# PrioteasaAndrei/music-style-transfer-ldm

Hardware: AMD Instinct MI355X
Metric: UNet denoising steps/sec on 1×128×512 mel-latents, 1/2/4/8 MI355X (higher is better)
Workload: dtype fp32; 1 GPU; config 2: 50-step DDIM reverse sample (49 UNet+update iterations per step), batch 8/GPU, 1x128x512 mel -> [8,32,16,64] latents, eta=0.0, hipGraph replay of 1 concurrent sub-batch chains; global_batch=8, parallelism=dp1 (batch shards)

## Files before the change

### include/ldm_capi.h

```cpp
#ifndef LDM_CAPI_H
#define LDM_CAPI_H

#include <stddef.h>
#include <stdint.h>

#ifdef __cplusplus
extern "C" {
#endif

#define LDM_CAPI_VERSION 1

const char* ldm_last_error(void);
int ldm_capi_version(void);
int ldm_device_count(int* count);

typedef struct ldm_conv_desc {
    int32_t B, Cin, Hin, Win;
    int32_t Cout, Hout, Wout;
    int32_t kh, kw, stride, pad, out_pad;
    int32_t transposed;
    int32_t layout;
} ldm_conv_desc;

enum {
// ... 19 lines not shown
    float bn_eps;
    int32_t act;
    const float* bcast_add;
    const float* skip_add;
    float* act_out;
    int32_t dtype;
} ldm_epilogue;

typedef struct ldm_conv_plan {
    int32_t kind;
    int32_t tm, tn, wk;
    int32_t ks;
    int32_t balance;
    int64_t packed_floats;
    int64_t ws_floats;
} ldm_conv_plan;

int ldm_conv_make_plan(const ldm_conv_desc* d, ldm_conv_plan* plan);
int ldm_conv_tiled_plan(const ldm_conv_desc* d, int32_t dtype, ldm_conv_plan* plan);
int ldm_conv_sconv_plan(const ldm_conv_desc* d, int32_t dtype, ldm_conv_plan* plan);
int ldm_conv_make_plan_forced(const ldm_conv_desc* d, int kind, int tm, int tn, int wk, int ks,
                              ldm_conv_plan* plan);
int ldm_conv_pack_weight(const ldm_conv_desc* d, const ldm_conv_plan* plan, const float* w,
                         float* packed, void* stream);
int32_t ldm_conv_storage16(const ldm_conv_desc* d, const ldm_conv_plan* plan);
int ldm_conv_forward(const ldm_conv_desc* d, const ldm_conv_plan* plan, const float* x, const float* w,
                     const ldm_epilogue* ep, float* y, void* stream);
int ldm_conv_forward_ws(const ldm_conv_desc* d, const ldm_conv_plan* plan, const float* x, const float* w,
                        const ldm_epilogue* ep, float* y, float* workspace, void* stream);

int64_t ldm_reduce_workspace_floats(int32_t B, int32_t C, int32_t HW);
int ldm_batchnorm_train(float* x, int32_t B, int32_t C, int32_t HW, const float* weight, const float* bias,
                        float* running_mean, float* running_var, float momentum, float eps, int32_t act,
                        float* save_mean, float* save_invstd, float* workspace, void* stream);
int ldm_batchnorm_train_out(const float* x, float* y, int32_t B, int32_t C, int32_t HW, const float* weight,
                            const float* bias, float* running_mean, float* running_var, float momentum, float eps,
                            int32_t act, float* save_mean, float* save_invstd, float* workspace, void* stream);
int ldm_batchnorm_stats(const float* x, int32_t B, int32_t C, int32_t HW, double* stats, float* workspace,
                        void* stream);
int ldm_batchnorm_stats_code(const float* x, int32_t code, int32_t B, int32_t C, int32_t HW, double* stats,
                             float* workspace, void* stream);
int ldm_batchnorm_apply(float* x, int32_t B, int32_t C, int32_t HW, const double* stats, double count,
                        const float* weight, const float* bias, float* running_mean, float* running_var,
                        float momentum, float eps, int32_t act, float* save_mean, float* save_invstd, void* stream);
int ldm_batchnorm_apply_out(const float* x, float* y, int32_t B, int32_t C, int32_t HW, const double* stats,
                            double count, const float* weight, const float* bias, float* running_mean,
                            float* running_var, float momentum, float eps, int32_t act, float* save_mean,
                            float* save_invstd, void* stream);

int ldm_batchnorm_eval(const float* x, float* y, int32_t B, int32_t C, int32_t HW, const float* weight,
                       const float* bias, const float* running_mean, const float* running_var, float eps, int32_t act,
                       void* stream);

int ldm_activation(const float* x, float* y, int64_t n, int32_t act, void* stream);

int ldm_sinusoid_embed(const void* t, int32_t t_is_float, int32_t B, int32_t dim, const float* freqs, float* out,
                       void* stream);

int ldm_time_mlp_forward(const void* t, int32_t t_is_float, int32_t B, int32_t dim, const float* freqs,
                         const float* w1, const float* b1, const float* w2, const float* b2, float* out,
                         void* stream);

int ldm_attention_fold_keys(const float* kv, const float* wq, const float* bq, int32_t B, int32_t E, int32_t heads,
                            int32_t S, float scale, float* kf, float* bf, void* stream);
int ldm_attention_folded(const float* z, const float* kv, const float* kf, const float* bf, float* out, int32_t B,
                         int32_t E, int32_t heads, int32_t L, int32_t S, void* stream);
int ldm_attention_folded_keys(const float* z, const float* kv, const float* kf, const float* bf,
                              const float* key_bias, float* out, int32_t B, int32_t E, int32_t heads, int32_t L,
                              int32_t S, void* stream);
int ldm_attention_fold_keys_bias(const float* kv, const float* wq, const float* bq, int32_t B, int32_t E,
                                 int32_t heads, int32_t S, float scale, const float* key_bias, float* kf, float* bf,
                                 void* stream);
int ldm_attention_folded_probs(const float* z, const float* kf, const float* bf, float* p, int32_t B, int32_t E,
                               int32_t heads, int32_t L, int32_t S, void* stream);
int32_t ldm_bneck_fold_supported(int32_t B, int32_t H, int32_t W);
int ldm_bneck_fold_values(const float* w_fold, const float* kv, float* u, int32_t B, void* stream);
int ldm_bneck_pv(const float* u, const float* p, const float* pos_bias, float* y, int32_t B, int32_t dtype,
                 void* stream);
int ldm_ca1_probs(const float* z4, const float* kf, const float* bf, float* p, int32_t B, void* stream);
int32_t ldm_ca1_probs_form(void);
int ldm_set_cin1_packed(int on);
int ldm_set_cin1_s1(int on);
int ldm_set_flash_split(int on);
int ldm_fold_conv_proj(const ldm_conv_desc* d, const float* w_conv, const float* b_conv, const float* w_proj,
                       const float* b_proj, int32_t Cmid, float* w_out, float* pos_bias_out, void* stream);
int ldm_attention_core(const float* q, const float* kv, float* out, int32_t B, int32_t E, int32_t heads,
                       int32_t L, int32_t S, float scale, void* stream);
int ldm_attention_flash_supported(int32_t E, int32_t heads);
int ldm_attention_forward_lse(const float* q, const float* kv, float* out, float* lse, int32_t B, int32_t E,
                              int32_t heads, int32_t L, int32_t S, float scale, void* stream);

int ldm_q_sample(const float* x0, const float* eps, const float* coef_table, int32_t T, const int64_t* t, float* zt,
                 int32_t B, int64_t per_sample, void* stream);
int ldm_predict_start(const float* zt, const float* eps, const float* coef_table, int32_t T, const int64_t* t,
                      float* x0, int32_t B, int64_t per_sample, void* stream);
int ldm_sched_backward(int32_t kind, const float* grad, const float* coef_table, int32_t T, const int64_t* t,
                       float* grad_a, float* grad_b, int32_t B, int64_t per_sample, void* stream);
int ldm_ddim_step(float* x, const float* eps, const float* coef, float eta, float* x0_log, float* eps_log,
                  int64_t n, void* stream);
int ldm_msolver_step(float* x, const float* eps, const float* coef, const float* x0_prev, float* x0_log,
                     float* eps_log, int64_t n, void* stream);

int ldm_loss_forward(int32_t kind, const float* a, const float* b, int64_t n, void* workspace, float* out,
                     void* stream);
int ldm_loss_backward(int32_t kind, const float* a, const float* b, int64_t n, const float* grad_out, float* grad_a,
                      float* grad_b, void* stream);

typedef struct ldm_unet_weights {
    const float* conv_w[9];
    const float* conv_b[9];
    ldm_conv_plan conv_plan[9];
    const float* ca_wq[2];
    const float* ca_bq[2];
    ldm_conv_plan ca_plan_q[2];
    const float* ca_wkv[2];
    const float* ca_bkv[2];
    ldm_conv_plan ca_plan_kv[2];
    const float* ca_wo[2];
    const float* ca_bo[2];
    ldm_conv_plan ca_plan_o[2];
    const float* t_freqs;
    const float* t_w1;
    const float* t_b1;
    const float* t_w2;
    const float* t_b2;
    const float* ca_wq_raw[2];
    const float* fold_w[2];
    const float* fold_pb[2];
    int32_t use_fold;
    const float* step_w[9];
    const float* step_pb[2];
    int32_t use_step;
    int32_t step_dtype;
    const float* step_bneck_w;
} ldm_unet_weights;

typedef struct ldm_unet_shape {
    int32_t B, C, H, W;
    int32_t nf;
} ldm_unet_shape;

int64_t ldm_unet_workspace_floats(const ldm_unet_shape* s, const ldm_unet_weights* w);
int ldm_unet_make_plans(const ldm_unet_shape* s, ldm_unet_weights* w);
int ldm_unet_layer_desc(const ldm_unet_shape* s, int32_t layer, ldm_conv_desc* d);
int ldm_unet_forward(const ldm_unet_shape* s, const ldm_unet_weights* w, const float* z, const void* t,
                     int32_t t_is_float, const float* s5, const float* s6, float* out, float* workspace,
                     void* stream);

#define LDM_SOLVER_DDIM 0
#define LDM_SOLVER_MULTISTEP 1

typedef struct ldm_sample_args {
    int32_t solver, nsteps;
    float eta;
    int32_t S5, S6;
    float* x;
    const float *s5, *s6, *key_bias5, *key_bias6;
    const float *s5_base, *s6_base, *key_bias5_base, *key_bias6_base, *guide_scale;
    const float *z0, *n0, *keep, *keep_coef;
    const int64_t* t_table;
    const float* coef_table;
    float *x0_logs, *eps_logs;
    int64_t log_step_stride;
    float* workspace;
    void* stream;
} ldm_sample_args;

int64_t ldm_sample_workspace_floats(const ldm_unet_shape* s, const ldm_unet_weights* w, const ldm_sample_args* a);
int ldm_sample(const ldm_unet_shape* s, const ldm_unet_weights* w, const ldm_sample_args* a);
int ldm_guide_eps(const float* e_t, const float* e_b, const float* scale, int64_t per_sample, int32_t B, float* out,
                  void* stream);
int ldm_keep_blend(float* x, const float* z0, const float* n0, const float* keep, const float* coef, int32_t B, int32_t C,
                   int64_t HW, void* stream);

int ldm_mel_quantize(const float* db, uint8_t* out, int64_t n, float max_db, void* stream);
int ldm_mel_dequantize(const uint8_t* in, float* db, int64_t n, float max_db, void* stream);
int ldm_u8_to_unit(const uint8_t* in, float* out, int64_t n, void* stream);

int64_t ldm_stft_table_floats(int32_t n_fft);
int ldm_stft_fill_tables(int32_t n_fft, float* host_tables);
int ldm_stft(const float* y, int32_t B, int64_t L, int32_t n_fft, int32_t hop, const float* tables, float* S,
             float* mag, int32_t power, void* stream);
int ldm_istft(const float* S, const float* mag, float* y, int32_t B, int32_t T, int64_t L, int32_t n_fft,
              int32_t hop, const float* tables, void* stream);
int64_t ldm_griffinlim_workspace(int32_t B, int32_t n_fft, int32_t T);
int ldm_griffinlim(const float* mag, const float* init_angles, float* y, int32_t B, int32_t T, int64_t L,
                   int32_t n_fft, int32_t hop, int32_t n_iter, float momentum, const float* tables,
                   float* workspace, void* stream);
int ldm_mel_project(const float* P, const float* M, const int32_t* lohi, float* mel, int32_t B, int32_t F,
                    int32_t n_mels, int32_t T, void* stream);
int ldm_power_to_db(const float* x, float* out, int32_t B, int64_t n, float amin, float top_db, float* workspace,
                    void* stream);
int ldm_db_to_power(const float* x, float* out, int64_t n, void* stream);
int ldm_mel_invert(const float* mel, const float* M, const float* Mt, const float* Minv, const int32_t* lohi,
                   float inv_lambda, int32_t iters, int32_t take_sqrt, float* x, float* workspace, int32_t B,
                   int32_t F, int32_t n_mels, int32_t T, void* stream);

int64_t ldm_resample_out_len(int64_t L, int32_t up, int32_t down);
int ldm_resample_f32(const float* x, int32_t B, int64_t L, const float* taps, int32_t up, int32_t down, int32_t W,
                     float* y, void* stream);
int ldm_resample_pcm16(const int16_t* pcm, int64_t L, int32_t channels, const float* taps, int32_t up, int32_t down,
                       int32_t W, float* y, void* stream);
int64_t ldm_trim_workspace_floats(int32_t B, int64_t L, int32_t hop);
int ldm_trim_bounds(const float* y, int32_t B, int64_t L, int32_t frame_length, int32_t hop, float top_db,
                    float* workspace, int64_t* bounds, void* stream);

int64_t ldm_mel_window_count(int64_t T_total, int32_t frames, int32_t overlap);
int ldm_mel_windows(const float* P, int32_t n_mels, int64_t T_total, int32_t frames, int32_t overlap, float amin,
                    float top_db, float max_db, float* x, float* ref_db, void* stream);
int ldm_mel_stitch(const float* y, const float* ref_db, int32_t N, int32_t n_mels, int32_t frames, int32_t overlap,
                   int64_t T_total, float max_db, float* power, float* db, void* stream);

int64_t ldm_step_packed_floats(int32_t layer);
int ldm_step_pack_weight(int32_t layer, const float* w, float* packed, void* stream);
int ldm_step_pack_weight_dt(int32_t layer, int32_t dtype, const float* w, float* packed, void* stream);
int ldm_step_conv(int32_t layer, int32_t B, int32_t H, int32_t W, const float* x, const float* packed,
                  const float* bias, const float* bcast, const float* skip, float* y, void* stream);
int64_t ldm_step_workspace_floats(int32_t B, int32_t H, int32_t W);
int64_t ldm_step_workspace_counter_floats(int32_t B, int32_t H, int32_t W);
int ldm_step_conv_ws(int32_t layer, int32_t B, int32_t H, int32_t W, const float* x, const float* packed,
                     const float* bias, const float* bcast, const float* skip, float* y, int32_t dtype,
                     float* workspace, void* stream);
int ldm_step_dec1_ddim(int32_t B, int32_t H, int32_t W, const float* d2, const float* packed, const float* bias,
                       const float* coef, float eta, float* xs, float* x0_log, float* eps_log, int32_t dtype,
                       void* stream);
int ldm_step_dec1_msolver(int32_t B, int32_t H, int32_t W, const float* d2, const float* packed, const float* bias,
                          const float* coef, float* xs, const float* x0_prev, float* x0_log, float* eps_log,
                          int32_t dtype, void* stream);
int ldm_step_layer_forms(int32_t* ks_layers);
int ldm_step_conv_dt(int32_t layer, int32_t B, int32_t H, int32_t W, const float* x, const float* packed,
                     const float* bias, const float* bcast, const float* skip, float* y, int32_t dtype, void* stream);

int64_t ldm_conv_wgrad_workspace_floats(const ldm_conv_desc* d);
int ldm_conv_backward_weight_dt(const ldm_conv_desc* d, const float* x, const float* dy, float* dw,
                                int32_t accumulate, float* workspace, int32_t dtype, void* stream);
int ldm_conv_backward_weight_defer(const ldm_conv_desc* d, const float* x, const float* dy, float* dw,
                                   int32_t accumulate, float* workspace, int32_t dtype, int32_t* splits_out,
                                   void* stream);
typedef struct ldm_wgrad_red_job {
    const float* partial;
    float* dw;
    int32_t S, MN, accumulate;
} ldm_wgrad_red_job;
int ldm_wgrad_reduce_many(const ldm_wgrad_red_job* jobs, int32_t n, void* stream);
int32_t ldm_conv_wgrad_storage16(const ldm_conv_desc* d);
int ldm_conv_backward_weight(const ldm_conv_desc* d, const float* x, const float* dy, float* dw, int32_t accumulate,
                             float* workspace, void* stream);
int ldm_act_backward(const float* dy, const float* act_out, const float* pre_act, int32_t act, int32_t B, int32_t C,
                     int32_t HW, float* dv, float* dbias, float* dbcast, float* workspace, void* stream);
int ldm_act_backward_defer(const float* dy, const float* act_out, const float* pre_act, int32_t act_code, int32_t B,
                           int32_t C, int32_t HW, float* dv, float* dbias, float* workspace, int32_t* q_out, void* stream);
int64_t ldm_act_partial_floats(int32_t B, int32_t C, int32_t HW);
// ... 84 lines not shown
```

### music-style-transfer-ldm_amd/csrc/common.h

```cpp
#pragma once
#include <hip/hip_runtime.h>

#include <cstdint>
#include <string>

#include "ldm_capi.h"

namespace ldm {

void set_error(const std::string& msg);
int fail(int code, const std::string& msg);

#define LDM_HIP_TRY(expr)                                                                      \
    do {                                                                                       \
        hipError_t _e = (expr);                                                                \
        if (_e != hipSuccess)                                                                  \
            return ::ldm::fail(1000 + (int)_e, std::string(#expr) + ": " + hipGetErrorString(_e)); \
    } while (0)

#define LDM_CHECK_LAUNCH(name)                                                                 \
    do {                                                                                       \
        hipError_t _e = hipGetLastError();                                                     \
        if (_e != hipSuccess)                                                                  \
            return ::ldm::fail(1000 + (int)_e, std::string("launch ") + name + ": " + hipGetErrorString(_e)); \
// ... 86 lines not shown
    int32_t dy[kMaxPhase][kMaxTap], dx[kMaxPhase][kMaxTap];
    int32_t kk[kMaxPhase][kMaxTap];
    int64_t wofs[kMaxPhase];
    int32_t kchunks[kMaxPhase];
};

int build_phase_table(const ldm_conv_desc& d, PhaseTable& pt);

struct PackJob {
    const float* w;
    void* out;
    int64_t first_block, total;
    int32_t kind, dt, Cin, Cout, KK, transposed, Mpad, nphase;
    int32_t ntap[kMaxPhase];
    int64_t wofs[kMaxPhase];
    int32_t kk[kMaxPhase][kMaxTap];
    FastDiv fd_mpad, fd_cin, fd_ntap[kMaxPhase];
    FastDiv fd_kr;
    int32_t remap;
};
int conv_pack_job(const ldm_conv_desc& d, const ldm_conv_plan& p, PackJob& j);
int tconv_pack_job(const ldm_conv_desc& d, const ldm_conv_plan& p, PackJob& j);

struct EpiArgs;
bool tconv_plan(const ldm_conv_desc& d, int dtype, ldm_conv_plan& plan);
int tconv_pack(const ldm_conv_desc& d, const ldm_conv_plan& p, const float* w, float* packed, hipStream_t st);
int tconv_forward(const ldm_conv_desc& d, const ldm_conv_plan& p, const float* x, const float* w, const EpiArgs& ep,
                  float* y, hipStream_t st);
bool sconv_plan(const ldm_conv_desc& d, int dtype, ldm_conv_plan& plan);
int sconv_forward(const ldm_conv_desc& d, const ldm_conv_plan& p, const float* x, const float* w, const EpiArgs& ep,
                  float* y, hipStream_t st);

struct EpiArgs {
    const float* bias;
    const float* bn_w;
    const float* bn_b;
    const float* bn_m;
    const float* bn_v;
    float bn_eps;
    int32_t act;
    const float* pos_bias;
    const float* bcast;
    const float* skip;
    float* act_out;
    const float* ddim_coef;
    float ddim_eta;
    float* ddim_x;
    float* ddim_x0_log;
    float* ddim_eps_log;
    int32_t lowp;
    int32_t round_out;
    int32_t x16, y16;
    const float* ms_coef;
    const float* ms_x0_prev;
    const float* guide_eb;
    const float* guide_scale;
    float* ddim_x2;
    const float* keep_z0;
    const float* keep_n0;
    const float* keep_w;
    const float* keep_coef;
};

int conv_forward_ex(const ldm_conv_desc& d, const ldm_conv_plan& p, const float* x, const float* w, const EpiArgs& ep,
                    float* y, float* ws, hipStream_t st);

int attention_core_ex(const float* q, const float* kv, float* out, int32_t B, int32_t E, int32_t heads, int32_t L,
                      int32_t S, float scale, bool tok, hipStream_t st);

bool attention_flash_supported(int E, int heads);
int attention_flash(const float* q, const float* kv, float* out, float* lse, int32_t B, int32_t E, int32_t heads,
                    int32_t L, int32_t S, float scale, bool tok, hipStream_t st);

int attention_folded(const float* z, const float* kv, const float* kf, const float* bf, float* out, int32_t B,
                     int32_t E, int32_t heads, int32_t L, int32_t S, hipStream_t st);
int attention_fold_keys(const float* kv, const float* wq, const float* bq, int32_t B, int32_t E, int32_t heads,
                        int32_t S, float scale, float* kf, float* bf, hipStream_t st);
int attention_folded_probs(const float* z, const float* kf, const float* bf, float* p, int32_t B, int32_t E,
                           int32_t heads, int32_t L, int32_t S, hipStream_t st);
int attention_folded_keys(const float* z, const float* kv, const float* kf, const float* bf, const float* key_bias,
                          float* out, int32_t B, int32_t E, int32_t heads, int32_t L, int32_t S, hipStream_t st);
int attention_fold_keys_bias(const float* kv, const float* wq, const float* bq, int32_t B, int32_t E, int32_t heads,
                             int32_t S, float scale, const float* key_bias, float* kf, float* bf, hipStream_t st);
bool bneck_fold_supported(int B, int H, int W);
int bneck_fold_values(const float* wf, const float* kv, float* u, int B, hipStream_t st);
int bneck_pv(const float* u, const float* p, const float* pb, float* y, int B, int dtype, hipStream_t st);

struct StepConv {
    const float* x;
    const float* w;
    float* y;
    const float* bias;
    const float* bcast;
    const float* skip;
    const float* coef;
    float eta;
    float* xs;
    float* x0_log;
    float* eps_log;
    int msolver;
    const float* x0_prev;
    int dtype;
    int plain;
    const float* guide_eb;
    const float* guide_scale;
    float* xs2;
    const float* keep_base;
    const float* keep_row;
    int64_t keep_stride;
    float* ws;
};
int step_conv(int layer, int B, int H, int W, const StepConv& s, hipStream_t st);
int64_t step_ws_floats(int B, int H, int W, int64_t* cnt_floats = nullptr);
int step_ks_mask();
#ifndef LDM_DEBUG_BOUNDS
#define LDM_DEBUG_BOUNDS 0
#endif
int step_layout(const float* x, float* y, int B, int C, int HW, bool to_nhwc, hipStream_t st);

bool wgrad2_plan_ws(const ldm_conv_desc& d, int64_t& ws_floats);
int wgrad2_run(const ldm_conv_desc& d, const float* dense, const float* gath, float* partial, int& splits, int dtype,
               hipStream_t st, int st16 = 0, float* dw_direct = nullptr);
int wgrad2_storage16(const ldm_conv_desc& d);

__device__ __forceinline__ float ddim_update(float xv, float e, const float* coef, float eta, float& x0) {
#pragma clang fp contract(off)
    const float sat = coef[0], s1t = coef[1], san = coef[2], s1n = coef[3];
    const float dxt = s1t * e;
    x0 = (xv - dxt) / sat;
    const float dxn = s1n * e;
    const float nc = eta * (dxn - dxt);
    const float t1 = san * x0;
    return (t1 + dxn) + nc;
}

__device__ __forceinline__ float msolver_update(float xv, float e, const float* coef, bool has_prev, float x0_prev,
                                                float& x0) {
#pragma clang fp contract(off)
    const float at = coef[0], st = coef[1], cx = coef[2], c0 = coef[3];
    const float dxt = st * e;
    x0 = (xv - dxt) / at;
    const float t0 = cx * xv;
    const float t1 = c0 * x0;
    float xn = t0 + t1;
    if (has_prev) {
        const float t2 = coef[4] * x0_prev;
        xn = xn + t2;
    }
    return xn;
}

__device__ __forceinline__ float guide_eps(float e_t, float e_b, float s) {
#pragma clang fp contract(off)
    const float d = e_t - e_b;
    const float g = s * d;
    return e_b + g;
}

__device__ __forceinline__ float keep_blend(float xu, float z0, float n0, float w, float a, float b) {
#pragma clang fp contract(off)
    const float k = a * z0;
    const float n = b * n0;
    const float known = k + n;
    const float u = 1.0f - w;
    const float p = u * xu;
    const float q = w * known;
    return p + q;
}

__device__ __forceinline__ float round16(float v, int mode) {
    if (mode == LDM_DT_F16) return (float)(_Float16)v;
    if (mode == LDM_DT_BF16) return (float)(__bf16)v;
    return v;
}

template <int ST>
__device__ __forceinline__ float from16(unsigned short u) {
    if constexpr (ST == LDM_DT_F16) return (float)__builtin_bit_cast(_Float16, u);
    else return __builtin_bit_cast(float, (unsigned)u << 16);
}
template <int ST>
__device__ __forceinline__ unsigned short to16s(float v) {
    if constexpr (ST == LDM_DT_F16) return __builtin_bit_cast(unsigned short, (_Float16)v);
    else return __builtin_bit_cast(unsigned short, (__bf16)v);
}
template <int ST, int W>
__device__ __forceinline__ void ld_st(const void* p, size_t o, bool h, float (&v)[W]) {
    if (ST != 0 && h) {
        const unsigned short* q = reinterpret_cast<const unsigned short*>(p) + o;
        if constexpr (W == 8) {
            const uint4 t = *reinterpret_cast<const uint4*>(q);
            const unsigned u[4] = {t.x, t.y, t.z, t.w};
#pragma unroll
// ... 125 lines not shown
```

### music-style-transfer-ldm_amd/csrc/conv.hip

```cpp
#include <algorithm>
#include <type_traits>
#include <cstdio>
#include <cstdlib>

#include "common.h"
#include "conv_epi.h"

#pragma clang fp contract(off)

#ifndef LDM_DIAG
#define LDM_DIAG 0
#endif

namespace ldm {

template <bool PH4 = true>
__device__ __forceinline__ int sel_phase(const int32_t (&v)[kMaxPhase], int ph) {
    if constexpr (!PH4) return v[0];
    const int x0 = v[0], x1 = v[1], x2 = v[2], x3 = v[3];
    return (x0 & -(int)(ph == 0)) | (x1 & -(int)(ph == 1)) | (x2 & -(int)(ph == 2)) | (x3 & -(int)(ph == 3));
}

int build_phase_table(const ldm_conv_desc& d, PhaseTable& pt) {
    pt = PhaseTable{};
    for (int p = 0; p < kMaxPhase; ++p)
        for (int t = 0; t < kMaxTap; ++t) pt.dy[p][t] = -0x4000;
    LDM_REQUIRE(d.B > 0 && d.Cin > 0 && d.Hin > 0 && d.Win > 0 && d.Cout > 0, "conv: empty dimension");
    LDM_REQUIRE(d.kh > 0 && d.kw > 0 && d.kh * d.kw <= kMaxTap, "conv: kernel larger than 4x4 unsupported");
    if (!d.transposed) {
        const int ho = (d.Hin + 2 * d.pad - d.kh) / d.stride + 1;
        const int wo = (d.Win + 2 * d.pad - d.kw) / d.stride + 1;
        LDM_REQUIRE(d.stride >= 1 && d.Hout == ho && d.Wout == wo, "conv: output size mismatch");
        pt.nphase = 1;
        pt.Hq = d.Hout;
        pt.Wq = d.Wout;
        pt.sy = d.stride;
        pt.osy = 1;
        pt.ry[0] = pt.rx[0] = 0;
        int n = 0;
        for (int a = 0; a < d.kh; ++a)
            for (int b = 0; b < d.kw; ++b) {
                pt.dy[0][n] = (int32_t)(a - d.pad);
                pt.dx[0][n] = (int32_t)(b - d.pad);
                pt.kk[0][n] = (int32_t)(a * d.kw + b);
                ++n;
            }
        pt.ntap[0] = n;
        return 0;
    }
    const int ho = (d.Hin - 1) * d.stride - 2 * d.pad + d.kh + d.out_pad;
    const int wo = (d.Win - 1) * d.stride - 2 * d.pad + d.kw + d.out_pad;
    LDM_REQUIRE(d.Hout == ho && d.Wout == wo, "conv_transpose: output size mismatch");
    if (d.stride == 1) {
        pt.nphase = 1;
        pt.Hq = d.Hout;
        pt.Wq = d.Wout;
        pt.sy = 1;
        pt.osy = 1;
        int n = 0;
        for (int a = 0; a < d.kh; ++a)
            for (int b = 0; b < d.kw; ++b) {
                pt.dy[0][n] = (int32_t)(d.pad - a);
                pt.dx[0][n] = (int32_t)(d.pad - b);
                pt.kk[0][n] = (int32_t)(a * d.kw + b);
                ++n;
            }
        pt.ntap[0] = n;
        return 0;
    }
    LDM_REQUIRE(d.stride == 2 && d.Hout == 2 * d.Hin && d.Wout == 2 * d.Win,
                "conv_transpose: only stride 2 with Hout == 2*Hin is supported");
    pt.nphase = 4;
    pt.Hq = d.Hin;
    pt.Wq = d.Win;
    pt.sy = 1;
    pt.osy = 2;
    for (int ry = 0; ry < 2; ++ry)
        for (int rx = 0; rx < 2; ++rx) {
            const int p = ry * 2 + rx;
            pt.ry[p] = ry;
            pt.rx[p] = rx;
            int n = 0;
            for (int a = 0; a < d.kh; ++a) {
                const int vy = ry + d.pad - a;
                if (vy & 1) continue;
                for (int b = 0; b < d.kw; ++b) {
                    const int vx = rx + d.pad - b;
                    if (vx & 1) continue;
                    LDM_REQUIRE(n < kMaxTap, "conv_transpose: too many taps");
// ... 13 lines not shown

static int layout_for_plan(const ldm_conv_desc& d, const ldm_conv_plan& p, PhaseTable& pt, int& Mpad, int64_t& floats) {
    int rc = build_phase_table(d, pt);
    if (rc) return rc;
    floats = 0;
    Mpad = d.Cout;
    if (p.kind == 0) {
        for (int i = 0; i < pt.nphase; ++i) pt.wofs[i] = 0, pt.kchunks[i] = 0;
        return 0;
    }
    const int ck = chunk_k(p.kind);
    LDM_REQUIRE(d.Cin % ck == 0, "conv: MFMA plan needs Cin % chunk == 0");
    const int bm = tile_m(p.kind) * p.tm;
    Mpad = (d.Cout + bm - 1) / bm * bm;
    for (int i = 0; i < pt.nphase; ++i) {
        pt.kchunks[i] = pt.ntap[i] * (d.Cin / ck);
        pt.wofs[i] = floats;
        floats += (int64_t)pt.kchunks[i] * Mpad * ck;
    }
    return 0;
}

template <int KIND>
struct Mfma;

template <>
struct Mfma<1> {
    static constexpr int TILE = 32, NLG = 2, NACC = 16;
    typedef floatx16 acc_t;
    static __device__ __forceinline__ acc_t mma(float a, float b, acc_t c) {
        return __builtin_amdgcn_mfma_f32_32x32x2f32(a, b, c, 0, 0, 0);
    }
    static __device__ __forceinline__ int row(int r, int lg) { return (r & 3) + 8 * (r >> 2) + 4 * lg; }
    template <int DT>
    static __device__ __forceinline__ acc_t mma4(floatx4 a, floatx4 b, acc_t c) { return mma32_lowp<DT>(a, b, c); }
};

template <>
struct Mfma<2> {
    static constexpr int TILE = 16, NLG = 4, NACC = 4;
    typedef floatx4 acc_t;
    static __device__ __forceinline__ acc_t mma(float a, float b, acc_t c) {
        return __builtin_amdgcn_mfma_f32_16x16x4f32(a, b, c, 0, 0, 0);
    }
    static __device__ __forceinline__ int row(int r, int lg) { return 4 * lg + r; }
    template <int DT>
    static __device__ __forceinline__ acc_t mma4(floatx4 a, floatx4 b, acc_t c) { return mma16_lowp<DT>(a, b, c); }
};

constexpr int kMaxKSplit = 16;
constexpr int kMaxConvLds = 160 * 1024;

template <int TM, int TN>
struct Frag {
    floatx4 a[TM];
    float b[TN][4];
};

#ifndef LDM_DIAG
#define LDM_DIAG 0
#endif
#if (LDM_DIAG & 4)
__device__ unsigned long long g_ldm_stamps[1 << 16][6];
#define LDM_STAMP(k)                                                                               \
    do {                                                                                           \
        if (threadIdx.x == 0 && blockIdx.x < (1u << 16))                                          \
            g_ldm_stamps[blockIdx.x][k] = ((k) == 0 || (k) == 5) ? __builtin_amdgcn_s_memrealtime()           \
                                                                 : __builtin_amdgcn_s_memtime();          \
    } while (0)
#else
#define LDM_STAMP(k) \
    do {             \
    } while (0)
#endif

__device__ __forceinline__ void part_store(float* p, float v) {
    __hip_atomic_store(p, v, __ATOMIC_RELAXED, __HIP_MEMORY_SCOPE_AGENT);
}
__device__ __forceinline__ float part_load(const float* p) {
    return __hip_atomic_load(const_cast<float*>(p), __ATOMIC_RELAXED, __HIP_MEMORY_SCOPE_AGENT);
}

template <int KIND, int TM, int TN, int WK, int NT, bool NHWC, int DT>
__global__ __launch_bounds__(64 * WK) void conv_mfma_kernel(ConvArgs a) {
    LDM_STAMP(0);
    using MF = Mfma<KIND>;
    constexpr bool PH4 = NT == 4;
    constexpr int kGroup = TM * TN == 1 ? 8 : (TM * TN == 2 ? 4 : 2);
    constexpr int TILE = MF::TILE, NLG = MF::NLG, CK = 4 * NLG;
    constexpr int BM = TILE * TM, BN = TILE * TN;
    constexpr int LDB = BN + 1, SLAB = BM * LDB;
    extern __shared__ __attribute__((aligned(16))) float smem[];
    __shared__ int s_last;
    const int lane = threadIdx.x & 63;
    const int wave = __builtin_amdgcn_readfirstlane(threadIdx.x >> 6);
    const int HqWq = a.pt.Hq * a.pt.Wq;
    const int Nq = a.B * HqWq;
    int ph, mt, nt, ksp;
    {
        const int nwg = gridDim.x, orig = blockIdx.x;
        const int rest = a.fd_nn.div(orig);
        const int nt0 = orig - rest * a.fd_nn.d;
        const int ph0 = PH4 ? a.fd_nm.div(rest) : 0;
        const int mx0 = rest - ph0 * a.fd_nm.d;
        const int q = nwg >> 3, r = nwg & 7, xcd = orig & 7;
        const int wgid = (xcd < r ? xcd * (q + 1) : r * (q + 1) + (xcd - r) * q) + (orig >> 3);
        const int tile = PH4 ? (wgid >> 2) : wgid;
        const int ph1 = PH4 ? (wgid & 3) : 0;
        const int outer = a.fd_inner.div(tile);
        const int inner = tile - outer * a.fd_inner.d;
        const int o = a.tile_order;
        const int m0_ = -(int)(o == 0), m1_ = -(int)(o == 1), m2_ = -(int)(o == 2);
        ph = (ph0 & m0_) | (ph1 & ~m0_);
        const int mtx = (mx0 & m0_) | (outer & m1_) | (inner & m2_);
        nt = (nt0 & m0_) | (inner & m1_) | (outer & m2_);
        mt = a.fd_ks.div(mtx);
        ksp = mtx - mt * a.ks;
        if constexpr (PH4) {
            if (a.balance) {
                const int p = (int)(wgid >= a.bofs[1]) + (int)(wgid >= a.bofs[2]) + (int)(wgid >= a.bofs[3]);
                const int local = wgid - sel_phase<true>(a.bofs, p);
                const int lks = sel_phase<true>(a.bks_log2, p);
                const int r2 = a.fd_nn.div(local);
                nt = local - r2 * a.fd_nn.d;
                mt = r2 >> lks;
                ksp = r2 - (mt << lks);
                ph = p;
            }
        }
    }
    const int ksn = uni((PH4 && a.balance) ? 1 << sel_phase<PH4>(a.bks_log2, ph) : a.ks);
    const int m0 = mt * BM, n0 = nt * BN;
    const int HWin = a.Hin * a.Win;
    const int col = lane % TILE, lg = lane / TILE;

    constexpr int kOOB = 0x7ffffff0;
    int iy0[TN], ix0[TN], base4[TN];
#pragma unroll
    for (int ni = 0; ni < TN; ++ni) {
        const int n = n0 + TILE * ni + col;
        const bool nv = n < Nq;
        const int nn = nv ? n : 0;
        const int b = a.fd_hw.div(nn);
        const int r = nn - b * HqWq;
        const int qy = a.fd_w.div(r);
        const int qx = r - qy * a.pt.Wq;
        const int iyv = qy * a.pt.sy;
        iy0[ni] = nv ? iyv : -0x4000000;
        ix0[ni] = qx * a.pt.sy;
        base4[ni] = NHWC ? (((b * a.Hin + iyv) * a.Win + ix0[ni]) * a.Cin + 4 * lg) * 4
                         : ((b * a.Cin + 4 * lg) * HWin + iyv * a.Win + ix0[ni]) * 4;
    }

    typename MF::acc_t acc[TM][TN];
#pragma unroll
    for (int mi = 0; mi < TM; ++mi)
#pragma unroll
        for (int ni = 0; ni < TN; ++ni)
#pragma unroll
            for (int r = 0; r < MF::NACC; ++r) acc[mi][ni][r] = 0.f;

    const int cpt = a.Cin / CK;
    const int nchunk = sel_phase<PH4>(a.pk.kchunks, ph);
    const int ph_ry = sel_phase<PH4>(a.pk.ry, ph), ph_rx = sel_phase<PH4>(a.pk.rx, ph);
    const int wstride_b = a.Mpad * CK * 4;
    const int G = uni(ksn * WK), g = uni(ksp * WK + wave);
    const int nmine = nchunk > g ? uni((nchunk - g + G - 1) / G) : 0;
    const int ngrp = (nmine + kGroup - 1) / kGroup;
    const __amdgpu_buffer_rsrc_t xr =
        __builtin_amdgcn_make_buffer_rsrc(uni_ptr(a.x), (short)0, uni(a.B * a.Cin * HWin * 4), 0x00020000);
    const __amdgpu_buffer_rsrc_t wr = __builtin_amdgcn_make_buffer_rsrc(
        uni_ptr(a.w + sel_phase<PH4>(a.pk.wofs, ph)), (short)0, uni(nchunk * wstride_b), 0x00020000);
    const int a_voff = ((m0 + col) * CK + lg * 4) * 4;
    const int cstep_b = NHWC ? CK * 4 : CK * HWin * 4;
    const int tap_mul = NHWC ? a.Cin * 4 : 4;

    constexpr int EPT = (BM * BN + 64 * WK - 1) / (64 * WK);
    constexpr bool kPre = EPT <= 8;
    EpiPre pre[kPre ? EPT : 1];
    int po[kPre ? EPT : 1], pm[kPre ? EPT : 1], ps[kPre ? EPT : 1];
    const bool onhwc = a.out_nhwc != 0;
    auto elem = [&](int e, int& mloc, int& nloc) {
        const int nl_c = e / BM, ml_c = e - nl_c * BM;
// ... 196 lines not shown
        for (int ni = 0; ni < TN; ++ni)
#pragma unroll
            for (int r = 0; r < MF::NACC; ++r)
                sw[(TILE * mi + MF::row(r, lg)) * LDB + TILE * ni + col] = acc[mi][ni][r];
    __syncthreads();
    LDM_STAMP(4);
    if (ksn == 1) {
        if constexpr (kPre) {
#pragma unroll
            for (int k = 0; k < EPT; ++k) {
                if (po[k] < 0) continue;
                const int si = ps[k];
                float v = smem[si];
#pragma unroll
                for (int w = 1; w < WK; ++w) v = v + smem[w * SLAB + si];
                epi_finish(a, pm[k], (size_t)po[k], v, pre[k]);
            }
        } else {
            for (int e = threadIdx.x; e < BM * BN; e += 64 * WK) {
                int mloc, nloc;
                elem(e, mloc, nloc);
                const int m = m0 + mloc, n = n0 + nloc;
                if (m >= a.Cout || n >= Nq) continue;
                const int si = mloc * LDB + nloc;
                float v = smem[si];
#pragma unroll
                for (int w = 1; w < WK; ++w) v = v + smem[w * SLAB + si];
                const int b = n / HqWq;
                const int r = n - b * HqWq;
                const int qyy = r / a.pt.Wq;
                const int qxx = r - qyy * a.pt.Wq;
                epilogue_store(a, m, b, qyy * a.pt.osy + ph_ry, qxx * a.pt.osy + ph_rx, v);
            }
        }
        LDM_STAMP(5);
        return;
    }

    const int tile = (ph * a.nM + mt) * a.nN + nt;
    float* tpart = a.part + (size_t)tile * a.ks * (BM * BN);
    for (int e = threadIdx.x; e < BM * BN; e += 64 * WK) {
        int mloc, nloc;
        elem(e, mloc, nloc);
        const int si = mloc * LDB + nloc;
        float v = smem[si];
#pragma unroll
        for (int w = 1; w < WK; ++w) v = v + smem[w * SLAB + si];
        part_store(tpart + (size_t)ksp * (BM * BN) + e, v);
    }
    asm volatile("s_waitcnt vmcnt(0)" ::: "memory");
    __syncthreads();
    if (threadIdx.x == 0) {
        const int old = __hip_atomic_fetch_add(a.cnt + tile, 1, __ATOMIC_RELAXED, __HIP_MEMORY_SCOPE_AGENT);
        const int last = old == ksn - 1;
        if (last) __hip_atomic_store(a.cnt + tile, 0, __ATOMIC_RELAXED, __HIP_MEMORY_SCOPE_AGENT);
        s_last = last;
    }
    __syncthreads();
    if (!s_last) return;
    for (int e = threadIdx.x; e < BM * BN; e += 64 * WK) {
        int mloc, nloc;
        elem(e, mloc, nloc);
        const int m = m0 + mloc, n = n0 + nloc;
        if (m >= a.Cout || n >= Nq) continue;
        const int si = mloc * LDB + nloc;
        float own = smem[si];
#pragma unroll
        for (int w = 1; w < WK; ++w) own = own + smem[w * SLAB + si];
        float pv[kMaxKSplit];
#pragma unroll
        for (int s2 = 0; s2 < kMaxKSplit; ++s2)
            if (s2 < ksn && s2 != ksp) pv[s2] = part_load(tpart + (size_t)s2 * (BM * BN) + e);
        float v = ksp == 0 ? own : pv[0];
#pragma unroll
        for (int s2 = 1; s2 < kMaxKSplit; ++s2)
            if (s2 < ksn) v = v + (s2 == ksp ? own : pv[s2]);
        const int b = n / HqWq;
        const int r = n - b * HqWq;
        const int qyy = r / a.pt.Wq;
        const int qxx = r - qyy * a.pt.Wq;
        epilogue_store(a, m, b, qyy * a.pt.osy + ph_ry, qxx * a.pt.osy + ph_rx, v);
    }
    LDM_STAMP(5);
}
#if (LDM_DIAG & 4)
extern "C" int ldm_debug_stamps(unsigned long long* host, int nblocks) {
    return (int)hipMemcpyFromSymbol(host, HIP_SYMBOL(g_ldm_stamps), sizeof(unsigned long long) * 6 * nblocks, 0,
                                    hipMemcpyDeviceToHost);
}
#endif

__global__ __launch_bounds__(256) void conv_direct_kernel(ConvArgs a) {
    __shared__ int tab[kMaxPhase * kMaxTap * 3 + kMaxPhase];
    for (int i = threadIdx.x; i < kMaxPhase * kMaxTap * 3 + kMaxPhase; i += blockDim.x) {
        const int which = i / (kMaxPhase * kMaxTap), e = i - which * (kMaxPhase * kMaxTap);
        const int ph = e / kMaxTap, t = e - ph * kMaxTap;
        tab[i] = which == 0 ? a.pt.dy[ph][t] : which == 1 ? a.pt.dx[ph][t] : which == 2 ? a.pt.kk[ph][t]
                                                                                      : a.pt.ntap[e < kMaxPhase ? e : 0];
    }
    __syncthreads();
    const int total = a.B * a.Cout * a.Hout * a.Wout;
    const int idx = (int)(blockIdx.x * blockDim.x + threadIdx.x);
    if (idx >= total) return;
    int rest = a.fd_dwo.div(idx);
    const int ox = idx - rest * a.Wout;
    int r2 = a.fd_dho.div(rest);
    const int oy = rest - r2 * a.Hout;
    const int b = a.fd_dco.div(r2);
    const int co = r2 - b * a.Cout;
    int ph, qy, qx;
    if (a.pt.osy == 1) {
        ph = 0;
        qy = oy;
        qx = ox;
    } else {
        ph = (oy & 1) * 2 + (ox & 1);
        qy = oy >> 1;
        qx = ox >> 1;
    }
    const int HWin = a.Hin * a.Win;
    const float* xb = a.x + (size_t)b * a.Cin * HWin;
    const int wci = a.transposed ? a.Cout * a.KK : a.KK;
    const float* wb = a.w + (a.transposed ? (size_t)co * a.KK : (size_t)co * a.Cin * a.KK);
    const int nt = tab[kMaxPhase * kMaxTap * 3 + ph];
    int off[kMaxTap], wkk[kMaxTap];
    bool ok[kMaxTap];
#pragma unroll
    for (int t = 0; t < kMaxTap; ++t) {
        const int e = ph * kMaxTap + t;
        const int iy = qy * a.pt.sy + tab[e];
        const int ix = qx * a.pt.sy + tab[kMaxPhase * kMaxTap + e];
        ok[t] = t < nt && iy >= 0 && iy < a.Hin && ix >= 0 && ix < a.Win;
        off[t] = ok[t] ? iy * a.Win + ix : 0;
        wkk[t] = t < nt ? tab[2 * kMaxPhase * kMaxTap + e] : 0;
    }
    float acc = 0.f;
    for (int ci = 0; ci < a.Cin; ++ci) {
        const float* xp = xb + (size_t)ci * HWin;
        const float* wq = wb + (size_t)ci * wci;
        float xv[kMaxTap], wv[kMaxTap];
#pragma unroll
        for (int t = 0; t < kMaxTap; ++t) {
            xv[t] = round16(t < nt ? xp[off[t]] : 0.f, a.ep.lowp);
            wv[t] = round16(t < nt ? wq[wkk[t]] : 0.f, a.ep.lowp);
        }
#pragma unroll
        for (int t = 0; t < kMaxTap; ++t)
            if (ok[t]) acc = fmaf(xv[t], wv[t], acc);
    }
    epilogue_store(a, co, b, oy, ox, acc);
}

constexpr int kC1Groups = 8;
__global__ __launch_bounds__(256) void conv_cout1_k3_kernel(ConvArgs a) {
    constexpr int G = kC1Groups, QB = 256 / G;
    __shared__ float wsm[512 * 9];
    __shared__ float4 red[G][QB];
    const int Cin = a.Cin;
    for (int i = threadIdx.x; i < Cin * 9; i += 256) wsm[i] = round16(a.w[i], a.ep.lowp);
    __syncthreads();
    const int g = threadIdx.x / QB, ql = threadIdx.x - g * QB;
    const int wq = a.Wout >> 2;
    const int quad = blockIdx.x * QB + ql;
    const int nquad = a.B * a.Hout * wq;
    const bool qv = quad < nquad;
    const int qq = qv ? quad : 0;
// ... 849 lines not shown
            a.fd_dwo = FastDiv::make(d.Win / 4);
            static const bool split = [] {
                const char* e = std::getenv("LDM_CT4_SPLIT");
                return !e || std::atoi(e) != 0;
            }();
            if (d.Hin % 2 == 0 && d.Cin % 8 == 0 && split) {
                a.fd_dho = FastDiv::make(d.Hin / 2);
                const int64_t tiles = (int64_t)d.B * (d.Hin / 2) * (d.Win / 4);
                lp_dispatch(a.ep, [&](auto lp, auto ro) {
                    constexpr int LP = decltype(lp)::value, RO = decltype(ro)::value;
                    if (LP != 0 && ep.x16)
                        hipLaunchKernelGGL((convT4_cout1_r2s_kernel<LP, RO, LP>), dim3((unsigned)((tiles + 63) / 64)), dim3(256), 0, st, a);
                    else
                        hipLaunchKernelGGL((convT4_cout1_r2s_kernel<LP, RO, 0>), dim3((unsigned)((tiles + 63) / 64)), dim3(256), 0, st, a);
                });
                LDM_CHECK_LAUNCH("convT4_cout1_r2s_kernel");
                return 0;
            }
            if (d.Hin % 2 == 0) {
                a.fd_dho = FastDiv::make(d.Hin / 2);
                const int64_t lanes = (int64_t)d.B * (d.Hin / 2) * (d.Win / 4);
                lp_dispatch(a.ep, [&](auto lp, auto ro) {
                    constexpr int LP = decltype(lp)::value, RO = decltype(ro)::value;
                    if (LP != 0 && ep.x16)
                        hipLaunchKernelGGL((convT4_cout1_r2_kernel<LP, RO, LP>), dim3((unsigned)((lanes + 255) / 256)), dim3(256), 0, st, a);
                    else
                        hipLaunchKernelGGL((convT4_cout1_r2_kernel<LP, RO, 0>), dim3((unsigned)((lanes + 255) / 256)), dim3(256), 0, st, a);
                });
                LDM_CHECK_LAUNCH("convT4_cout1_r2_kernel");
                return 0;
            }
            a.fd_dho = FastDiv::make(d.Hin);
            const int64_t lanes = (int64_t)d.B * d.Hin * (d.Win / 4);
            lp_dispatch(a.ep, [&](auto lp, auto ro) {
                    constexpr int LP = decltype(lp)::value, RO = decltype(ro)::value;
                    if (LP != 0 && ep.x16)
                        hipLaunchKernelGGL((convT4_cout1_kernel<LP, RO, LP>), dim3((unsigned)((lanes + 255) / 256)), dim3(256), 0, st, a);
                    else
                        hipLaunchKernelGGL((convT4_cout1_kernel<LP, RO, 0>), dim3((unsigned)((lanes + 255) / 256)), dim3(256), 0, st, a);
                });
            LDM_CHECK_LAUNCH("convT4_cout1_kernel");
            return 0;
        }
        LDM_REQUIRE(!ep.x16 && !ep.y16, "conv: 16-bit storage on a path without it (ldm_conv_storage16)");
        if (d.Cin == 1 && !d.transposed && d.Cout <= 64 && a.KK <= 16) {
            const int64_t pix = (int64_t)d.B * d.Hout * d.Wout;
            hipLaunchKernelGGL(conv_cin1_kernel, dim3((unsigned)((pix + 255) / 256)), dim3(256), 0, st, a);
            LDM_CHECK_LAUNCH("conv_cin1_kernel");
            return 0;
        }
        if (!d.transposed && d.Cout == 1 && d.kh == 3 && d.kw == 3 && d.stride == 1 && d.pad == 1 && d.Cin % kC1Groups == 0 &&
            d.Cin <= 512 && d.Wout % 4 == 0 && d.Win == d.Wout && d.Hin == d.Hout && ((uintptr_t)x & 15) == 0 && cout1_on()) {
            a.fd_dwo = FastDiv::make(d.Wout / 4);
            a.fd_dho = FastDiv::make(d.Hout);
            const int64_t quads = (int64_t)d.B * d.Hout * (d.Wout / 4);
            constexpr int QB = 256 / kC1Groups;
            hipLaunchKernelGGL(conv_cout1_k3_kernel, dim3((unsigned)((quads + QB - 1) / QB)), dim3(256), 0, st, a);
            LDM_CHECK_LAUNCH("conv_cout1_k3_kernel");
            return 0;
        }
        hipLaunchKernelGGL(conv_direct_kernel, dim3((unsigned)((total + 255) / 256)), dim3(256), 0, st, a);
        LDM_CHECK_LAUNCH("conv_direct_kernel");
        return 0;
    }
    LDM_REQUIRE(plan_ok(d, p.kind, p.tm, p.tn, p.wk, p.ks), "conv forward: invalid plan");
    LDM_REQUIRE(!ep.x16 && !ep.y16, "conv: 16-bit storage on a path without it (ldm_conv_storage16)");
    if (a.ks > 1) {
        PhaseTable pt2;
        LDM_REQUIRE(build_phase_table(d, pt2) == 0 && p.ws_floats == split_ws_floats(d, p, pt2),
                    "conv forward: plan workspace size does not match the descriptor");
        a.cnt = reinterpret_cast<int32_t*>(ws);
        a.part = ws + kSplitCounters;
    }
    LDM_REQUIRE((int64_t)d.B * d.Cin * d.Hin * d.Win * 4 < 0x7ff00000LL &&
                    p.packed_floats * 4 < 0x7ff00000LL && (int64_t)d.B * d.Cout * d.Hout * d.Wout * 4 < 0x7ff00000LL,
                "conv forward: tensor too large for 32-bit buffer offsets (split the batch)");
    const bool in_nhwc = d.layout & 1;
    if (a.ep.lowp == LDM_DT_BF16 && !in_nhwc)
        return p.kind == 1 ? launch_mfma<1, false, 2>(a, p, Nq, st) : launch_mfma<2, false, 2>(a, p, Nq, st);
    if (p.kind == 1) return in_nhwc ? launch_mfma<1, true, 0>(a, p, Nq, st) : launch_mfma<1, false, 0>(a, p, Nq, st);
    return in_nhwc ? launch_mfma<2, true, 0>(a, p, Nq, st) : launch_mfma<2, false, 0>(a, p, Nq, st);
}

}

extern "C" int ldm_conv_forward_ws(const ldm_conv_desc* d, const ldm_conv_plan* plan, const float* x, const float* w,
                                   const ldm_epilogue* ep, float* y, float* workspace, void* stream) {
    LDM_REQUIRE(d && plan && x && w && y, "conv forward: null argument");
    EpiArgs e{};
    if (ep) {
        e.bias = ep->bias;
        e.bn_w = ep->bn_weight;
        e.bn_b = ep->bn_bias;
        e.bn_m = ep->bn_mean;
        e.bn_v = ep->bn_var;
        e.bn_eps = ep->bn_eps;
        e.act = ep->act;
        e.bcast = ep->bcast_add;
        e.skip = ep->skip_add;
        e.act_out = ep->act_out;
        e.lowp = ep->dtype & 0xff;
        LDM_REQUIRE(e.lowp >= LDM_DT_F32 && e.lowp <= LDM_DT_BF16 &&
                        (ep->dtype & ~(0xff | LDM_DT_ROUND_OUT | LDM_DT_X16 | LDM_DT_Y16)) == 0,
                    "conv forward: unknown operand precision");
        e.round_out = (ep->dtype & LDM_DT_ROUND_OUT) ? e.lowp : 0;
        e.x16 = (ep->dtype & LDM_DT_X16) ? 1 : 0;
        e.y16 = (ep->dtype & LDM_DT_Y16) ? 1 : 0;
        LDM_REQUIRE(e.lowp != LDM_DT_F32 || (!e.x16 && !e.y16), "conv forward: 16-bit storage needs a 16-bit dtype");
    }
    return conv_forward_ex(*d, *plan, x, w, e, y, workspace, (hipStream_t)stream);
}

extern "C" int32_t ldm_conv_storage16(const ldm_conv_desc* d, const ldm_conv_plan* plan) {
    if (!d || !plan) return 0;
    if (plan->kind == 3) return LDM_DT_X16 | LDM_DT_Y16;
    if (plan->kind != 0 || d->layout != 0) return 0;
    if (d->Cin == 1 && !d->transposed && d->Cout <= 64 && d->kh == d->kw && (d->kh == 3 || d->kh == 4) &&
        d->stride == 2 && d->Wout % 4 == 0)
        return LDM_DT_Y16;
    if (d->transposed && d->Cout == 1 && d->kh == 4 && d->kw == 4 && d->stride == 2 && d->pad == 1 && d->out_pad == 0 &&
        d->Win % 4 == 0)
        return LDM_DT_X16;
    return 0;
}

extern "C" int ldm_conv_forward(const ldm_conv_desc* d, const ldm_conv_plan* plan, const float* x, const float* w,
                                const ldm_epilogue* ep, float* y, void* stream) {
    return ldm_conv_forward_ws(d, plan, x, w, ep, y, nullptr, stream);
}

extern "C" int ldm_set_cin1_packed(int on) {
    const int prev = ldm::g_cin1_packed;
    ldm::g_cin1_packed = on ? 1 : 0;
    return prev;
}

extern "C" int ldm_set_cin1_s1(int on) {
    const int prev = ldm::g_cin1_s1;
    ldm::g_cin1_s1 = on ? 1 : 0;
    return prev;
}
```

### music-style-transfer-ldm_amd/csrc/misc.hip

```cpp
#include <algorithm>

#include "common.h"

#pragma clang fp contract(off)

namespace ldm {

__global__ __launch_bounds__(256) void time_mlp_kernel(const void* t, int t_is_float, int dim, const float* __restrict__ freqs,
                                                       const float* __restrict__ w1, const float* __restrict__ b1,
                                                       const float* __restrict__ w2, const float* __restrict__ b2,
                                                       float* __restrict__ out) {
    extern __shared__ __attribute__((aligned(16))) float sm[];
    float* emb = sm;
    float* hid = sm + dim;
    const int b = blockIdx.x, i = threadIdx.x;
    const float tv = t_is_float ? ((const float*)t)[b] : (float)((const int64_t*)t)[b];
    const int half = dim / 2;
    if (i < dim) {
        const float arg = tv * freqs[i < half ? i : i - half];
        emb[i] = i < half ? sinf(arg) : cosf(arg);
    }
    __syncthreads();
    if (i < dim) {
        const float* wr = w1 + (size_t)i * dim;
        float acc = 0.f;
        for (int k = 0; k < dim; ++k) acc = fmaf(wr[k], emb[k], acc);
        const float x = acc + b1[i];
        hid[i] = x * 0.5f * (1.0f + erff(x * 0.70710678118654752440f));
    }
    __syncthreads();
    if (i < dim) {
        const float* wr = w2 + (size_t)i * dim;
        float acc = 0.f;
        for (int k = 0; k < dim; ++k) acc = fmaf(wr[k], hid[k], acc);
        out[(size_t)b * dim + i] = acc + b2[i];
    }
}

constexpr int kAttnLT = 16;

__global__ __launch_bounds__(256) void attention_core_kernel(const float* __restrict__ q, const float* __restrict__ kv,
                                                             float* __restrict__ out, int E, int heads, int L, int S,
                                                             float scale) {
    extern __shared__ __attribute__((aligned(16))) float sm[];
    const int d = E / heads;
    const int ltiles = (L + kAttnLT - 1) / kAttnLT;
    const int lt = blockIdx.x % ltiles;
    const int h = (blockIdx.x / ltiles) % heads;
    const int b = blockIdx.x / (ltiles * heads);
    const int l0 = lt * kAttnLT;
    const int nl = min(kAttnLT, L - l0);
    float* Qs = sm;
    float* Ks = Qs + d * kAttnLT;
    float* Vs = Ks + d * S;
    float* Ps = Vs + d * S;
    const float* qb = q + ((size_t)b * E + (size_t)h * d) * L;
    const float* kb = kv + ((size_t)b * 2 * E + (size_t)h * d) * S;
    const float* vb = kv + ((size_t)b * 2 * E + E + (size_t)h * d) * S;
    for (int e = threadIdx.x; e < d * kAttnLT; e += blockDim.x) {
        const int c = e / kAttnLT, l = e - c * kAttnLT;
        Qs[e] = l < nl ? qb[(size_t)c * L + l0 + l] * scale : 0.f;
    }
    for (int e = threadIdx.x; e < d * S; e += blockDim.x) {
        Ks[e] = kb[e];
        Vs[e] = vb[e];
    }
    __syncthreads();
    for (int e = threadIdx.x; e < kAttnLT * S; e += blockDim.x) {
        const int l = e / S, s = e - l * S;
        float acc = 0.f;
        for (int c = 0; c < d; ++c) acc = fmaf(Qs[c * kAttnLT + l], Ks[c * S + s], acc);
        Ps[e] = acc;
    }
    __syncthreads();
    const int lane = threadIdx.x & 63, wave = threadIdx.x >> 6, nw = blockDim.x >> 6;
    for (int l = wave; l < nl; l += nw) {
        float* row = Ps + l * S;
        float mx = -INFINITY;
        for (int s = lane; s < S; s += 64) mx = fmaxf(mx, row[s]);
        for (int o = 32; o > 0; o >>= 1) mx = fmaxf(mx, __shfl_xor(mx, o));
        float sum = 0.f;
        for (int s = lane; s < S; s += 64) {
            const float ex = expf(row[s] - mx);
            row[s] = ex;
            sum += ex;
        }
        for (int o = 32; o > 0; o >>= 1) sum += __shfl_xor(sum, o);
        for (int s = lane; s < S; s += 64) row[s] = row[s] / sum;
    }
    __syncthreads();
    float* ob = out + ((size_t)b * E + (size_t)h * d) * L;
    for (int e = threadIdx.x; e < d * kAttnLT; e += blockDim.x) {
        const int c = e / kAttnLT, l = e - c * kAttnLT;
        if (l >= nl) continue;
        float acc = 0.f;
        const float* pr = Ps + l * S;
        const float* vr = Vs + c * S;
        for (int s = 0; s < S; ++s) acc = fmaf(pr[s], vr[s], acc);
        ob[(size_t)c * L + l0 + l] = acc;
    }
}

template <int KIND>
struct AMfma;
template <>
struct AMfma<1> {
    static constexpr int TILE = 32, NLG = 2, NACC = 16;
    typedef floatx16 acc_t;
    static __device__ __forceinline__ acc_t mma(float a, float b, acc_t c) {
        return __builtin_amdgcn_mfma_f32_32x32x2f32(a, b, c, 0, 0, 0);
    }
    static __device__ __forceinline__ int row(int r, int lg) { return (r & 3) + 8 * (r >> 2) + 4 * lg; }
};
template <>
struct AMfma<2> {
    static constexpr int TILE = 16, NLG = 4, NACC = 4;
    typedef floatx4 acc_t;
    static __device__ __forceinline__ acc_t mma(float a, float b, acc_t c) {
        return __builtin_amdgcn_mfma_f32_16x16x4f32(a, b, c, 0, 0, 0);
// ... 178 lines not shown
    }
    __syncthreads();
    if constexpr (PONLY) {
        float* pb = out + ((size_t)(b * heads + h) * L + l0) * S;
        for (int e = threadIdx.x; e < LT * SP; e += 64 * NW) {
            const int r = e / SP, s = e % SP;
            if (l0 + r < L && s < S) pb[(size_t)r * S + s] = Ps[r * LDP + s];
        }
        return;
    }
    constexpr int NTC = D / TILE;
    float* ob = TOK ? out + (size_t)b * L * E + (size_t)h * D : out + ((size_t)b * E + (size_t)h * D) * L;
    for (int tile = wave; tile < NTC * NTL; tile += NW) {
        const int ct = tile / NTL, lt = tile % NTL;
        typename MF::acc_t acc;
#pragma unroll
        for (int r = 0; r < MF::NACC; ++r) acc[r] = 0.f;
        const float* va = Vs + (ct * TILE + col) * LDP + lg;
        const float* pb = Ps + (lt * TILE + col) * LDP + lg;
#pragma unroll
        for (int k0 = 0; k0 < SP; k0 += KBP * NLG) {
            float av[KBP], bv[KBP];
#pragma unroll
            for (int j = 0; j < KBP; ++j) {
                av[j] = va[k0 + NLG * j];
                bv[j] = pb[k0 + NLG * j];
            }
#pragma unroll
            for (int j = 0; j < KBP; ++j) acc = MF::mma(av[j], bv[j], acc);
        }
        const int l = l0 + lt * TILE + col;
        if (l < L) {
            if constexpr (TOK && KIND == 2) {
                *reinterpret_cast<float4*>(ob + (size_t)l * E + ct * TILE + 4 * lg) = make_float4(acc[0], acc[1], acc[2], acc[3]);
            } else {
#pragma unroll
                for (int r = 0; r < MF::NACC; ++r) ob[(ct * TILE + MF::row(r, lg)) * qcs + l * qls] = acc[r];
            }
        }
    }
}

__global__ __launch_bounds__(256) void attention_fold_keys_kernel(const float* __restrict__ kv, const float* __restrict__ wq,
                                                                  const float* __restrict__ bq, int B, int E, int heads,
                                                                  int S, float scale, float* __restrict__ kf,
                                                                  float* __restrict__ bf, int64_t first) {
    const int d = E / heads;
    const int64_t nk = (int64_t)B * heads * E * S;
    const int64_t idx = first + (int64_t)blockIdx.x * blockDim.x + threadIdx.x;
    if (idx < nk) {
        const int e = (int)(idx % E);
        int64_t r = idx / E;
        const int s = (int)(r % S);
        r /= S;
        const int h = (int)(r % heads), b = (int)(r / heads);
        const float* kr = kv + ((int64_t)b * 2 * E + (int64_t)h * d) * S + s;
        const float* wr = wq + (int64_t)h * d * E + e;
        double acc = 0.0;
        int c = 0;
        for (; c + 16 <= d; c += 16) {
            float wv[16], kvv[16];
#pragma unroll
            for (int u = 0; u < 16; ++u) {
                wv[u] = wr[(int64_t)(c + u) * E];
                kvv[u] = kr[(int64_t)(c + u) * S];
            }
#pragma unroll
            for (int u = 0; u < 16; ++u) acc += (double)wv[u] * (double)kvv[u];
        }
        for (; c < d; ++c) acc += (double)wr[(int64_t)c * E] * (double)kr[(int64_t)c * S];
        kf[idx] = (float)(acc * (double)scale);
    } else if (idx < nk + (int64_t)B * heads * S) {
        const int64_t j = idx - nk;
        const int s = (int)(j % S);
        const int bh = (int)(j / S);
        const int h = bh % heads, b = bh / heads;
        const float* kr = kv + ((int64_t)b * 2 * E + (int64_t)h * d) * S + s;
        double acc = 0.0;
        for (int c = 0; c < d; ++c) acc += (double)bq[h * d + c] * (double)kr[(int64_t)c * S];
        bf[j] = (float)(acc * (double)scale);
    }
}

__global__ __launch_bounds__(256) void attention_fold_keys4_kernel(const float* __restrict__ kv, const float* __restrict__ wq,
                                                                   const float* __restrict__ bq, int B, int E, int heads,
                                                                   int S, float scale, float* __restrict__ kf,
                                                                   float* __restrict__ bf) {
    const int d = E / heads;
    const int SG = S / 4;
    const int64_t n = (int64_t)B * heads * SG * (E + 1);
    const int64_t idx = (int64_t)blockIdx.x * blockDim.x + threadIdx.x;
    if (idx >= n) return;
    const int e = (int)(idx % (E + 1));
    int64_t r = idx / (E + 1);
    const int sg = (int)(r % SG);
    r /= SG;
    const int h = (int)(r % heads), b = (int)(r / heads);
    const float* kr = kv + ((int64_t)b * 2 * E + (int64_t)h * d) * S + sg * 4;
    const bool isb = e == E;
    const float* wr = isb ? bq + h * d : wq + (int64_t)h * d * E + e;
    const int64_t ws = isb ? 1 : E;
    double acc[4] = {0., 0., 0., 0.};
    int c = 0;
    for (; c + 16 <= d; c += 16) {
        float wv[16];
        float4 kq[16];
#pragma unroll
        for (int u = 0; u < 16; ++u) {
            wv[u] = wr[(int64_t)(c + u) * ws];
            kq[u] = *reinterpret_cast<const float4*>(kr + (int64_t)(c + u) * S);
        }
#pragma unroll
        for (int u = 0; u < 16; ++u) {
            const double w = (double)wv[u];
            acc[0] += w * (double)kq[u].x;
            acc[1] += w * (double)kq[u].y;
            acc[2] += w * (double)kq[u].z;
            acc[3] += w * (double)kq[u].w;
        }
    }
    for (; c < d; ++c) {
        const double w = (double)wr[(int64_t)c * ws];
        const float4 k = *reinterpret_cast<const float4*>(kr + (int64_t)c * S);
        acc[0] += w * (double)k.x;
        acc[1] += w * (double)k.y;
        acc[2] += w * (double)k.z;
        acc[3] += w * (double)k.w;
    }
    if (isb) {
#pragma unroll
        for (int j = 0; j < 4; ++j) bf[((int64_t)b * heads + h) * S + sg * 4 + j] = (float)(acc[j] * (double)scale);
        return;
    }
    float* out = kf + (((int64_t)b * heads + h) * S + sg * 4) * E + e;
#pragma unroll
    for (int j = 0; j < 4; ++j) out[(int64_t)j * E] = (float)(acc[j] * (double)scale);
}

__global__ __launch_bounds__(256) void fold_conv_proj_kernel(const float* __restrict__ wc, const float* __restrict__ bc,
                                                             const float* __restrict__ wp, const float* __restrict__ bp,
                                                             int Cout, int Cmid, int Cin, int kh, int kw, int stride,
                                                             int pad, int Hin, int Win, int Hout, int Wout,
                                                             float* __restrict__ w_out, float* __restrict__ pb_out) {
    const int KK = kh * kw;
    const int64_t nw = (int64_t)Cout * Cin * KK;
    const int64_t idx = (int64_t)blockIdx.x * blockDim.x + threadIdx.x;
    if (idx < nw) {
        const int t = (int)(idx % KK);
        const int64_t r = idx / KK;
        const int ci = (int)(r % Cin), co = (int)(r / Cin);
        const float* wr = wc + (int64_t)co * Cmid * KK + t;
        double acc = 0.0;
        for (int j = 0; j < Cmid; ++j) acc += (double)wr[(int64_t)j * KK] * (double)wp[(int64_t)j * Cin + ci];
        w_out[idx] = (float)acc;
    } else if (idx < nw + (int64_t)Cout * Hout * Wout) {
        const int64_t p = idx - nw;
        const int ox = (int)(p % Wout);
        const int oy = (int)((p / Wout) % Hout);
        const int co = (int)(p / ((int64_t)Hout * Wout));
        double acc = bc ? (double)bc[co] : 0.0;
        for (int ky = 0; ky < kh; ++ky) {
            const int iy = oy * stride - pad + ky;
            if (iy < 0 || iy >= Hin) continue;
            for (int kx = 0; kx < kw; ++kx) {
                const int ix = ox * stride - pad + kx;
                if (ix < 0 || ix >= Win) continue;
                const float* wr = wc + (int64_t)co * Cmid * KK + ky * kw + kx;
                for (int j = 0; j < Cmid; ++j) acc += (double)wr[(int64_t)j * KK] * (double)bp[j];
            }
        }
        pb_out[p] = (float)acc;
    }
}

__device__ __forceinline__ bool load_coef(const float* table, int T, const int64_t* t, int b, float& sa, float& s1) {
    const int64_t tb = t[b];
    if (tb < 0 || tb >= T) {
        sa = s1 = __builtin_nanf("");
        return false;
    }
    sa = table[2 * tb];
    s1 = table[2 * tb + 1];
    return true;
}

__global__ __launch_bounds__(256) void q_sample_kernel(const float* __restrict__ x0, const float* __restrict__ eps,
                                                       const float* __restrict__ table, int T,
                                                       const int64_t* __restrict__ t, float* __restrict__ zt,
                                                       int64_t per_sample, int64_t n) {
    const int64_t i = (int64_t)blockIdx.x * blockDim.x + threadIdx.x;
    if (i >= n) return;
    float sa, s1;
    load_coef(table, T, t, (int)(i / per_sample), sa, s1);
    const float u = sa * x0[i];
    const float v = s1 * eps[i];
    zt[i] = u + v;
}

__global__ __launch_bounds__(256) void predict_start_kernel(const float* __restrict__ zt, const float* __restrict__ eps,
                                                            const float* __restrict__ table, int T,
                                                            const int64_t* __restrict__ t, float* __restrict__ x0,
                                                            int64_t per_sample, int64_t n) {
    const int64_t i = (int64_t)blockIdx.x * blockDim.x + threadIdx.x;
    if (i >= n) return;
    float sa, s1;
    load_coef(table, T, t, (int)(i / per_sample), sa, s1);
    const float v = s1 * eps[i];
    x0[i] = (zt[i] - v) / sa;
}

__global__ __launch_bounds__(256) void sched_backward_kernel(int kind, const float* __restrict__ g,
                                                             const float* __restrict__ table, int T,
                                                             const int64_t* __restrict__ t, float* __restrict__ ga,
                                                             float* __restrict__ gb, int64_t per_sample, int64_t n) {
    const int64_t i = (int64_t)blockIdx.x * blockDim.x + threadIdx.x;
    if (i >= n) return;
    float sa, s1;
    load_coef(table, T, t, (int)(i / per_sample), sa, s1);
    const float gv = g[i];
// ... 126 lines not shown
    if (kind == 0) {
        const float d = 2.0f * (a[i] - (b ? b[i] : 0.f)) * scale;
        if (ga) ga[i] = d;
        if (gb) gb[i] = -d;
    } else {
        const float av = a[i];
        const float a2 = av * av;
        if (ga) ga[i] = (av - av / (a2 + 1e-8f)) * scale;
    }
}

static unsigned blocks_for(int64_t n, int t) { return (unsigned)((n + t - 1) / t); }

}

using namespace ldm;

extern "C" int ldm_time_mlp_forward(const void* t, int32_t t_is_float, int32_t B, int32_t dim, const float* freqs,
                                    const float* w1, const float* b1, const float* w2, const float* b2, float* out,
                                    void* stream) {
    LDM_REQUIRE(t && freqs && w1 && b1 && w2 && b2 && out, "time_mlp: null argument");
    LDM_REQUIRE(B > 0 && dim > 1 && dim % 2 == 0 && dim <= 256, "time_mlp: unsupported dim");
    const int threads = (dim + 63) / 64 * 64;
    hipLaunchKernelGGL(time_mlp_kernel, dim3(B), dim3(threads), 2 * dim * sizeof(float), (hipStream_t)stream, t,
                       t_is_float, dim, freqs, w1, b1, w2, b2, out);
    LDM_CHECK_LAUNCH("time_mlp_kernel");
    return 0;
}

namespace ldm {
int attention_folded(const float* z, const float* kv, const float* kf, const float* bf, float* out, int32_t B,
                     int32_t E, int32_t heads, int32_t L, int32_t S, hipStream_t st) {
    LDM_REQUIRE(z && kv && kf && bf && out, "attention (folded): null argument");
    LDM_REQUIRE(B > 0 && heads == 4 && L > 0 && S > 0, "attention (folded): bad shape");
    const int d = E / heads;
#define LDM_ATTF(LP, SP, D, LT, EQV, NWV)                                                                \
    if (d == D && E == EQV && L <= LP && S <= SP) {                                                      \
        const size_t lds = ((size_t)NWV * LT * (SP + 1) + (size_t)D * (SP + 1)) * sizeof(float);       \
        if (lds > 64 * 1024) {                                                                           \
            static bool opted = false;                                                                   \
            if (!opted) {                                                                                \
                LDM_HIP_TRY(hipFuncSetAttribute(                                                         \
                    (const void*)attention_mfma_kernel<2, LP, SP, D, LT, true, EQV, NWV>,                  \
                    hipFuncAttributeMaxDynamicSharedMemorySize, 160 * 1024));                            \
                opted = true;                                                                            \
            }                                                                                            \
        }                                                                                                \
        hipLaunchKernelGGL((attention_mfma_kernel<2, LP, SP, D, LT, true, EQV, NWV>), dim3(B * heads * (LP / LT)), \
                           dim3(64 * NWV), lds, st, z, kv, out, E, heads, L, S, 1.0f, kf, bf);           \
        LDM_CHECK_LAUNCH("attention_mfma_kernel (folded)");                                              \
        return 0;                                                                                        \
    }
    LDM_ATTF(16, 16, 128, 16, 512, 8)
    LDM_ATTF(64, 64, 64, 16, 256, 16)
    LDM_ATTF(32, 32, 64, 16, 256, 8)
    LDM_ATTF(32, 32, 128, 16, 512, 8)
    LDM_ATTF(16, 16, 64, 16, 256, 4)
#undef LDM_ATTF
    return fail(3, "attention (folded): no instance for this shape");
}

int attention_folded_probs(const float* z, const float* kf, const float* bf, float* p, int32_t B, int32_t E,
                           int32_t heads, int32_t L, int32_t S, hipStream_t st) {
    LDM_REQUIRE(z && kf && bf && p, "attention probs (folded): null argument");
    LDM_REQUIRE(B > 0 && heads == 4 && E == 512 && L > 0 && L <= 16 && S > 0 && S <= 16,
                "attention probs (folded): instances for CA1's 2 x 8 plane only (E 512, L, S <= 16)");
    static const int nw = [] {
        const char* e = std::getenv("LDM_CA1P_WAVES");
        return e && std::atoi(e) == 16 ? 16 : 8;
    }();
    if (nw == 16) {
        auto kfn = attention_mfma_kernel<2, 16, 16, 128, 16, true, 512, 16, true>;
        const size_t lds = ((size_t)16 * 16 * 17 + (size_t)128 * 17) * sizeof(float);
        hipLaunchKernelGGL(kfn, dim3(B * heads), dim3(64 * 16), lds, st, z, kf, p, E, heads, L, S, 1.0f, kf, bf);
    } else {
        auto kfn = attention_mfma_kernel<2, 16, 16, 128, 16, true, 512, 8, true>;
        const size_t lds = ((size_t)8 * 16 * 17 + (size_t)128 * 17) * sizeof(float);
        hipLaunchKernelGGL(kfn, dim3(B * heads), dim3(64 * 8), lds, st, z, kf, p, E, heads, L, S, 1.0f, kf, bf);
    }
    LDM_CHECK_LAUNCH("attention_mfma_kernel (folded, probabilities)");
    return 0;
}

int attention_fold_keys(const float* kv, const float* wq, const float* bq, int32_t B, int32_t E, int32_t heads,
                        int32_t S, float scale, float* kf, float* bf, hipStream_t st) {
    LDM_REQUIRE(kv && wq && bq && kf && bf && B > 0 && heads > 0 && E % heads == 0 && S > 0, "fold keys: bad argument");
    const int64_t nk = (int64_t)B * heads * E * S, nb = (int64_t)B * heads * S;
    static const bool k4_on = [] {
        const char* e = std::getenv("LDM_FOLD_KEYS4");
        return e ? std::atoi(e) != 0 : true;
    }();
    const bool k4 = k4_on && S % 4 == 0 && ((uintptr_t)kv & 15) == 0;
    if (k4) {
        const int64_t n4 = (int64_t)B * heads * (S / 4) * (E + 1);
        hipLaunchKernelGGL(attention_fold_keys4_kernel, dim3((unsigned)((n4 + 255) / 256)), dim3(256), 0, st, kv, wq, bq,
                           B, E, heads, S, scale, kf, bf);
        LDM_CHECK_LAUNCH("attention_fold_keys4_kernel");
        return 0;
    }
    const int64_t first = 0, n = nk + nb - first;
    hipLaunchKernelGGL(attention_fold_keys_kernel, dim3((unsigned)((n + 255) / 256)), dim3(256), 0, st, kv, wq, bq, B,
                       E, heads, S, scale, kf, bf, first);
    LDM_CHECK_LAUNCH("attention_fold_keys_kernel");
    return 0;
}

int attention_core_ex(const float* q, const float* kv, float* out, int32_t B, int32_t E, int32_t heads, int32_t L,
                      int32_t S, float scale, bool tok, hipStream_t st) {
    LDM_REQUIRE(q && kv && out, "attention: null argument");
    LDM_REQUIRE(B > 0 && heads > 0 && E % heads == 0 && L > 0 && S > 0, "attention: bad shape");
    const int d = E / heads;
    {
        const dim3 blk(256);
#define LDM_ATT(KIND, LP, SP, D, LT)                                                                      \
    if (d == D && L <= LP && S <= SP) {                                                                   \
        const size_t lds = ((size_t)LT * (SP + 1) + (size_t)D * (SP + 1)) * sizeof(float);              \
        if (tok)                                                                                          \
            hipLaunchKernelGGL((attention_mfma_kernel<KIND, LP, SP, D, LT, true>), dim3(B * heads * (LP / LT)), blk, \
                               lds, st, q, kv, out, E, heads, L, S, scale);                               \
        else                                                                                              \
            hipLaunchKernelGGL((attention_mfma_kernel<KIND, LP, SP, D, LT, false>), dim3(B * heads * (LP / LT)), \
                               blk, lds, st, q, kv, out, E, heads, L, S, scale);                          \
        LDM_CHECK_LAUNCH("attention_mfma_kernel");                                                        \
        return 0;                                                                                         \
    }
        LDM_ATT(2, 16, 16, 64, 16)
        LDM_ATT(2, 16, 16, 128, 16)
        LDM_ATT(2, 32, 32, 64, 16)
        LDM_ATT(2, 32, 32, 128, 16)
        LDM_ATT(2, 64, 64, 64, 16)
        LDM_ATT(2, 64, 64, 128, 16)
#undef LDM_ATT
    }
    if (attention_flash_supported(E, heads)) return attention_flash(q, kv, out, nullptr, B, E, heads, L, S, scale, tok, st);
    LDM_REQUIRE(!tok, "attention: token-major layout needs an MFMA instance for this head size");
    const size_t lds = ((size_t)d * kAttnLT + 2 * (size_t)d * S + (size_t)kAttnLT * S) * sizeof(float);
    LDM_REQUIRE(lds <= 64 * 1024, "attention: head tile exceeds LDS budget");
    const int ltiles = (L + kAttnLT - 1) / kAttnLT;
    hipLaunchKernelGGL(attention_core_kernel, dim3(B * heads * ltiles), dim3(256), lds, st, q, kv, out, E, heads, L, S,
                       scale);
    LDM_CHECK_LAUNCH("attention_core_kernel");
    return 0;
}
}

extern "C" int ldm_attention_core(const float* q, const float* kv, float* out, int32_t B, int32_t E, int32_t heads,
                                  int32_t L, int32_t S, float scale, void* stream) {
    return ldm::attention_core_ex(q, kv, out, B, E, heads, L, S, scale, false, (hipStream_t)stream);
}

extern "C" int ldm_q_sample(const float* x0, const float* eps, const float* coef_table, int32_t T, const int64_t* t,
                            float* zt, int32_t B, int64_t per_sample, void* stream) {
    LDM_REQUIRE(x0 && eps && coef_table && t && zt && B > 0 && per_sample > 0 && T > 0, "q_sample: bad argument");
    const int64_t n = (int64_t)B * per_sample;
    hipLaunchKernelGGL(q_sample_kernel, dim3(blocks_for(n, 256)), dim3(256), 0, (hipStream_t)stream, x0, eps,
                       coef_table, T, t, zt, per_sample, n);
    LDM_CHECK_LAUNCH("q_sample_kernel");
    return 0;
}

extern "C" int ldm_predict_start(const float* zt, const float* eps, const float* coef_table, int32_t T,
                                 const int64_t* t, float* x0, int32_t B, int64_t per_sample, void* stream) {
    LDM_REQUIRE(x0 && eps && coef_table && t && zt && B > 0 && per_sample > 0 && T > 0, "predict_start: bad argument");
    const int64_t n = (int64_t)B * per_sample;
    hipLaunchKernelGGL(predict_start_kernel, dim3(blocks_for(n, 256)), dim3(256), 0, (hipStream_t)stream, zt, eps,
                       coef_table, T, t, x0, per_sample, n);
    LDM_CHECK_LAUNCH("predict_start_kernel");
    return 0;
}

extern "C" int ldm_sched_backward(int32_t kind, const float* grad, const float* coef_table, int32_t T, const int64_t* t,
                                  float* grad_a, float* grad_b, int32_t B, int64_t per_sample, void* stream) {
    LDM_REQUIRE(grad && coef_table && t && B > 0 && per_sample > 0 && T > 0 && (kind == 0 || kind == 1),
                "sched_backward: bad argument");
    const int64_t n = (int64_t)B * per_sample;
    hipLaunchKernelGGL(sched_backward_kernel, dim3(blocks_for(n, 256)), dim3(256), 0, (hipStream_t)stream, kind, grad,
// ... 121 lines not shown
```

### music-style-transfer-ldm_amd/csrc/uconv.hip

```cpp
#include <algorithm>
#include <cstdlib>

#include "uconv_kernel.h"

namespace ldm {
namespace uc {

template <int DT>
__global__ __launch_bounds__(256) void uconv_pack_kernel(const float* __restrict__ w, void* __restrict__ outp,
                                                         int CIN, int COUT, int transposed) {
    const int64_t total = (int64_t)9 * CIN * COUT;
    const int64_t idx = (int64_t)blockIdx.x * blockDim.x + threadIdx.x;
    if (idx >= total) return;
    const int e = (int)(idx % 16);
    const int m = (int)((idx / 16) % COUT);
    const int c = (int)(idx / (16 * (int64_t)COUT));
    const int cc = c / 9, t = c % 9;
    const int ci = cc * 16 + e;
    const float v = transposed ? w[((int64_t)ci * COUT + m) * 9 + t] : w[((int64_t)m * CIN + ci) * 9 + t];
    if constexpr (DT == 0)
        reinterpret_cast<float*>(outp)[idx] = v;
    else if constexpr (DT == LDM_DT_F16)
        reinterpret_cast<_Float16*>(outp)[idx] = (_Float16)v;
    else
        reinterpret_cast<__bf16*>(outp)[idx] = (__bf16)v;
}

__global__ __launch_bounds__(256) void nchw_to_nhwc_kernel(const float* __restrict__ x, float* __restrict__ y, int C,
                                                           int HW, int64_t n) {
    const int64_t idx = (int64_t)blockIdx.x * blockDim.x + threadIdx.x;
    if (idx >= n) return;
    const int c = (int)(idx % C);
    const int64_t r = idx / C;
    const int p = (int)(r % HW);
    const int64_t b = r / HW;
    y[idx] = x[(b * C + c) * HW + p];
}
__global__ __launch_bounds__(256) void nhwc_to_nchw_kernel(const float* __restrict__ x, float* __restrict__ y, int C,
                                                           int HW, int64_t n) {
    const int64_t idx = (int64_t)blockIdx.x * blockDim.x + threadIdx.x;
    if (idx >= n) return;
    const int p = (int)(idx % HW);
    const int64_t r = idx / HW;
    const int c = (int)(r % C);
    const int64_t b = r / C;
    y[idx] = x[(b * HW + p) * C + c];
}

struct LayerGeo {
    int mode, cin, cout;
};
constexpr LayerGeo kGeo[9] = {
    {0, 32, 64},
    {1, 64, 128},
    {1, 128, 256},
    {1, 256, 512},
    {0, 512, 512},
    {2, 512, 256},
    {2, 256, 128},
    {2, 128, 64},
    {0, 64, 32},
};
constexpr int kDiv[9] = {1, 1, 2, 4, 8, 8, 4, 2, 1};


struct KsGeo {
    int tm, tn, wk, ks, wn = 1;
};
constexpr KsGeo kKs[9] = {
    {0, 0, 0, 0},
    {0, 0, 0, 0},
    {2, 2, 4, 2},
    {2, 2, 4, 4},
    {2, 2, 8, 4},
    {2, 2, 4, 8},
    {2, 2, 4, 4},
    {0, 0, 0, 0},
    {0, 0, 0, 0},
};

constexpr KsGeo kKs2[9] = {
    {0, 0, 0, 0}, {0, 0, 0, 0}, {0, 0, 0, 0},
    {1, 2, 8, 2},
    {1, 2, 4, 4, 2},
    {1, 2, 8, 4},
    {0, 0, 0, 0}, {0, 0, 0, 0}, {0, 0, 0, 0},
};

constexpr KsGeo kKs3[9] = {
    {2, 1, 2, 1, 4},
    {2, 1, 4, 1, 2},
    {2, 1, 8, 1},
    {1, 1, 16, 1},
    {0, 0, 0, 0},
    {1, 1, 16, 2},
    {1, 1, 16, 1},
    {1, 2, 8, 1},
    {1, 2, 4, 1, 2},
};
constexpr int kKs3Default = 0x1ED;

static int env_int(const char* name, int dflt, int base = 10) {
    const char* e = std::getenv(name);
    return e ? (int)std::strtol(e, nullptr, base) : dflt;
}
static int ks3_mask() {
    static const int m = env_int("LDM_UCONV_KS3", kKs3Default, 0);
    return m;
}
constexpr int kKsDefault = (1 << 3) | (1 << 4) | (1 << 5);
static int ks_mask() {
    static const int m = env_int("LDM_UCONV_KS", kKsDefault, 0);
    return m;
}
constexpr int kKsDefaultLowp = kKsDefault;
static int ks_mask_lowp() {
    static const int m = env_int("LDM_UCONV_KS_LOWP", kKsDefaultLowp, 0);
    return m;
}
// ... 24 lines not shown
}
static bool plane_taps() {
    static const bool on = env_int("LDM_UCONV_PLANE", 1) != 0;
    return on;
}
static bool dec4_par() {
    static const bool on = env_int("LDM_UCONV_DEC4_PAR", 1) != 0;
    return on;
}

static bool ks_on(int layer, int dtype = LDM_DT_F32) {
    return kKs[layer].ks > 1 && (((dtype == LDM_DT_F32 ? ks_mask() : ks_mask_lowp()) >> layer) & 1);
}
static int ks_form(int layer, int dtype = LDM_DT_F32, int H = 16, int W = 64) {
    if (layer >= 0 && layer <= 8 && kKs3[layer].wk > 0 && ((ks3_mask() >> layer) & 1) && H == 16 && W == 64 &&
        (layer == 3 || layer == 5 ? plane_taps() : window_taps()))
        return 3;
    if (layer < 0 || layer > 8 || !ks_on(layer, dtype)) return 0;
    return (kKs2[layer].ks > 1 && ((ks2_mask() >> layer) & 1)) ? 2 : 1;
}
static const KsGeo& ks_row(int layer, int form) { return form == 3 ? kKs3[layer] : (form == 2 ? kKs2[layer] : kKs[layer]); }
static void ks_tiles(int layer, int B, int H, int W, int64_t& tiles, int64_t& slab_floats, int form = 1) {
    const LayerGeo& g = kGeo[layer];
    const KsGeo& k = ks_row(layer, form);
    const int Hin = H / kDiv[layer], Win = W / kDiv[layer];
    const int64_t nq = (int64_t)B * (g.mode == 1 ? (Hin / 2) * (Win / 2) : Hin * Win);
    tiles = (int64_t)(g.cout / (16 * k.tm)) * ((nq + 16 * k.tn * k.wn - 1) / (16 * k.tn * k.wn));
    slab_floats = tiles * k.ks * (g.mode == 2 ? 4 : 1) * k.tm * k.tn * k.wn * 256;
}
}

int64_t step_packed_floats(int layer) {
    if (layer < 0 || layer > 8) return -1;
    return (int64_t)9 * uc::kGeo[layer].cin * uc::kGeo[layer].cout;
}

int step_ks_mask() {
    int m = uc::ks_mask();
    for (int l = 0; l < 9; ++l)
        if (uc::kKs3[l].wk > 0 && ((uc::ks3_mask() >> l) & 1))
            m = uc::kKs3[l].ks > 1 && !(l == 5 && uc::dec4_par()) ? (m | (1 << l)) : (m & ~(1 << l));
    return m;
}

int64_t step_ws_floats(int B, int H, int W, int64_t* cnt_floats) {
    using namespace uc;
    int64_t mt = 0, ms = 0;
    for (int l = 0; l < 9; ++l) {
        for (int form = 1; form <= 3; ++form) {
            if ((form == 1 ? kKs[l].ks : (form == 2 ? kKs2[l].ks : kKs3[l].ks)) <= 1) continue;
            int64_t t, sf;
            ks_tiles(l, B, H, W, t, sf, form);
            mt = std::max(mt, t);
            ms = std::max(ms, sf);
        }
    }
    const int64_t c = (mt + 63) / 64 * 64;
    if (cnt_floats) *cnt_floats = c;
    return c + ms;
}


namespace uc {
static int make_args(int layer, int B, int H, int W, const StepConv& s, UArgs& a) {
    LDM_REQUIRE(layer >= 0 && layer <= 8, "step conv: layer index");
    LDM_REQUIRE(B > 0 && H % 8 == 0 && W % 8 == 0, "step conv: latent H, W must be multiples of 8");
    const LayerGeo& g = kGeo[layer];
    const int Hin = H / kDiv[layer], Win = W / kDiv[layer];
    a = UArgs{};
    a.x = s.x;
    a.w = s.w;
    a.y = s.y;
    a.bias = s.bias;
    a.bcast = s.bcast;
    a.skip = s.skip;
    a.coef = s.coef;
    a.xs = s.xs;
    a.x0_log = s.x0_log;
    a.eps_log = s.eps_log;
    a.eta = s.eta;
    a.x0_prev = s.x0_prev;
    if (s.guide_eb) a.skip = s.guide_eb, a.bcast = s.guide_scale, a.y = s.xs2;
    if (s.keep_base) a.skip = s.keep_base, a.bcast = s.keep_row;
    a.B = B;
    a.Hin = Hin;
    a.Win = Win;
    if (g.mode == 0) {
        a.Hout = Hin, a.Wout = Win, a.Hq = Hin, a.Wq = Win;
    } else if (g.mode == 1) {
        a.Hout = Hin / 2, a.Wout = Win / 2, a.Hq = a.Hout, a.Wq = a.Wout;
    } else {
        a.Hout = 2 * Hin, a.Wout = 2 * Win, a.Hq = Hin, a.Wq = Win;
    }
    a.Nq = B * a.Hq * a.Wq;
    a.fd_hw = FastDiv::make(a.Hq * a.Wq);
    a.fd_w = FastDiv::make(a.Wq);
    LDM_REQUIRE((int64_t)B * Hin * Win * g.cin * 4 < 0x7ff00000LL && (int64_t)B * a.Hout * a.Wout * g.cout * 4 < 0x7ff00000LL,
                "step conv: tensor too large for 32-bit buffer offsets");
    LDM_REQUIRE(s.x && s.w && s.bias, "step conv: null operand");
    LDM_REQUIRE(!s.msolver || (layer == 8 && s.x0_log), "step conv: the multistep update is dec1's and needs its x0 log");
    LDM_REQUIRE((!s.plain && !s.guide_eb) || layer == 8, "step conv: the guided loop's two launches are dec1's");
    LDM_REQUIRE(!s.plain || (s.y && !s.guide_eb), "step conv: dec1's base half is a plain conv into y");
    LDM_REQUIRE(!s.guide_eb || ((s.guide_scale || s.keep_base) && s.xs2 && s.xs2 != s.xs),
                "step conv: guidance needs its scales and second state");
    LDM_REQUIRE(!s.keep_base || (layer == 8 && !s.plain && s.keep_row && (!s.guide_eb || s.guide_eb == s.keep_base)),
                "step conv: the regional keep is dec1's and needs its region and row (e_b leading the region when guided)");
    LDM_REQUIRE(!s.keep_base || (int64_t)a.B * a.Hout * a.Wout * g.cout == s.keep_stride,
                "step conv: the keep region was laid out for another batch or plane than this launch's");
    return 0;
}

static KsWs ks_ws(int layer, int B, int H, int W, int ksv, float* ws) {
    KsWs k;
    if (ksv && ks_row(layer, ksv).ks > 1) {
        k.ws = ws;
        k.ws_floats = step_ws_floats(B, H, W, &k.cnt_floats);
        ks_tiles(layer, B, H, W, k.tiles, k.slab_floats, ksv);
    }
    return k;
}

template <int FLAG, int MODE, int CIN, int COUT, int TM, int TN, int WN, int WK, int NCH, int S, int EPI, int KS = 1>
static int launch_opt(bool on, const UArgs& a, int dtype, hipStream_t st, const KsWs& k = {}) {
    if (on) return launch<MODE, CIN, COUT, TM, TN, WN, WK, NCH, S, EPI | FLAG, KS>(a, dtype, st, k);
    return launch<MODE, CIN, COUT, TM, TN, WN, WK, NCH, S, EPI, KS>(a, dtype, st, k);
}

static int dec1_geo(int ksv, int W, int Wq) {
    if (ksv == 3) return 0;
    if (dec1_thin(W)) return window_taps() ? 1 : 2;
    return window_taps() && Wq % 32 == 0 ? 3 : 4;
}
}

int step_conv(int layer, int B, int H, int W, const StepConv& s, hipStream_t st) {
    using namespace uc;
    const int ksv = s.ws ? ks_form(layer, s.dtype, H, W) : 0;
    UArgs a;
    if (int rc = make_args(layer, B, H, W, s, a)) return rc;
    const KsWs k = ks_ws(layer, B, H, W, ksv, s.ws);
    const int dt = s.dtype;
    const bool win = window_taps();
    const bool pl28 = a.Hin == 2 && a.Win == 8 && plane_taps(), pl416 = a.Hin == 4 && a.Win == 16 && plane_taps();
    int geo = 0;
    auto dec1_ms = [&](auto g) { return dec1_launch<EPI_MSOLVER, decltype(g)::value>(a, dt, st); };
    auto dec1_ddim = [&](auto g) { return dec1_launch<EPI_DDIM, decltype(g)::value>(a, dt, st); };
    if (layer == 8) {
        LDM_REQUIRE(ksv != 3 || (win && a.Wq % 64 == 0), "dec1 (variant 3): 64-column rows");
        geo = dec1_geo(ksv, W, a.Wq);
        if (s.keep_base) return step_dec1_keep(geo, a, s, st);
        if (s.plain || s.guide_eb) return step_dec1_guided(geo, a, s, st);
        LDM_REQUIRE(s.xs && s.coef, "dec1: sampler state, coefficients");
    }
    if (ksv == 3) {
        switch (layer) {
            case 0: LDM_REQUIRE(s.y && win && a.Wq % 64 == 0, "enc1 (variant 3): y, 64-column rows");
                return launch<0, 32, 64, 2, 1, 4, 2, 9, 9, EPI_RELU | EPI_WINDOW, 1>(a, dt, st);
            case 1: LDM_REQUIRE(s.y && s.bcast && win && a.Wq % 32 == 0, "enc2 (variant 3): y, t_emb, 32-column rows");
                return launch<1, 64, 128, 2, 1, 2, 4, 9, 9, EPI_RELU | EPI_BCAST | EPI_WINDOW, 1>(a, dt, st);
            case 2: LDM_REQUIRE(s.y && win && a.Wq % 16 == 0, "enc3 (variant 3): y, 16-column rows");
                return launch<1, 128, 256, 2, 1, 1, 8, 9, 9, EPI_RELU | EPI_WINDOW, 1>(a, dt, st);
            case 6: LDM_REQUIRE(s.y && s.skip && win && a.Wq % 16 == 0, "dec3 (variant 3): y, skip, 16-column rows");
                return launch<2, 256, 128, 1, 1, 1, 16, 9, 9, EPI_RELU | EPI_SKIP | EPI_WINDOW, 1>(a, dt, st);
            case 7: LDM_REQUIRE(s.y && s.skip && win && a.Wq % 32 == 0, "dec2 (variant 3): y, skip, 32-column rows");
                return launch<2, 128, 64, 1, 2, 1, 8, 9, 9, EPI_RELU | EPI_SKIP | EPI_WINDOW, 1>(a, dt, st);
            case 8: return s.msolver ? dec1_ms(std::integral_constant<int, 0>{}) : dec1_ddim(std::integral_constant<int, 0>{});
            case 3: LDM_REQUIRE(s.y && pl416, "enc4 (variant 3): y, 4 x 16 input plane");
                return launch<1, 256, 512, 1, 1, 1, 16, 9, 9, EPI_RELU | EPI_POSB | EPI_PLANE, 1>(a, dt, st);
            case 5: LDM_REQUIRE(s.y && s.skip && pl28, "dec4 (variant 3): y, skip, 2 x 8 plane");
                if (dec4_par())
                    return launch<2, 512, 256, 1, 1, 1, 16, 10, 10, EPI_RELU | EPI_SKIP | EPI_PLANE, kTapClass>(a, dt, st);
                return launch<2, 512, 256, 1, 1, 1, 16, 9, 9, EPI_RELU | EPI_SKIP | EPI_PLANE, 2>(a, dt, st, k);
            default: return fail(2, "step conv: no K-split variant 3 for this layer");
        }
    }
    if (ksv == 2) {
        switch (layer) {
            case 3: LDM_REQUIRE(s.y, "enc4: y");
                return launch_opt<EPI_PLANE, 1, 256, 512, 1, 2, 1, 8, 9, 9, EPI_RELU | EPI_POSB, 2>(pl416, a, dt, st, k);
            case 4: LDM_REQUIRE(s.y, "bottleneck: y");
                return launch_opt<EPI_PLANE, 0, 512, 512, 1, 2, 2, 4, 18, 18, EPI_RELU | EPI_POSB, 4>(pl28, a, dt, st, k);
            case 5: LDM_REQUIRE(s.y && s.skip, "dec4: y, skip");
                return launch_opt<EPI_PLANE, 2, 512, 256, 1, 2, 1, 8, 9, 9, EPI_RELU | EPI_SKIP, 4>(pl28, a, dt, st, k);
            default: return fail(2, "step conv: no K-split variant 2 for this layer");
        }
    }
    if (ksv) {
        switch (layer) {
            case 2: LDM_REQUIRE(s.y, "enc3: y"); return launch<1, 128, 256, 2, 2, 1, 4, 9, 9, EPI_RELU, 2>(a, dt, st, k);
            case 3: LDM_REQUIRE(s.y, "enc4: y");
                return launch_opt<EPI_PLANE, 1, 256, 512, 2, 2, 1, 4, 9, 9, EPI_RELU | EPI_POSB, 4>(pl416, a, dt, st, k);
            case 4: LDM_REQUIRE(s.y, "bottleneck: y");
                return launch_opt<EPI_PLANE, 0, 512, 512, 2, 2, 1, 8, 9, 9, EPI_RELU | EPI_POSB, 4>(pl28, a, dt, st, k);
            case 5: LDM_REQUIRE(s.y && s.skip, "dec4: y, skip");
                return launch_opt<EPI_PLANE, 2, 512, 256, 2, 2, 1, 4, 9, 9, EPI_RELU | EPI_SKIP, 8>(pl28, a, dt, st, k);
            case 6: LDM_REQUIRE(s.y && s.skip, "dec3: y, skip");
                return launch<2, 256, 128, 2, 2, 1, 4, 9, 9, EPI_RELU | EPI_SKIP, 4>(a, dt, st, k);
            default: return fail(2, "step conv: no K-split variant for this layer");
        }
    }
    switch (layer) {
        case 0: LDM_REQUIRE(s.y, "enc1: y");
            return launch_opt<EPI_WINDOW, 0, 32, 64, 2, 1, 4, 1, 18, 18, EPI_RELU>(win && a.Wq % 64 == 0, a, dt, st);
        case 1: LDM_REQUIRE(s.y && s.bcast, "enc2: y, t_emb");
            if (enc2_wide(W)) return launch_opt<EPI_WINDOW, 1, 64, 128, 1, 1, 4, 1, 36, 36, EPI_RELU | EPI_BCAST>(win, a, dt, st);
            return launch_opt<EPI_WINDOW, 1, 64, 128, 2, 2, 1, 4, 9, 9, EPI_RELU | EPI_BCAST>(win && a.Wq % 32 == 0, a, dt, st);
        case 2: LDM_REQUIRE(s.y, "enc3: y");
            if (enc3_thin(W)) return launch_opt<EPI_WINDOW, 1, 128, 256, 1, 1, 2, 2, 36, 36, EPI_RELU>(win, a, dt, st);
            return launch_opt<EPI_WINDOW, 1, 128, 256, 2, 1, 1, 4, 18, 18, EPI_RELU>(win && a.Wq % 16 == 0, a, dt, st);
        case 3: LDM_REQUIRE(s.y, "enc4: y"); return launch<1, 256, 512, 1, 1, 1, 4, 36, 36, EPI_RELU | EPI_POSB>(a, dt, st);
        case 4: LDM_REQUIRE(s.y, "bottleneck: y"); return launch<0, 512, 512, 1, 1, 1, 8, 36, 12, EPI_RELU | EPI_POSB>(a, dt, st);
        case 5: LDM_REQUIRE(s.y && s.skip, "dec4: y, skip");
            return launch<2, 512, 256, 1, 1, 1, 8, 36, 12, EPI_RELU | EPI_SKIP>(a, dt, st);
        case 6: LDM_REQUIRE(s.y && s.skip, "dec3: y, skip");
            return launch_opt<EPI_WINDOW, 2, 256, 128, 1, 1, 1, 4, 36, 36, EPI_RELU | EPI_SKIP>(win && a.Wq % 16 == 0, a, dt, st);
        case 7: LDM_REQUIRE(s.y && s.skip, "dec2: y, skip");
            return launch_opt<EPI_WINDOW, 2, 128, 64, 1, 2, 1, 4, 18, 18, EPI_RELU | EPI_SKIP>(win && a.Wq % 32 == 0, a, dt, st);
        default: return s.msolver ? dec1_visit(geo, dec1_ms) : dec1_visit(geo, dec1_ddim);
    }
}

int step_layout(const float* x, float* y, int B, int C, int HW, bool to_nhwc, hipStream_t st) {
    const int64_t n = (int64_t)B * C * HW;
    const unsigned blocks = (unsigned)((n + 255) / 256);
    if (to_nhwc)
        hipLaunchKernelGGL(uc::nchw_to_nhwc_kernel, dim3(blocks), dim3(256), 0, st, x, y, C, HW, n);
    else
        hipLaunchKernelGGL(uc::nhwc_to_nchw_kernel, dim3(blocks), dim3(256), 0, st, x, y, C, HW, n);
    LDM_CHECK_LAUNCH("layout transpose");
    return 0;
}

}

using namespace ldm;
// ... 107 lines not shown
```

### music-style-transfer-ldm_amd/csrc/uconv_kernel.h

```cpp
#pragma once
#include <algorithm>
#include <type_traits>
#include <utility>

#include "common.h"

#pragma clang fp contract(off)

namespace ldm {
namespace uc {

enum : int { EPI_RELU = 1, EPI_BCAST = 2, EPI_SKIP = 4, EPI_POSB = 8, EPI_DDIM = 16, EPI_PLANE = 32, EPI_WINDOW = 64, EPI_MSOLVER = 128, EPI_GUIDE = 256, EPI_KEEP = 512 };

struct UArgs {
    const float* x;
    const float* w;
    float* y;
    const float* bias;
    const float* bcast;
    const float* skip;
    const float* coef;
    float* xs;
    float* x0_log;
    float* eps_log;
    float eta;
    int32_t B, Hin, Win, Hout, Wout;
    int32_t Hq, Wq, Nq;
    int32_t nMt, nNt, order;
    int32_t xpm, xpn;
    FastDiv fd_hw, fd_w, fd_mt, fd_nt, fd_tiles;
    float* slab;
    int32_t* cnt;
    const float* x0_prev;
};

__host__ __device__ constexpr int tky(int t) { return t / 3; }
__host__ __device__ constexpr int tkx(int t) { return t % 3; }
__host__ __device__ constexpr int tphase(int t) { return (tky(t) != 1 ? 2 : 0) + (tkx(t) != 1 ? 1 : 0); }
__host__ __device__ constexpr int toff(int t) { return (tky(t) == 0 ? 2 : 0) + (tkx(t) == 0 ? 1 : 0); }
constexpr int kTapClass = -1;
__host__ __device__ constexpr int tc_ntap(int TC) { return TC == 1 ? 4 : (TC == 2 ? 5 : 9); }
__host__ __device__ constexpr int tc_tap(int TC, int i) {
    return TC == 1 ? 6 * (i >> 1) + 2 * (i & 1) : (TC == 2 ? (i == 0 ? 1 : (i == 4 ? 7 : i + 2)) : i);
}
__host__ __device__ constexpr int tc_nph(int MODE, int TC) { return MODE != 2 ? 1 : (TC == 1 ? 1 : (TC == 2 ? 3 : 4)); }
template <int MODE, int TC = 0>
__host__ __device__ constexpr int b_src(int st, int S, int i) {
    if (MODE != 2) return i;
    constexpr int CPC = tc_ntap(TC);
    const int c = st * S + i;
    for (int j = 0; j < i; ++j) {
        const int cj = st * S + j;
        if (cj / CPC == c / CPC && toff(tc_tap(TC, cj % CPC)) == toff(tc_tap(TC, c % CPC))) return j;
    }
    return i;
}
__host__ __device__ constexpr int tc_own(int TC) {
    for (int i = 0; i < tc_ntap(TC); ++i)
        if (toff(tc_tap(TC, i)) == 0) return i;
    return -1;
}

#ifndef UCONV_DIAG
#define UCONV_DIAG 0
#endif
#ifndef UCONV_XAUX
#define UCONV_XAUX 0
#endif
#if (UCONV_DIAG & 4)
__device__ unsigned long long g_uconv_stamps[4096][5];
#define UCONV_STAMP(k)                                                                                 \
    do {                                                                                               \
        if (threadIdx.x == 0 && blockIdx.x < 4096u)                                                    \
            g_uconv_stamps[blockIdx.x][k] = ((k) == 0 || (k) == 4) ? __builtin_amdgcn_s_memrealtime() \
                                                                   : __builtin_amdgcn_s_memtime();    \
    } while (0)
#else
#define UCONV_STAMP(k) \
    do {               \
    } while (0)
#endif

template <int B, int E, class F>
__device__ __forceinline__ void static_for(F&& f) {
    if constexpr (B < E) {
        f(std::integral_constant<int, B>{});
        static_for<B + 1, E>(f);
    }
}

template <int MODE, int CIN, int COUT, int TM, int TN, int WN, int WK, int NCH, int S, int EPI, int DT, int KS, int TC = 0>
__device__ __forceinline__ void uconv_body(const UArgs& a, int bid_in) {
    constexpr int NPH = tc_nph(MODE, TC);
    constexpr int NST = NCH / S;
    constexpr int CPC = tc_ntap(TC);
// ... 450 lines not shown
            constexpr int p = k / (TM * TN), mi = (k / TN) % TM, ni = k % TN;
            vv[k] = acc[0][p][mi][ni];
        }
    });
    if constexpr (KS > 1) {
        const int tile = mt + nt * a.nMt;
        const __amdgpu_buffer_rsrc_t sr = __builtin_amdgcn_make_buffer_rsrc(uni_ptr(a.slab), (short)0, 0x7fffffff, 0x00020000);
        auto slab_off = [&](int kk, int f) { return ((((tile * KS + kk) * WN + wn) * NFR + f) * 64 + lane) * 16; };
        static_for<0, NMY>([&](auto kc) {
            constexpr int k = decltype(kc)::value;
            const int f = frag(k);
            if (f < NFR)
                __builtin_amdgcn_raw_buffer_store_b128(__builtin_bit_cast(__attribute__((ext_vector_type(4))) unsigned, vv[k]),
                                                       sr, slab_off(ks, f), 0, 16);
        });
        asm volatile("s_waitcnt vmcnt(0)" ::: "memory");
        __syncthreads();
        int* flag = reinterpret_cast<int*>(smem);
        if (threadIdx.x == 0) {
            const int old = __hip_atomic_fetch_add(a.cnt + tile, 1, __ATOMIC_RELAXED, __HIP_MEMORY_SCOPE_AGENT);
            const int last = old == KS - 1;
            if (last) __hip_atomic_store(a.cnt + tile, 0, __ATOMIC_RELAXED, __HIP_MEMORY_SCOPE_AGENT);
            *flag = last;
        }
        __syncthreads();
        if (!*flag) return;
        static_for<0, NMY>([&](auto kc) {
            constexpr int k = decltype(kc)::value;
            const int f = frag(k);
            const int fc = f < NFR ? f : NFR - 1;
            floatx4 part[KS];
#pragma unroll
            for (int kk = 0; kk < KS; ++kk)
                part[kk] = __builtin_bit_cast(floatx4, __builtin_amdgcn_raw_buffer_load_b128(sr, slab_off(kk, fc), 0, 16));
            floatx4 sum = ks == 0 ? vv[k] : part[0];
#pragma unroll
            for (int kk = 1; kk < KS; ++kk) sum = sum + (kk == ks ? vv[k] : part[kk]);
            vv[k] = sum;
        });
    }
    static_for<0, NMY>([&](auto kc) {
        constexpr int k = decltype(kc)::value;
        const int f = frag(k);
        const floatx4 v = vv[k];
        const Out ot = out_of(f);
        if (!ot.ok) return;
        const floatx4 bias = pre_b[k];
        floatx4 o;
#pragma unroll
        for (int r = 0; r < 4; ++r) {
            float sv = round16(v[r] + bias[r], DT);
            if (EPI & EPI_RELU) sv = sv < 0.f ? 0.f : sv;
            o[r] = sv;
        }
        if constexpr ((EPI & EPI_BCAST) != 0) {
#pragma unroll
            for (int r = 0; r < 4; ++r) o[r] = round16(o[r] + pre_c[k][r], DT);
        }
        if constexpr ((EPI & EPI_SKIP) != 0) {
#pragma unroll
            for (int r = 0; r < 4; ++r) o[r] = round16(o[r] + pre_s[k][r], DT);
        }
        if constexpr ((EPI & EPI_GUIDE) != 0) {
#pragma unroll
            for (int r = 0; r < 4; ++r) o[r] = guide_eps(o[r], pre_g[k][r], pre_gs[k]);
        }
        if constexpr ((EPI & EPI_MSOLVER) != 0) {
            const floatx4 xv = pre_s[k];
            floatx4 xn;
            const bool hp = a.x0_prev != nullptr;
            const size_t hw = (size_t)a.Hout * a.Wout;
            const size_t lbase = ((size_t)ot.b * COUT + ot.m) * hw + (size_t)ot.oy * a.Wout + ot.ox;
#pragma unroll
            for (int r = 0; r < 4; ++r) {
                float x0;
                xn[r] = msolver_update(xv[r], o[r], a.coef, hp, hp ? pre_h[k][r] : 0.f, x0);
                a.x0_log[lbase + r * hw] = x0;
                if (a.eps_log) a.eps_log[lbase + r * hw] = o[r];
            }
            if constexpr ((EPI & EPI_KEEP) != 0) {
#pragma unroll
                for (int r = 0; r < 4; ++r) xn[r] = keep_blend(xn[r], pre_kz[k][r], pre_kn[k][r], pre_kw[k], pre_ka, pre_kb);
            }
            *reinterpret_cast<floatx4*>(a.xs + (size_t)ot.pix * COUT + ot.m) = xn;
            if constexpr ((EPI & EPI_GUIDE) != 0) *reinterpret_cast<floatx4*>(a.y + (size_t)ot.pix * COUT + ot.m) = xn;
        } else if constexpr ((EPI & EPI_DDIM) != 0) {
            const floatx4 xv = pre_s[k];
            floatx4 xn;
            const size_t hw = (size_t)a.Hout * a.Wout;
            const size_t lbase = ((size_t)ot.b * COUT + ot.m) * hw + (size_t)ot.oy * a.Wout + ot.ox;
#pragma unroll
            for (int r = 0; r < 4; ++r) {
                float x0;
                xn[r] = ddim_update(xv[r], o[r], a.coef, a.eta, x0);
                if (a.x0_log) a.x0_log[lbase + r * hw] = x0;
                if (a.eps_log) a.eps_log[lbase + r * hw] = o[r];
            }
            if constexpr ((EPI & EPI_KEEP) != 0) {
#pragma unroll
                for (int r = 0; r < 4; ++r) xn[r] = keep_blend(xn[r], pre_kz[k][r], pre_kn[k][r], pre_kw[k], pre_ka, pre_kb);
            }
            *reinterpret_cast<floatx4*>(a.xs + (size_t)ot.pix * COUT + ot.m) = xn;
            if constexpr ((EPI & EPI_GUIDE) != 0) *reinterpret_cast<floatx4*>(a.y + (size_t)ot.pix * COUT + ot.m) = xn;
        } else {
            *reinterpret_cast<floatx4*>(a.y + (size_t)ot.pix * COUT + ot.m) = o;
        }
    });
    UCONV_STAMP(4);
}

template <int MODE, int CIN, int COUT, int TM, int TN, int WN, int WK, int NCH, int S, int EPI, int DT, int KS = 1>
__global__ __launch_bounds__(64 * WN * WK) __attribute__((amdgpu_waves_per_eu((WN * WK + 3) / 4, (WN * WK + 3) / 4)))
void uconv_kernel(UArgs a) {
    if constexpr (KS == kTapClass) {
        const int tiles = a.nMt * a.nNt;
        if ((int)blockIdx.x < tiles)
            uconv_body<MODE, CIN, COUT, TM, TN, WN, WK, NCH / 5 * 4, S / 5 * 4, EPI, DT, 1, 1>(a, blockIdx.x);
        else
            uconv_body<MODE, CIN, COUT, TM, TN, WN, WK, NCH, S, EPI, DT, 1, 2>(a, (int)blockIdx.x - tiles);
    } else {
        uconv_body<MODE, CIN, COUT, TM, TN, WN, WK, NCH, S, EPI, DT, KS>(a, blockIdx.x);
    }
}

bool xcd_grid();

struct KsWs {
    float* ws = nullptr;
    int64_t tiles = 0, slab_floats = 0, cnt_floats = 0, ws_floats = 0;
};

template <int CIN, int COUT, int TM, int TN, int WN, int KS>
static int set_grid(UArgs& a, const KsWs& k) {
    constexpr int bm = 16 * TM, bn = 16 * TN * WN;
    a.nMt = COUT / bm;
    a.nNt = (a.Nq + bn - 1) / bn;
    const int64_t wbytes = (int64_t)9 * CIN * COUT * 4, xbytes = (int64_t)a.B * a.Hin * a.Win * CIN * 4;
    a.order = wbytes > xbytes ? 0 : 1;
    if (xcd_grid() && ((int64_t)a.nMt * a.nNt) % 8 == 0) {
        int64_t best = -1;
        for (int pm = 1; pm <= 8; pm *= 2) {
            const int pn = 8 / pm;
            if (a.nMt % pm || a.nNt % pn) continue;
            const int64_t est = pn * wbytes + pm * xbytes;
            if (best < 0 || est < best) best = est, a.xpm = pm, a.xpn = pn;
        }
        if (best >= 0) a.order = 2;
    }
    a.fd_mt = FastDiv::make(a.nMt);
    a.fd_nt = FastDiv::make(a.nNt);
    a.fd_tiles = FastDiv::make(a.nMt * a.nNt);
    if constexpr (KS > 1) {
        LDM_REQUIRE(k.ws && k.tiles == (int64_t)a.nMt * a.nNt && k.ws_floats >= k.cnt_floats + k.slab_floats &&
                        (k.cnt_floats + k.slab_floats) * 4 < 0x7fffffffLL,
                    "step conv: split-K workspace geometry");
        a.cnt = reinterpret_cast<int32_t*>(k.ws);
        a.slab = k.ws + k.cnt_floats;
    }
    return 0;
}

template <int MODE, int CIN, int COUT, int TM, int TN, int WN, int WK, int NCH, int S, int EPI, int DT, int KS>
static int launch_dt(const UArgs& a, hipStream_t st) {
    constexpr int NPH = KS == kTapClass ? tc_nph(MODE, 2) : tc_nph(MODE, 0);
    constexpr int NCC = KS == kTapClass ? S / 5 : S / 9;
    const int blocks = a.nMt * a.nNt * (KS == kTapClass ? 2 : KS);
    size_t lds = std::max<size_t>(WK > 1 ? (size_t)WK * WN * NPH * TM * TN * 64 * 16 : 0, KS > 1 ? 16 : 0);
    if constexpr ((EPI & EPI_PLANE) != 0)
        lds = (WK > 1 ? (size_t)WK * WN * NPH * TM * TN * 64 * 16 : 0) + (size_t)WN * WK * NCC * TN * (MODE == 1 ? 4096 : 1024);
    if constexpr ((EPI & EPI_WINDOW) != 0) {
        constexpr int WR = MODE == 2 ? 2 : 3;
        constexpr int WC = MODE == 0 ? 16 * TN + 2 : (MODE == 1 ? 32 * TN + 1 : 16 * TN + 1);
        lds = (WK > 1 ? (size_t)WK * WN * NPH * TM * TN * 64 * 16 : 0) + (size_t)WN * WK * NCC * WR * WC * 64;
    }
    auto kfn = uconv_kernel<MODE, CIN, COUT, TM, TN, WN, WK, NCH, S, EPI, DT, KS>;
    if (lds > 64 * 1024) {
        static bool opted = false;
        if (!opted) {
            LDM_HIP_TRY(hipFuncSetAttribute((const void*)kfn, hipFuncAttributeMaxDynamicSharedMemorySize, 160 * 1024));
            opted = true;
        }
    }
    hipLaunchKernelGGL(kfn, dim3((unsigned)blocks), dim3(64 * WN * WK), lds, st, a);
    LDM_CHECK_LAUNCH("uconv_kernel");
    return 0;
}

template <int MODE, int CIN, int COUT, int TM, int TN, int WN, int WK, int NCH, int S, int EPI, int KS = 1>
static int launch(UArgs a, int dtype, hipStream_t st, const KsWs& k = {}) {
    if (int rc = set_grid<CIN, COUT, TM, TN, WN, KS>(a, k)) return rc;
    switch (dtype) {
        case LDM_DT_F32: return launch_dt<MODE, CIN, COUT, TM, TN, WN, WK, NCH, S, EPI, 0, KS>(a, st);
        case LDM_DT_F16: return launch_dt<MODE, CIN, COUT, TM, TN, WN, WK, NCH, S, EPI, 1, KS>(a, st);
        case LDM_DT_BF16: return launch_dt<MODE, CIN, COUT, TM, TN, WN, WK, NCH, S, EPI, 2, KS>(a, st);
        default: return fail(2, "step conv: unknown operand precision");
    }
}

struct Dec1Geo {
    int tm, tn, wn, wk, nch, s, flag;
};
constexpr Dec1Geo kDec1Geo[5] = {
    {1, 2, 2, 4, 9, 9, EPI_WINDOW},
    {1, 2, 2, 2, 18, 18, EPI_WINDOW},
    {1, 2, 2, 2, 18, 18, 0},
    {2, 2, 1, 4, 9, 9, EPI_WINDOW},
    {2, 2, 1, 4, 9, 9, 0},
};
template <int EPI, int GEO>
static int dec1_launch(const UArgs& a, int dtype, hipStream_t st) {
    constexpr Dec1Geo g = kDec1Geo[GEO];
    return launch<0, 64, 32, g.tm, g.tn, g.wn, g.wk, g.nch, g.s, EPI | g.flag>(a, dtype, st);
}
template <class F>
static int dec1_visit(int geo, F&& f) {
    switch (geo) {
        case 0: return f(std::integral_constant<int, 0>{});
        case 1: return f(std::integral_constant<int, 1>{});
        case 2: return f(std::integral_constant<int, 2>{});
        case 3: return f(std::integral_constant<int, 3>{});
        case 4: return f(std::integral_constant<int, 4>{});
        default: return fail(2, "step conv: unknown dec1 geometry");
    }
}

int step_dec1_guided(int geo, const UArgs& a, const StepConv& s, hipStream_t st);
int step_dec1_keep(int geo, const UArgs& a, const StepConv& s, hipStream_t st);

}
}
```

### music-style-transfer-ldm_amd/csrc/unet.hip

```cpp
#include <cmath>
#include <cstdlib>

#include "common.h"

namespace ldm {

static int layer_desc(const ldm_unet_shape& s, int layer, ldm_conv_desc& d) {
    LDM_REQUIRE(s.B > 0 && s.C > 0 && s.nf > 0, "unet: bad shape");
    LDM_REQUIRE(s.H % 8 == 0 && s.W % 8 == 0 && s.H >= 8 && s.W >= 8,
                "unet: latent H and W must be multiples of 8 (skip connections, model.py:221-227)");
    LDM_REQUIRE(s.nf * 4 == 256, "unet: CrossAttention dims are fixed at 512/256 (model.py:184-185) -> num_filters 64");
    d = ldm_conv_desc{};
    d.B = s.B;
    const int nf = s.nf;
    const int H = s.H, W = s.W;
    auto conv = [&](int cin, int hin, int win, int cout, int stride) {
        d.Cin = cin;
        d.Hin = hin;
        d.Win = win;
        d.Cout = cout;
        d.kh = d.kw = 3;
        d.stride = stride;
        d.pad = 1;
        d.out_pad = 0;
// ... 206 lines not shown
    LDM_TRY(conv_forward_ex(d, plan, d2 + fuse->gB * HW * s.nf, w.conv_w[8], eb, fuse->eb, convws, st));
    EpiArgs ep = eb;
    fuse_epi(ep, *fuse);
    ep.guide_eb = fuse->eb;
    ep.guide_scale = fuse->gscale;
    ep.ddim_x2 = fuse->x + fuse->gB * HW * s.C;
    return conv_forward_ex(d, plan, d2, w.conv_w[8], ep, nullptr, convws, st);
}

static int style_kv(const ldm_unet_shape& s, const ldm_unet_weights& w, const float* s5, const float* s6,
                    const UNetWs& ws, hipStream_t st) {
    LDM_TRY(conv_call(s, ws.convws, 10, w.ca_plan_kv[0], s5, w.ca_wkv[0], w.ca_bkv[0], 0, nullptr, nullptr, ws.kv2, st));
    LDM_TRY(conv_call(s, ws.convws, 13, w.ca_plan_kv[1], s6, w.ca_wkv[1], w.ca_bkv[1], 0, nullptr, nullptr, ws.kv1, st));
    return 0;
}

static int style_kv_tokens(const ldm_unet_shape& s, const ldm_unet_weights& w, int j, const float* sm, int S, float* kv,
                           hipStream_t st) {
    ldm_conv_desc d;
    LDM_TRY(layer_desc(s, 10 + 3 * j, d));
    d.Win = d.Wout = S;
    const ldm_conv_plan& bound = w.ca_plan_kv[j];
    LDM_REQUIRE(bound.kind >= 0 && bound.kind <= 2, "style mix: the K/V projection's plan must be a direct or fp32 MFMA plan");
    ldm_conv_plan plan;
    LDM_TRY(ldm_conv_make_plan_forced(&d, bound.kind, bound.tm, bound.tn, bound.wk, 1, &plan));
    LDM_REQUIRE(plan.packed_floats == bound.packed_floats && plan.ws_floats == 0, "style mix: K/V projection plan mismatch");
    EpiArgs ep{};
    ep.bias = w.ca_bkv[j];
    ep.act = 0;
    return conv_forward_ex(d, plan, sm, w.ca_wkv[j], ep, kv, nullptr, st);
}

static int unet_forward(const ldm_unet_shape& s, const ldm_unet_weights& w, const float* z, const void* t,
                        int t_is_float, const float* s5, const float* s6, float* out, const UNetWs& ws,
                        hipStream_t st, const float* temb_pre = nullptr, const DdimFuse* fuse = nullptr,
                        bool kv_ready = false) {
    const int HW = s.H * s.W;
    const int L2 = HW / 16, L1 = HW / 64;
    const float* temb = temb_pre;
    if (!temb) {
        LDM_TRY(ldm_time_mlp_forward(t, t_is_float, s.B, 128, w.t_freqs, w.t_w1, w.t_b1, w.t_w2, w.t_b2, ws.temb, st));
        temb = ws.temb;
    }
    LDM_TRY(conv_call(s, ws.convws, 0, w.conv_plan[0], z, w.conv_w[0], w.conv_b[0], LDM_ACT_RELU, nullptr, nullptr, ws.z1, st));
    LDM_TRY(conv_call(s, ws.convws, 1, w.conv_plan[1], ws.z1, w.conv_w[1], w.conv_b[1], LDM_ACT_RELU, temb, nullptr, ws.z2, st));
    LDM_TRY(conv_call(s, ws.convws, 2, w.conv_plan[2], ws.z2, w.conv_w[2], w.conv_b[2], LDM_ACT_RELU, nullptr, nullptr, ws.z3, st));
    if (!kv_ready) LDM_TRY(style_kv(s, w, s5, s6, ws, st));
    LDM_TRY(conv_call(s, ws.convws, 9, w.ca_plan_q[0], ws.z3, w.ca_wq[0], w.ca_bq[0], 0, nullptr, nullptr, ws.q2, st));
    LDM_TRY(attention_core_ex(ws.q2, ws.kv2, ws.a2, s.B, 256, 4, L2, L2, (float)std::sqrt(1.0 / 64.0), true, st));
    LDM_TRY(conv_call(s, ws.convws, 11, w.ca_plan_o[0], ws.a2, w.ca_wo[0], w.ca_bo[0], 0, nullptr, nullptr, ws.c2, st));
    LDM_TRY(conv_call(s, ws.convws, 3, w.conv_plan[3], ws.c2, w.conv_w[3], w.conv_b[3], LDM_ACT_RELU, nullptr, nullptr, ws.z4, st));
    LDM_TRY(conv_call(s, ws.convws, 12, w.ca_plan_q[1], ws.z4, w.ca_wq[1], w.ca_bq[1], 0, nullptr, nullptr, ws.q1, st));
    LDM_TRY(attention_core_ex(ws.q1, ws.kv1, ws.a1, s.B, 512, 4, L1, L1, (float)std::sqrt(1.0 / 128.0), true, st));
    LDM_TRY(conv_call(s, ws.convws, 14, w.ca_plan_o[1], ws.a1, w.ca_wo[1], w.ca_bo[1], 0, nullptr, nullptr, ws.c1, st));
    LDM_TRY(conv_call(s, ws.convws, 4, w.conv_plan[4], ws.c1, w.conv_w[4], w.conv_b[4], LDM_ACT_RELU, nullptr, nullptr, ws.zb, st));
    LDM_TRY(conv_call(s, ws.convws, 5, w.conv_plan[5], ws.zb, w.conv_w[5], w.conv_b[5], LDM_ACT_RELU, nullptr, ws.z3, ws.d4, st));
    LDM_TRY(conv_call(s, ws.convws, 6, w.conv_plan[6], ws.d4, w.conv_w[6], w.conv_b[6], LDM_ACT_RELU, nullptr, ws.z2, ws.d3, st));
    LDM_TRY(conv_call(s, ws.convws, 7, w.conv_plan[7], ws.d3, w.conv_w[7], w.conv_b[7], LDM_ACT_RELU, nullptr, ws.z1, ws.d2, st));
    LDM_TRY(dec1_call(s, w, ws.d2, ws.convws, out, st, fuse));
    return 0;
}

static int unet_forward_folded(const ldm_unet_shape& s, const ldm_unet_weights& w, const float* z, const UNetWs& ws,
                               hipStream_t st, const float* temb, const DdimFuse* fuse, int S5, int S6) {
    const int HW = s.H * s.W;
    const int L2 = HW / 16, L1 = HW / 64;
    LDM_TRY(conv_call(s, ws.convws, 0, w.conv_plan[0], z, w.conv_w[0], w.conv_b[0], LDM_ACT_RELU, nullptr, nullptr, ws.z1, st));
    LDM_TRY(conv_call(s, ws.convws, 1, w.conv_plan[1], ws.z1, w.conv_w[1], w.conv_b[1], LDM_ACT_RELU, temb, nullptr, ws.z2, st));
    LDM_TRY(conv_call(s, ws.convws, 2, w.conv_plan[2], ws.z2, w.conv_w[2], w.conv_b[2], LDM_ACT_RELU, nullptr, nullptr, ws.z3, st));
    LDM_TRY(attention_folded_keys(ws.z3, ws.kv2, ws.kf2, ws.bf2, nullptr, ws.a2, s.B, 256, 4, L2, S5, st));
    LDM_TRY(conv_call(s, ws.convws, 3, w.conv_plan[3], ws.a2, w.fold_w[0], nullptr, LDM_ACT_RELU, nullptr, nullptr, ws.z4, st,
                      nullptr, w.fold_pb[0]));
    LDM_TRY(attention_folded_keys(ws.z4, ws.kv1, ws.kf1, ws.bf1, nullptr, ws.a1, s.B, 512, 4, L1, S6, st));
    LDM_TRY(conv_call(s, ws.convws, 4, w.conv_plan[4], ws.a1, w.fold_w[1], nullptr, LDM_ACT_RELU, nullptr, nullptr, ws.zb, st,
                      nullptr, w.fold_pb[1]));
    LDM_TRY(conv_call(s, ws.convws, 5, w.conv_plan[5], ws.zb, w.conv_w[5], w.conv_b[5], LDM_ACT_RELU, nullptr, ws.z3, ws.d4, st));
    LDM_TRY(conv_call(s, ws.convws, 6, w.conv_plan[6], ws.d4, w.conv_w[6], w.conv_b[6], LDM_ACT_RELU, nullptr, ws.z2, ws.d3, st));
    LDM_TRY(conv_call(s, ws.convws, 7, w.conv_plan[7], ws.d3, w.conv_w[7], w.conv_b[7], LDM_ACT_RELU, nullptr, ws.z1, ws.d2, st));
    LDM_TRY(dec1_call(s, w, ws.d2, ws.convws, nullptr, st, fuse));
    return 0;
}

static int unet_step_kernels(const ldm_unet_shape& s, const ldm_unet_weights& w, const UNetWs& ws, hipStream_t st,
                             const float* temb, const DdimFuse& fuse, int S5, int S6, bool bfold) {
    const int HW = s.H * s.W;
    const int L2 = HW / 16, L1 = HW / 64;
    const float* xin[9] = {ws.xs, ws.z1, ws.z2, ws.a2, ws.a1, ws.zb, ws.d4, ws.d3, ws.d2};
    float* yout[9] = {ws.z1, ws.z2, ws.z3, ws.z4, ws.zb, ws.d4, ws.d3, ws.d2, nullptr};
    const float* bias[9] = {w.conv_b[0], w.conv_b[1], w.conv_b[2], w.step_pb[0], w.step_pb[1], w.conv_b[5], w.conv_b[6],
                            w.conv_b[7], w.conv_b[8]};
    const float* skip[9] = {nullptr, nullptr, nullptr, nullptr, nullptr, ws.z3, ws.z2, ws.z1, nullptr};
    StepConv c[9];
    for (int l = 0; l < 9; ++l) {
        c[l] = StepConv{};
        c[l].x = xin[l];
        c[l].w = w.step_w[l];
        c[l].y = yout[l];
        c[l].bias = bias[l];
        c[l].skip = skip[l];
        c[l].dtype = w.step_dtype;
        c[l].ws = ws.uks;
    }
    c[1].bcast = temb;
    c[8].coef = fuse.coef;
    c[8].eta = fuse.eta;
    c[8].xs = ws.xs;
    c[8].x0_log = fuse.x0_log;
    c[8].eps_log = fuse.eps_log;
    c[8].msolver = fuse.msolver;
    c[8].x0_prev = fuse.x0_prev;
    if (fuse.kw && !fuse.gB) c[8].keep_base = fuse.kbase, c[8].keep_row = fuse.krow, c[8].keep_stride = fuse.kstride;
    auto dec1_guided = [&]() -> int {
        const int Bh = fuse.gB;
        StepConv cb = c[8];
        cb.x = ws.d2 + (size_t)Bh * HW * s.nf;
        cb.y = fuse.eb;
        cb.plain = 1;
        cb.coef = nullptr, cb.xs = nullptr, cb.x0_log = nullptr, cb.eps_log = nullptr, cb.msolver = 0, cb.x0_prev = nullptr;
        LDM_TRY(step_conv(8, Bh, s.H, s.W, cb, st));
        StepConv ct = c[8];
        ct.guide_eb = fuse.eb;
        ct.guide_scale = fuse.gscale;
        ct.xs2 = ws.xs + (size_t)Bh * HW * s.C;
        if (fuse.kw)
            ct.keep_base = fuse.kbase, ct.keep_row = fuse.krow, ct.keep_stride = fuse.kstride, ct.guide_scale = nullptr;
        return step_conv(8, Bh, s.H, s.W, ct, st);
    };
    auto run = [&](int l0, int l1) -> int {
        for (int l = l0; l <= l1; ++l) {
            if (l == 8 && fuse.gB) LDM_TRY(dec1_guided());
            else LDM_TRY(step_conv(l, s.B, s.H, s.W, c[l], st));
        }
        return 0;
    };
    LDM_TRY(run(0, 2));
    LDM_TRY(attention_folded_keys(ws.z3, ws.kv2, ws.kf2, ws.bf2, nullptr, ws.a2, s.B, 256, 4, L2, S5, st));
    LDM_TRY(run(3, 3));
    if (bfold) {
        if (ca1_probs_own()) LDM_TRY(ca1_probs(ws.z4, ws.kf1, ws.bf1, ws.p1, s.B, st));
        else LDM_TRY(attention_folded_probs(ws.z4, ws.kf1, ws.bf1, ws.p1, s.B, 512, 4, L1, L1, st));
        LDM_TRY(bneck_pv(ws.ubn, ws.p1, w.step_pb[1], ws.zb, s.B, w.step_dtype, st));
        return run(5, 8);
    }
    LDM_TRY(attention_folded_keys(ws.z4, ws.kv1, ws.kf1, ws.bf1, nullptr, ws.a1, s.B, 512, 4, L1, S6, st));
    return run(4, 8);
}

}

using namespace ldm;

extern "C" int ldm_step_layer_forms(int32_t* ks_layers) {
    LDM_REQUIRE(ks_layers, "step_layer_forms: null argument");
    *ks_layers = step_ks_mask();
    return 0;
}

extern "C" int ldm_unet_layer_desc(const ldm_unet_shape* s, int32_t layer, ldm_conv_desc* d) {
    LDM_REQUIRE(s && d, "unet_layer_desc: null argument");
    return layer_desc(*s, layer, *d);
}

extern "C" int64_t ldm_unet_workspace_floats(const ldm_unet_shape* s, const ldm_unet_weights* w) {
    if (!s) return -1;
    return carve(*s, w, nullptr).total;
}

extern "C" int ldm_unet_make_plans(const ldm_unet_shape* s, ldm_unet_weights* w) {
    LDM_REQUIRE(s && w, "unet_make_plans: null argument");
    for (int l = 0; l < 15; ++l) {
        ldm_conv_desc d;
        LDM_TRY(layer_desc(*s, l, d));
        ldm_conv_plan* p = l < 9 ? &w->conv_plan[l]
                                 : ((l - 9) % 3 == 0 ? &w->ca_plan_q[(l - 9) / 3]
                                                     : ((l - 9) % 3 == 1 ? &w->ca_plan_kv[(l - 9) / 3]
                                                                         : &w->ca_plan_o[(l - 9) / 3]));
        LDM_TRY(ldm_conv_make_plan(&d, p));
    }
    return 0;
}

extern "C" int ldm_unet_forward(const ldm_unet_shape* s, const ldm_unet_weights* w, const float* z, const void* t,
                                int32_t t_is_float, const float* s5, const float* s6, float* out, float* workspace,
                                void* stream) {
    LDM_REQUIRE(s && w && z && t && s5 && s6 && out && workspace, "unet_forward: null argument");
    UNetWs ws = carve(*s, w, workspace);
    return unet_forward(*s, *w, z, t, t_is_float, s5, s6, out, ws, (hipStream_t)stream);
}

struct Guide {
    const float *s5_base, *s6_base, *key_bias5_base, *key_bias6_base, *scale;
};
struct Keep {
    const float *z0, *n0, *w, *coef;
};
static int64_t keep_region_floats(const ldm_unet_shape& s, int32_t nsteps, bool guided) {
    const int64_t HW = (int64_t)s.H * s.W, dense = s.B * s.C * HW;
    return (guided ? 3 : 2) * dense + s.B * HW + (int64_t)nsteps * (2 + (guided ? s.B : 0));
}
__global__ __launch_bounds__(256) void keep_rows_kernel(const float* __restrict__ coef, const float* __restrict__ scale,
                                                        float* __restrict__ rows, int B, int64_t n) {
    const int64_t i = (int64_t)blockIdx.x * blockDim.x + threadIdx.x;
    if (i >= n) return;
    const int rl = 2 + (scale ? B : 0);
    const int64_t r = i / rl;
    const int j = (int)(i - r * rl);
    rows[i] = j < 2 ? coef[2 * r + j] : scale[j - 2];
}

__global__ __launch_bounds__(256) void concat_halves_kernel(const float* __restrict__ a, const float* __restrict__ b,
                                                            float* __restrict__ out, int64_t rowlen, int64_t n) {
    const int64_t i = (int64_t)blockIdx.x * blockDim.x + threadIdx.x;
    if (i >= n) return;
    const int64_t r = i / (2 * rowlen), j = i - r * 2 * rowlen;
    const float* src = j < rowlen ? a : b;
    out[i] = src ? src[r * rowlen + (j < rowlen ? j : j - rowlen)] : 0.f;
}
static int concat_halves(const float* a, const float* b, float* out, int64_t rows, int64_t rowlen, hipStream_t st) {
    const int64_t n = rows * 2 * rowlen;
    hipLaunchKernelGGL(concat_halves_kernel, dim3((unsigned)((n + 255) / 256)), dim3(256), 0, st, a, b, out, rowlen, n);
    LDM_CHECK_LAUNCH("concat_halves_kernel");
    return 0;
}

static int sample_loop(const ldm_unet_shape* sc, const ldm_unet_weights* w, float* x, const float* s5, const float* s6,
                       const int64_t* t_table, const float* coef_table, int32_t nsteps, float eta, float* x0_logs,
                       float* eps_logs, int64_t log_step_stride, float* workspace, void* stream, bool msolver,
                       int32_t S5 = 0, int32_t S6 = 0, const float* key_bias5 = nullptr,
                       const float* key_bias6 = nullptr, const Guide* g = nullptr, const Keep* kp = nullptr) {
    ldm_unet_shape sh = *sc;
    if (g) sh.B = 2 * sc->B;
    const ldm_unet_shape* s = &sh;
    const int L2 = s->H * s->W / 16, L1 = s->H * s->W / 64;
    if (S5 <= 0) S5 = L2;
    if (S6 <= 0) S6 = L1;
    const bool gbias = g && (key_bias5 || key_bias6 || g->key_bias5_base || g->key_bias6_base);
    const bool mix = S5 != L2 || S6 != L1 || key_bias5 || key_bias6 || gbias;
    LDM_REQUIRE(!mix || w->use_fold, "style mix: the reverse loop attends over several references only with the "
                                     "folded cross-attentions (use_fold)");
    UNetWs ws = carve(*s, w, workspace, S5, S6, g != nullptr);
    float* temb_all = workspace + ws.total;
    const int64_t dense = (int64_t)sc->B * s->C * s->H * s->W;
    LDM_REQUIRE(log_step_stride == 0 || log_step_stride >= dense, "ddim_sample: log stride smaller than a step");
    const int64_t n = log_step_stride ? log_step_stride : dense;
    hipStream_t st = (hipStream_t)stream;
    const size_t cw = msolver ? 8 : 4;
    if (g) {
        float* temb_b = temb_all + (size_t)nsteps * s->B * 128;
        LDM_TRY(ldm_time_mlp_forward(t_table, 0, nsteps * sc->B, 128, w->t_freqs, w->t_w1, w->t_b1, w->t_w2, w->t_b2,
                                     temb_b, st));
        LDM_TRY(concat_halves(temb_b, temb_b, temb_all, nsteps, (int64_t)sc->B * 128, st));
        LDM_TRY(concat_halves(s5, g->s5_base, ws.s5cat, 1, (int64_t)sc->B * 256 * S5, st));
        LDM_TRY(concat_halves(s6, g->s6_base, ws.s6cat, 1, (int64_t)sc->B * 512 * S6, st));
        s5 = ws.s5cat, s6 = ws.s6cat;
        if (key_bias5 || g->key_bias5_base) {
            LDM_TRY(concat_halves(key_bias5, g->key_bias5_base, ws.kb5cat, 1, (int64_t)sc->B * S5, st));
            key_bias5 = ws.kb5cat;
        }
        if (key_bias6 || g->key_bias6_base) {
            LDM_TRY(concat_halves(key_bias6, g->key_bias6_base, ws.kb6cat, 1, (int64_t)sc->B * S6, st));
            key_bias6 = ws.kb6cat;
        }
    } else {
        LDM_TRY(ldm_time_mlp_forward(t_table, 0, nsteps * s->B, 128, w->t_freqs, w->t_w1, w->t_b1, w->t_w2, w->t_b2,
                                     temb_all, st));
    }
    if (S5 == L2 && S6 == L1) {
        LDM_TRY(style_kv(*s, *w, s5, s6, ws, st));
    } else {
        LDM_TRY(style_kv_tokens(*s, *w, 0, s5, S5, ws.kv2, st));
        LDM_TRY(style_kv_tokens(*s, *w, 1, s6, S6, ws.kv1, st));
    }
    const int HW = s->H * s->W;
    auto make_fuse = [&](int i, float* xstate) {
        DdimFuse fuse{coef_table + cw * (size_t)i, eta, xstate, x0_logs ? x0_logs + (size_t)i * n : nullptr,
                      eps_logs ? eps_logs + (size_t)i * n : nullptr, msolver,
                      msolver && i > 0 ? x0_logs + (size_t)(i - 1) * n : nullptr};
        if (g) fuse.gB = sc->B, fuse.eb = ws.eb, fuse.gscale = g->scale;
        if (kp) fuse.kz0 = kp->z0, fuse.kn0 = kp->n0, fuse.kw = kp->w, fuse.kcoef = kp->coef + 2 * (size_t)i;
        return fuse;
    };
    if (w->use_fold) {
        LDM_REQUIRE(w->ca_wq_raw[0] && w->ca_wq_raw[1] && w->fold_w[0] && w->fold_w[1] && w->fold_pb[0] && w->fold_pb[1],
                    "ddim_sample: use_fold needs the folded weights");
        LDM_TRY(attention_fold_keys_bias(ws.kv2, w->ca_wq_raw[0], w->ca_bq[0], s->B, 256, 4, S5,
                                         (float)std::sqrt(1.0 / 64.0), key_bias5, ws.kf2, ws.bf2, st));
        LDM_TRY(attention_fold_keys_bias(ws.kv1, w->ca_wq_raw[1], w->ca_bq[1], s->B, 512, 4, S6,
                                         (float)std::sqrt(1.0 / 128.0), key_bias6, ws.kf1, ws.bf1, st));
        if (w->use_step) {
            LDM_REQUIRE(s->C == 32 && s->nf == 64, "ddim_sample: the step kernels are built for latent 32 / 64 filters");
            for (int l = 0; l < 9; ++l) LDM_REQUIRE(w->step_w[l], "ddim_sample: use_step needs the step weights");
            LDM_REQUIRE(w->step_pb[0] && w->step_pb[1], "ddim_sample: use_step needs the folded biases");
            LDM_REQUIRE(w->step_dtype >= LDM_DT_F32 && w->step_dtype <= LDM_DT_BF16, "ddim_sample: step_dtype");
            const bool bfold = use_bneck_fold(*s, w) && S6 == L1 && !key_bias6;
            if (bfold) LDM_TRY(bneck_fold_values(w->step_bneck_w, ws.kv1, ws.ubn, s->B, st));
            LDM_TRY(step_layout(x, ws.xs, sc->B, s->C, HW, true, st));
            if (g) LDM_TRY(step_layout(x, ws.xs + dense, sc->B, s->C, HW, true, st));
            float* kreg = temb_all + (size_t)nsteps * (g ? 3 : 1) * sc->B * 128;
            const int krl = 2 + (g ? sc->B : 0);
            float* krows = kreg + (g ? 3 : 2) * dense + (int64_t)sc->B * HW;
            if (kp) {
                float* kz = kreg + (g ? dense : 0);
                LDM_TRY(step_layout(kp->z0, kz, sc->B, s->C, HW, true, st));
                LDM_TRY(step_layout(kp->n0, kz + dense, sc->B, s->C, HW, true, st));
                LDM_HIP_TRY(hipMemcpyAsync(kz + 2 * dense, kp->w, (size_t)sc->B * HW * 4, hipMemcpyDeviceToDevice, st));
                const int64_t nr = (int64_t)nsteps * krl;
                hipLaunchKernelGGL(keep_rows_kernel, dim3((unsigned)((nr + 255) / 256)), dim3(256), 0, st, kp->coef,
                                   g ? g->scale : nullptr, krows, sc->B, nr);
                LDM_CHECK_LAUNCH("keep_rows_kernel");
            }
            for (int i = 0; i < nsteps; ++i) {
                DdimFuse fuse = make_fuse(i, ws.xs);
                if (kp) {
                    fuse.kbase = kreg, fuse.krow = krows + (size_t)i * krl, fuse.kstride = dense;
                    if (g) fuse.eb = kreg;
                }
                LDM_TRY(unet_step_kernels(*s, *w, ws, st, temb_all + (size_t)i * s->B * 128, fuse, S5, S6, bfold));
            }
            return step_layout(ws.xs, x, sc->B, s->C, HW, false, st);
        }
    }
    float* xstate = x;
    if (g) {
        LDM_TRY(concat_halves(x, x, ws.xs, 1, dense, st));
        xstate = ws.xs;
    }
    for (int i = 0; i < nsteps; ++i) {
        const DdimFuse fuse = make_fuse(i, xstate);
        if (w->use_fold)
            LDM_TRY(unet_forward_folded(*s, *w, xstate, ws, st, temb_all + (size_t)i * s->B * 128, &fuse, S5, S6));
        else
            LDM_TRY(unet_forward(*s, *w, xstate, t_table + (size_t)i * sc->B, 0, s5, s6, nullptr, ws, st,
                                 temb_all + (size_t)i * s->B * 128, &fuse, true));
    }
    if (g) LDM_HIP_TRY(hipMemcpyAsync(x, ws.xs, (size_t)dense * 4, hipMemcpyDeviceToDevice, st));
    return 0;
}

static bool guidance_on(const ldm_sample_args& a) { return a.s5_base || a.s6_base || a.guide_scale; }
static bool keep_on(const ldm_sample_args& a) { return a.z0 || a.n0 || a.keep || a.keep_coef; }

extern "C" int64_t ldm_sample_workspace_floats(const ldm_unet_shape* s, const ldm_unet_weights* w, const ldm_sample_args* a) {
    if (!s || !a || a->nsteps < 0 || a->S5 < 0 || a->S6 < 0 || s->B <= 0) return -1;
    const bool guided = guidance_on(*a);
    ldm_unet_shape sh = *s;
    if (guided) sh.B = 2 * s->B;
    const int64_t n = carve(sh, w, nullptr, a->S5, a->S6, guided).total + (int64_t)a->nsteps * (guided ? 3 : 1) * s->B * 128;
    return keep_on(*a) ? n + keep_region_floats(*s, a->nsteps, guided) : n;
}

static int workspace_extent_ok(int64_t need, const float* workspace, void* stream) {
    hipStreamCaptureStatus cs = hipStreamCaptureStatusNone;
    if (hipStreamIsCapturing((hipStream_t)stream, &cs) != hipSuccess) {
        (void)hipGetLastError();
        return 0;
    }
    if (cs != hipStreamCaptureStatusNone) return 0;
    hipDeviceptr_t base = nullptr;
    size_t size = 0;
    if (hipMemGetAddressRange(&base, &size, (hipDeviceptr_t)workspace) != hipSuccess || !base) {
        (void)hipGetLastError();
        return 0;
    }
    LDM_REQUIRE(need > 0, "sample: bad shape for the workspace size");
    const int64_t avail = (int64_t)(((const char*)base + size) - (const char*)workspace);
    LDM_REQUIRE(avail >= need * 4, "sample: the workspace's allocation ends before the size ldm_sample_workspace_floats "
                                   "gives for these arguments (was it sized for another configuration?)");
    return 0;
}

extern "C" int ldm_sample(const ldm_unet_shape* s, const ldm_unet_weights* w, const ldm_sample_args* a) {
    LDM_REQUIRE(s && w && a, "sample: null argument");
    LDM_REQUIRE(a->solver == LDM_SOLVER_DDIM || a->solver == LDM_SOLVER_MULTISTEP, "sample: unknown solver");
    const bool msolver = a->solver == LDM_SOLVER_MULTISTEP;
    LDM_REQUIRE(a->x && a->s5 && a->s6 && a->t_table && a->coef_table && a->workspace && (!msolver || a->x0_logs),
                "sample: null argument");
    LDM_REQUIRE(a->nsteps >= 0, "sample: negative step count");
    LDM_REQUIRE(a->S5 >= 0 && a->S6 >= 0, "sample: negative key count");
    const bool guided = guidance_on(*a), keep = keep_on(*a);
    if (guided) {
        LDM_REQUIRE(a->s5_base && a->s6_base, "guided sample: null base style maps");
        LDM_REQUIRE(a->guide_scale, "guided sample: null guidance scale");
        LDM_REQUIRE(s->B > 0 && s->B <= (1 << 20), "guided sample: bad batch");
    } else {
        LDM_REQUIRE(!a->key_bias5_base && !a->key_bias6_base, "sample: base key biases without a base style");
    }
    LDM_REQUIRE(!keep || (a->z0 && a->n0 && a->keep && a->keep_coef),
                "sample: z0, n0, keep and keep_coef go together (one is NULL)");
    if (a->nsteps == 0) return 0;
    LDM_TRY(workspace_extent_ok(ldm_sample_workspace_floats(s, w, a), a->workspace, a->stream));
    const Guide g{a->s5_base, a->s6_base, a->key_bias5_base, a->key_bias6_base, a->guide_scale};
    const Keep k{a->z0, a->n0, a->keep, a->keep_coef};
    return sample_loop(s, w, a->x, a->s5, a->s6, a->t_table, a->coef_table, a->nsteps, msolver ? 0.f : a->eta, a->x0_logs,
                       a->eps_logs, a->log_step_stride, a->workspace, a->stream, msolver, a->S5, a->S6, a->key_bias5,
                       a->key_bias6, guided ? &g : nullptr, keep ? &k : nullptr);
}
```

### music-style-transfer-ldm_amd/ldm_amd/_lib.py

```python
import ctypes
import os

import torch

PKG_ROOT = os.path.dirname(os.path.dirname(os.path.abspath(__file__)))
LIB_PATH = os.environ.get("LDM_AMD_LIB", os.path.join(PKG_ROOT, "lib", "libldm_amd.so"))

c_int32 = ctypes.c_int32
c_int64 = ctypes.c_int64
c_float = ctypes.c_float
c_vp = ctypes.c_void_p
c_fp = ctypes.c_void_p


class ConvDesc(ctypes.Structure):
    _fields_ = [(n, c_int32) for n in
                ("B", "Cin", "Hin", "Win", "Cout", "Hout", "Wout", "kh", "kw", "stride", "pad", "out_pad", "transposed",
                 "layout")]

    def key(self):
        return tuple(getattr(self, f[0]) for f in self._fields_)


class Epilogue(ctypes.Structure):
# ... 75 lines not shown
    "ldm_step_layer_forms": (c_int32, [c_vp]),
    "ldm_step_dec1_ddim": (c_int32, [c_int32, c_int32, c_int32, c_fp, c_fp, c_fp, c_fp, c_float, c_fp, c_fp, c_fp,
                                     c_int32, c_vp]),
    "ldm_step_dec1_msolver": (c_int32, [c_int32, c_int32, c_int32, c_fp, c_fp, c_fp, c_fp, c_fp, c_fp, c_fp, c_fp,
                                        c_int32, c_vp]),
    "ldm_step_conv_ws": (c_int32, [c_int32, c_int32, c_int32, c_int32, c_fp, c_fp, c_fp, c_fp, c_fp, c_fp, c_int32,
                                   c_fp, c_vp]),
    "ldm_mel_quantize": (c_int32, [c_fp, c_fp, c_int64, ctypes.c_float, c_vp]),
    "ldm_mel_dequantize": (c_int32, [c_fp, c_fp, c_int64, ctypes.c_float, c_vp]),
    "ldm_u8_to_unit": (c_int32, [c_fp, c_fp, c_int64, c_vp]),
    "ldm_stft_table_floats": (c_int64, [c_int32]),
    "ldm_stft_fill_tables": (c_int32, [c_int32, c_vp]),
    "ldm_stft": (c_int32, [c_fp, c_int32, c_int64, c_int32, c_int32, c_fp, c_fp, c_fp, c_int32, c_vp]),
    "ldm_istft": (c_int32, [c_fp, c_fp, c_fp, c_int32, c_int32, c_int64, c_int32, c_int32, c_fp, c_vp]),
    "ldm_griffinlim_workspace": (c_int64, [c_int32, c_int32, c_int32]),
    "ldm_griffinlim": (c_int32, [c_fp, c_fp, c_fp, c_int32, c_int32, c_int64, c_int32, c_int32, c_int32, c_float,
                                 c_fp, c_fp, c_vp]),
    "ldm_mel_project": (c_int32, [c_fp, c_fp, c_vp, c_fp, c_int32, c_int32, c_int32, c_int32, c_vp]),
    "ldm_power_to_db": (c_int32, [c_fp, c_fp, c_int32, c_int64, c_float, c_float, c_fp, c_vp]),
    "ldm_db_to_power": (c_int32, [c_fp, c_fp, c_int64, c_vp]),
    "ldm_mel_invert": (c_int32, [c_fp, c_fp, c_fp, c_fp, c_vp, c_float, c_int32, c_int32, c_fp, c_fp, c_int32,
                                 c_int32, c_int32, c_int32, c_vp]),
    "ldm_resample_out_len": (c_int64, [c_int64, c_int32, c_int32]),
    "ldm_resample_f32": (c_int32, [c_fp, c_int32, c_int64, c_fp, c_int32, c_int32, c_int32, c_fp, c_vp]),
    "ldm_resample_pcm16": (c_int32, [c_vp, c_int64, c_int32, c_fp, c_int32, c_int32, c_int32, c_fp, c_vp]),
    "ldm_trim_workspace_floats": (c_int64, [c_int32, c_int64, c_int32]),
    "ldm_trim_bounds": (c_int32, [c_fp, c_int32, c_int64, c_int32, c_int32, c_float, c_fp, c_vp, c_vp]),
    "ldm_mel_window_count": (c_int64, [c_int64, c_int32, c_int32]),
    "ldm_mel_windows": (c_int32, [c_fp, c_int32, c_int64, c_int32, c_int32, c_float, c_float, c_float, c_fp, c_fp,
                                  c_vp]),
    "ldm_mel_stitch": (c_int32, [c_fp, c_fp, c_int32, c_int32, c_int32, c_int32, c_int64, c_float, c_fp, c_fp, c_vp]),
    "ldm_batchnorm_train": (c_int32, [c_fp, c_int32, c_int32, c_int32, c_fp, c_fp, c_fp, c_fp, c_float, c_float,
                                      c_int32, c_fp, c_fp, c_fp, c_vp]),
    "ldm_batchnorm_train_out": (c_int32, [c_fp, c_fp, c_int32, c_int32, c_int32, c_fp, c_fp, c_fp, c_fp, c_float,
                                          c_float, c_int32, c_fp, c_fp, c_fp, c_vp]),
    "ldm_batchnorm_apply_out": (c_int32, [c_fp, c_fp, c_int32, c_int32, c_int32, c_vp, ctypes.c_double, c_fp, c_fp,
                                          c_fp, c_fp, c_float, c_float, c_int32, c_fp, c_fp, c_vp]),
    "ldm_maxpool2x2": (c_int32, [c_fp, c_fp, c_int32, c_int32, c_int32, c_int32, c_vp]),
    "ldm_std_mse_workspace_floats": (c_int64, [c_int32, c_int64]),
    "ldm_std_mse_moments": (c_int32, [c_fp, c_fp, c_int32, c_int64, c_vp, c_fp, c_vp]),
    "ldm_std_mse_accumulate": (c_int32, [c_vp, c_int32, c_int64, ctypes.c_double, ctypes.c_double, c_vp, c_fp, c_vp]),
    "ldm_batchnorm_stats": (c_int32, [c_fp, c_int32, c_int32, c_int32, c_vp, c_fp, c_vp]),
    "ldm_batchnorm_apply": (c_int32, [c_fp, c_int32, c_int32, c_int32, c_vp, ctypes.c_double, c_fp, c_fp, c_fp, c_fp,
                                      c_float, c_float, c_int32, c_fp, c_fp, c_vp]),
    "ldm_batchnorm_eval": (c_int32, [c_fp, c_fp, c_int32, c_int32, c_int32, c_fp, c_fp, c_fp, c_fp, c_float, c_int32,
                                     c_vp]),
    "ldm_activation": (c_int32, [c_fp, c_fp, c_int64, c_int32, c_vp]),
    "ldm_sinusoid_embed": (c_int32, [c_vp, c_int32, c_int32, c_int32, c_fp, c_fp, c_vp]),
    "ldm_time_mlp_forward": (c_int32, [c_vp, c_int32, c_int32, c_int32, c_fp, c_fp, c_fp, c_fp, c_fp, c_fp, c_vp]),
    "ldm_attention_core": (c_int32, [c_fp, c_fp, c_fp, c_int32, c_int32, c_int32, c_int32, c_int32, c_float, c_vp]),
    "ldm_attention_flash_supported": (c_int32, [c_int32, c_int32]),
    "ldm_attention_forward_lse": (c_int32, [c_fp, c_fp, c_fp, c_fp, c_int32, c_int32, c_int32, c_int32, c_int32,
                                            c_float, c_vp]),
    "ldm_attention_backward_flash": (c_int32, [c_fp, c_fp, c_fp, c_fp, c_fp, c_fp, c_fp, c_fp, c_int32, c_int32,
                                               c_int32, c_int32, c_int32, c_float, c_vp]),
    "ldm_pack_job_bytes": (c_int64, []),
    "ldm_pack_many_prepare": (c_int32, [ctypes.POINTER(ConvDesc), ctypes.POINTER(ConvPlan), ctypes.POINTER(c_vp),
                                        ctypes.POINTER(c_vp), c_int32, c_vp, ctypes.POINTER(c_int64)]),
    "ldm_pack_many": (c_int32, [c_vp, c_int32, c_int64, c_vp]),
    "ldm_im2col": (c_int32, [c_fp, c_int32, c_int32, c_int32, c_int32, c_int32, c_int32, c_int32, c_int32, c_int32,
                             c_fp, c_fp, c_int32, c_int32, c_fp, c_vp]),
    "ldm_col2im": (c_int32, [c_fp, c_int32, c_int32, c_int32, c_int32, c_int32, c_int32, c_int32, c_int32, c_int32,
                             c_fp, c_int32, c_int32, c_fp, c_vp]),
    "ldm_maxpool3s2": (c_int32, [c_fp, c_fp, c_int32, c_int32, c_int32, c_int32, c_vp]),
    "ldm_maxpool3s2_backward": (c_int32, [c_fp, c_fp, c_fp, c_int32, c_int32, c_int32, c_int32, c_vp]),
    "ldm_lpips_layer": (c_int32, [c_fp, c_fp, c_fp, c_int32, c_int32, c_int32, c_fp, c_fp, c_vp]),
    "ldm_lpips_layer_backward": (c_int32, [c_fp, c_fp, c_fp, c_fp, c_int32, c_int32, c_int32, c_int32, c_int32, c_fp,
                                           c_vp]),
    "ldm_attention_fold_keys": (c_int32, [c_fp, c_fp, c_fp, c_int32, c_int32, c_int32, c_int32, c_float, c_fp, c_fp,
                                          c_vp]),
    "ldm_attention_folded": (c_int32, [c_fp, c_fp, c_fp, c_fp, c_fp, c_int32, c_int32, c_int32, c_int32, c_int32,
                                       c_vp]),
    "ldm_fold_conv_proj": (c_int32, [ctypes.POINTER(ConvDesc), c_fp, c_fp, c_fp, c_fp, c_int32, c_fp, c_fp, c_vp]),
    "ldm_attention_folded_probs": (c_int32, [c_fp, c_fp, c_fp, c_fp, c_int32, c_int32, c_int32, c_int32, c_int32,
                                             c_vp]),
    "ldm_bneck_fold_supported": (c_int32, [c_int32, c_int32, c_int32]),
    "ldm_bneck_fold_values": (c_int32, [c_fp, c_fp, c_fp, c_int32, c_vp]),
    "ldm_bneck_pv": (c_int32, [c_fp, c_fp, c_fp, c_fp, c_int32, c_int32, c_vp]),
    "ldm_ca1_probs": (c_int32, [c_fp, c_fp, c_fp, c_fp, c_int32, c_vp]),
    "ldm_ca1_probs_form": (c_int32, []),
    "ldm_set_cin1_packed": (c_int32, [c_int32]),
    "ldm_set_cin1_s1": (c_int32, [c_int32]),
    "ldm_set_flash_split": (c_int32, [c_int32]),
    "ldm_q_sample": (c_int32, [c_fp, c_fp, c_fp, c_int32, c_vp, c_fp, c_int32, c_int64, c_vp]),
    "ldm_predict_start": (c_int32, [c_fp, c_fp, c_fp, c_int32, c_vp, c_fp, c_int32, c_int64, c_vp]),
    "ldm_sched_backward": (c_int32, [c_int32, c_fp, c_fp, c_int32, c_vp, c_fp, c_fp, c_int32, c_int64, c_vp]),
    "ldm_ddim_step":(c_int32, [c_fp, c_fp, c_fp, c_float, c_fp, c_fp, c_int64, c_vp]),
    "ldm_msolver_step": (c_int32, [c_fp, c_fp, c_fp, c_fp, c_fp, c_fp, c_int64, c_vp]),
    "ldm_loss_forward": (c_int32, [c_int32, c_fp, c_fp, c_int64, c_vp, c_fp, c_vp]),
    "ldm_loss_backward": (c_int32, [c_int32, c_fp, c_fp, c_int64, c_fp, c_fp, c_fp, c_vp]),
    "ldm_unet_workspace_floats": (c_int64, [ctypes.POINTER(UNetShape), ctypes.POINTER(UNetWeights)]),
    "ldm_unet_make_plans": (c_int32, [ctypes.POINTER(UNetShape), ctypes.POINTER(UNetWeights)]),
    "ldm_unet_layer_desc": (c_int32, [ctypes.POINTER(UNetShape), c_int32, ctypes.POINTER(ConvDesc)]),
    "ldm_unet_forward": (c_int32, [ctypes.POINTER(UNetShape), ctypes.POINTER(UNetWeights), c_fp, c_vp, c_int32,
                                   c_fp, c_fp, c_fp, c_fp, c_vp]),
    "ldm_sample_workspace_floats": (c_int64, [ctypes.POINTER(UNetShape), ctypes.POINTER(UNetWeights),
                                              ctypes.POINTER(SampleArgs)]),
    "ldm_sample": (c_int32, [ctypes.POINTER(UNetShape), ctypes.POINTER(UNetWeights), ctypes.POINTER(SampleArgs)]),
    "ldm_attention_folded_keys": (c_int32, [c_fp, c_fp, c_fp, c_fp, c_fp, c_fp, c_int32, c_int32, c_int32, c_int32,
                                            c_int32, c_vp]),
    "ldm_attention_fold_keys_bias": (c_int32, [c_fp, c_fp, c_fp, c_int32, c_int32, c_int32, c_int32, c_float, c_fp,
                                               c_fp, c_fp, c_vp]),
    "ldm_guide_eps": (c_int32, [c_fp, c_fp, c_fp, c_int64, c_int32, c_fp, c_vp]),
    "ldm_keep_blend": (c_int32, [c_fp, c_fp, c_fp, c_fp, c_fp, c_int32, c_int32, c_int64, c_vp]),
    "ldm_conv_tiled_plan": (c_int32, [ctypes.POINTER(ConvDesc), c_int32, ctypes.POINTER(ConvPlan)]),
    "ldm_conv_sconv_plan": (c_int32, [ctypes.POINTER(ConvDesc), c_int32, ctypes.POINTER(ConvPlan)]),
    "ldm_conv_storage16": (c_int32, [ctypes.POINTER(ConvDesc), ctypes.POINTER(ConvPlan)]),
    "ldm_conv_wgrad_storage16": (c_int32, [ctypes.POINTER(ConvDesc)]),
    "ldm_batchnorm_stats_code": (c_int32, [c_fp, c_int32, c_int32, c_int32, c_int32, c_vp, c_fp, c_vp]),
    "ldm_conv_wgrad_workspace_floats": (c_int64, [ctypes.POINTER(ConvDesc)]),
    "ldm_conv_backward_weight_dt": (c_int32, [ctypes.POINTER(ConvDesc), c_fp, c_fp, c_fp, c_int32, c_fp, c_int32, c_vp]),
    "ldm_conv_backward_weight": (c_int32, [ctypes.POINTER(ConvDesc), c_fp, c_fp, c_fp, c_int32, c_fp, c_vp]),
    "ldm_act_backward_defer": (c_int32, [c_fp, c_fp, c_fp, c_int32, c_int32, c_int32, c_int32, c_fp, c_fp, c_fp, c_vp,
                                         c_vp]),
    "ldm_act_partial_floats": (c_int64, [c_int32, c_int32, c_int32]),
    "ldm_batchnorm_backward_dxsum_defer": (c_int32, [c_fp, c_fp, c_fp, c_fp, c_fp, c_fp, c_fp, c_int32, c_int32, c_int32,
                                                     c_int32, c_fp, c_fp, c_fp, c_fp, c_vp, c_vp, c_fp, c_vp]),
    "ldm_bn_dxsum_partial_floats": (c_int64, [c_int32, c_int32, c_int32]),
    "ldm_conv_backward_weight_defer": (c_int32, [c_vp, c_fp, c_fp, c_fp, c_int32, c_fp, c_int32, c_vp, c_vp]),
    "ldm_wgrad_reduce_many": (c_int32, [c_vp, c_int32, c_vp]),
    "ldm_act_finalize_many": (c_int32, [c_vp, c_int32, c_vp]),
    "ldm_act_backward": (c_int32, [c_fp, c_fp, c_fp, c_int32, c_int32, c_int32, c_int32, c_fp, c_fp, c_fp, c_fp,
                                   c_vp]),
    "ldm_batchnorm_backward": (c_int32, [c_fp, c_fp, c_fp, c_fp, c_fp, c_fp, c_fp, c_int32, c_int32, c_int32,
                                         c_int32, c_fp, c_fp, c_fp, c_fp, c_vp]),
    "ldm_batchnorm_backward_dxsum": (c_int32, [c_fp, c_fp, c_fp, c_fp, c_fp, c_fp, c_fp, c_int32, c_int32, c_int32,
                                               c_int32, c_fp, c_fp, c_fp, c_fp, c_fp, c_vp]),
    "ldm_batchnorm_backward_reduce": (c_int32, [c_fp, c_fp, c_fp, c_fp, c_fp, c_fp, c_fp, c_int32, c_int32, c_int32,
                                                c_int32, c_vp, c_fp, c_fp, c_fp, c_vp]),
    "ldm_batchnorm_backward_apply": (c_int32, [c_fp, c_fp, c_fp, c_fp, c_fp, c_fp, c_fp, c_int32, c_int32, c_int32,
                                               c_int32, c_vp, ctypes.c_double, c_fp, c_vp]),
    "ldm_attention_backward": (c_int32, [c_fp, c_fp, c_fp, c_fp, c_fp, c_int32, c_int32, c_int32, c_int32, c_int32,
                                         c_float, c_vp]),
    "ldm_attention_backward_supported": (c_int32, [c_int32, c_int32, c_int32, c_int32]),
    "ldm_unscale_check": (c_int32, [c_vp, c_vp, c_vp, c_int32, c_int32, c_fp, c_vp, c_vp]),
    "ldm_adam_step": (c_int32, [c_vp, c_vp, c_vp, c_int32, c_int32, ctypes.c_double, ctypes.c_double,
                                ctypes.c_double, ctypes.c_double, ctypes.c_double, c_int32, c_int32, c_vp, c_vp]),
    "ldm_adam_step_dev": (c_int32, [c_vp, c_vp, c_vp, c_int32, c_int32, ctypes.c_double, ctypes.c_double,
                                    ctypes.c_double, ctypes.c_double, ctypes.c_double, c_int32, c_fp, c_vp, c_fp,
                                    c_vp]),
    "ldm_update_scale": (c_int32, [c_fp, c_vp, c_vp, c_float, c_float, c_int32, c_vp]),
}

TENSOR_SLOT_WORDS = 5

_LIB = None


class LDMError(RuntimeError):
    pass


def load(path=None):
    global _LIB
    if _LIB is not None and path is None:
        return _LIB
    p = path or LIB_PATH
    if not os.path.exists(p):
        raise LDMError(f"libldm_amd.so not found at {p}: build it with `make -C music-style-transfer-ldm_amd/csrc` "
                       "(or __graft_entry__.build()); there is no CPU fallback")
    lib = ctypes.CDLL(p)
    for name, (res, args) in SIGNATURES.items():
        fn = getattr(lib, name)
        fn.restype = res
        fn.argtypes = args
    if path is None:
# ... 21 lines not shown
```

Baseline: 14610 steps/s.

## Fuse DDIM sample-loop prologue kernels into combined launches and write final x directly

Merges the two cross-attention K/V 1x1 projection convs, the time-embedding MLP for all steps, and the NCHW->NHWC layout of x into one block-partitioned prologue kernel. The two key-folding kernels become a second combined launch. The last step kernel now writes x directly, so the final layout conversion back is skipped. This cuts launch count and serial small kernels before the 49-step loop, at the cost of a heterogeneous kernel whose register and LDS footprint is set by its largest branch.

```diff
diff --git a/include/ldm_capi.h b/include/ldm_capi.h
--- a/include/ldm_capi.h
+++ b/include/ldm_capi.h
@@ -125,6 +125,7 @@
 int ldm_set_cin1_packed(int on);
 int ldm_set_cin1_s1(int on);
 int ldm_set_flash_split(int on);
+int ldm_set_loop_prologue(int on);
 int ldm_fold_conv_proj(const ldm_conv_desc* d, const float* w_conv, const float* b_conv, const float* w_proj,
                        const float* b_proj, int32_t Cmid, float* w_out, float* pos_bias_out, void* stream);
 int ldm_attention_core(const float* q, const float* kv, float* out, int32_t B, int32_t E, int32_t heads,
@@ -211,6 +212,9 @@
 
 int64_t ldm_sample_workspace_floats(const ldm_unet_shape* s, const ldm_unet_weights* w, const ldm_sample_args* a);
 int ldm_sample(const ldm_unet_shape* s, const ldm_unet_weights* w, const ldm_sample_args* a);
+int ldm_loop_prologue(const ldm_unet_shape* s, const ldm_unet_weights* w, const float* x, const float* s5,
+                      const float* s6, const int64_t* t_table, int32_t nsteps, float* workspace, void* stream,
+                      int64_t* off, int32_t* stages);
 int ldm_guide_eps(const float* e_t, const float* e_b, const float* scale, int64_t per_sample, int32_t B, float* out,
                   void* stream);
 int ldm_keep_blend(float* x, const float* z0, const float* n0, const float* keep, const float* coef, int32_t B, int32_t C,
diff --git a/music-style-transfer-ldm_amd/csrc/common.h b/music-style-transfer-ldm_amd/csrc/common.h
--- a/music-style-transfer-ldm_amd/csrc/common.h
+++ b/music-style-transfer-ldm_amd/csrc/common.h
@@ -192,6 +192,14 @@
                           float* out, int32_t B, int32_t E, int32_t heads, int32_t L, int32_t S, hipStream_t st);
 int attention_fold_keys_bias(const float* kv, const float* wq, const float* bq, int32_t B, int32_t E, int32_t heads,
                              int32_t S, float scale, const float* key_bias, float* kf, float* bf, hipStream_t st);
+int loop_prologue_a(const ldm_conv_desc& d5, const ldm_conv_plan& p5, const float* s5, const float* w5, const float* b5,
+                    float* kv2, const ldm_conv_desc& d6, const ldm_conv_plan& p6, const float* s6, const float* w6,
+                    const float* b6, float* kv1, const int64_t* t, int nrows, const float* freqs, const float* w1,
+                    const float* b1, const float* w2, const float* b2, float* temb, const float* x, float* xs, int B,
+                    int C, int HW, hipStream_t st, bool& used);
+int attention_fold_keys_pair(const float* kv2, const float* wq2, const float* bq2, int32_t S2, float scale2, float* kf2,
+                             float* bf2, const float* kv1, const float* wq1, const float* bq1, int32_t S1, float scale1,
+                             float* kf1, float* bf1, int32_t B, hipStream_t st, bool& used);
 bool bneck_fold_supported(int B, int H, int W);
 int bneck_fold_values(const float* wf, const float* kv, float* u, int B, hipStream_t st);
 int bneck_pv(const float* u, const float* p, const float* pb, float* y, int B, int dtype, hipStream_t st);
@@ -219,6 +227,7 @@
     const float* keep_row;
     int64_t keep_stride;
     float* ws;
+    float* x_out;
 };
 int step_conv(int layer, int B, int H, int W, const StepConv& s, hipStream_t st);
 int64_t step_ws_floats(int B, int H, int W, int64_t* cnt_floats = nullptr);
diff --git a/music-style-transfer-ldm_amd/csrc/conv.hip b/music-style-transfer-ldm_amd/csrc/conv.hip
--- a/music-style-transfer-ldm_amd/csrc/conv.hip
+++ b/music-style-transfer-ldm_amd/csrc/conv.hip
@@ -5,6 +5,7 @@
 
 #include "common.h"
 #include "conv_epi.h"
+#include "loop_prologue.h"
 
 #pragma clang fp contract(off)
 
@@ -184,7 +185,7 @@
 }
 
 template <int KIND, int TM, int TN, int WK, int NT, bool NHWC, int DT>
-__global__ __launch_bounds__(64 * WK) void conv_mfma_kernel(ConvArgs a) {
+__device__ __forceinline__ void conv_mfma_body(const ConvArgs& a, const int orig, const int nwg) {
     LDM_STAMP(0);
     using MF = Mfma<KIND>;
     constexpr bool PH4 = NT == 4;
@@ -200,7 +201,6 @@
     const int Nq = a.B * HqWq;
     int ph, mt, nt, ksp;
     {
-        const int nwg = gridDim.x, orig = blockIdx.x;
         const int rest = a.fd_nn.div(orig);
         const int nt0 = orig - rest * a.fd_nn.d;
         const int ph0 = PH4 ? a.fd_nm.div(rest) : 0;
@@ -563,6 +563,11 @@
         epilogue_store(a, m, b, qyy * a.pt.osy + ph_ry, qxx * a.pt.osy + ph_rx, v);
     }
     LDM_STAMP(5);
+}
+
+template <int KIND, int TM, int TN, int WK, int NT, bool NHWC, int DT>
+__global__ __launch_bounds__(64 * WK) void conv_mfma_kernel(ConvArgs a) {
+    conv_mfma_body<KIND, TM, TN, WK, NT, NHWC, DT>(a, blockIdx.x, gridDim.x);
 }
 #if (LDM_DIAG & 4)
 extern "C" int ldm_debug_stamps(unsigned long long* host, int nblocks) {
@@ -1578,6 +1583,103 @@
     return in_nhwc ? launch_mfma<2, true, 0>(a, p, Nq, st) : launch_mfma<2, false, 0>(a, p, Nq, st);
 }
 
+struct PrologueAArgs {
+    ConvArgs c5, c6;
+    const void* t;
+    const float *freqs, *w1, *b1, *w2, *b2;
+    float* temb;
+    const float* x;
+    float* xs;
+    int64_t n;
+    int32_t nrows, C, HW;
+    int32_t e5, e6, et;
+};
+static_assert(sizeof(PrologueAArgs) <= 4096, "the prologue's arguments must fit the kernarg segment");
+
+constexpr int kProWK = 8;
+constexpr int kProRows = 4;
+constexpr int kProLayout = 2048;
+
+template <int K5, int K6>
+__global__ __launch_bounds__(64 * kProWK) void loop_prologue_a_kernel(PrologueAArgs p) {
+    extern __shared__ __attribute__((aligned(16))) float smem[];
+    const int blk = blockIdx.x;
+    if (blk < p.e5) {
+        conv_mfma_body<K5, 1, 1, kProWK, 1, false, 0>(p.c5, blk, p.e5);
+    } else if (blk < p.e6) {
+        conv_mfma_body<K6, 1, 1, kProWK, 1, false, 0>(p.c6, blk - p.e5, p.e6 - p.e5);
+    } else if (blk < p.et) {
+        const int grp = threadIdx.x >> 7, i = threadIdx.x & 127;
+        const int row = (blk - p.e6) * kProRows + grp;
+        float* sm = smem + grp * 256;
+        time_mlp_body(p.t, 0, 128, p.freqs, p.w1, p.b1, p.w2, p.b2, p.temb, sm, sm + 128, row, i, row < p.nrows);
+    } else {
+        const int64_t first = (int64_t)(blk - p.et) * kProLayout + threadIdx.x;
+#pragma unroll
+        for (int k = 0; k < kProLayout / (64 * kProWK); ++k)
+            nchw_to_nhwc_body(p.x, p.xs, p.C, p.HW, p.n, first + k * (64 * kProWK));
+    }
+}
+
+static bool prologue_plan_ok(const ldm_conv_desc& d, const ldm_conv_plan& p) {
+    return (p.kind == 1 || p.kind == 2) && p.tm == 1 && p.tn == 1 && p.wk == kProWK && p.ks == 1 && !p.balance &&
+           p.ws_floats == 0 && d.layout == 0 && d.kh == 1 && d.kw == 1 && !d.transposed &&
+           plan_ok(d, p.kind, p.tm, p.tn, p.wk, p.ks);
+}
+
+static int prologue_conv_args(const ldm_conv_desc& d, const ldm_conv_plan& p, const float* x, const float* w,
+                              const float* bias, float* y, ConvArgs& a, int& blocks, size_t& lds) {
+    if (int rc = make_args(d, p, a)) return rc;
+    LDM_REQUIRE(a.pt.nphase == 1 && a.pt.ntap[0] == 1 && a.ks == 1, "loop prologue: the K/V projection is a 1x1 conv");
+    LDM_REQUIRE((int64_t)d.B * d.Cin * d.Hin * d.Win * 4 < 0x7ff00000LL && p.packed_floats * 4 < 0x7ff00000LL &&
+                    (int64_t)d.B * d.Cout * d.Hout * d.Wout * 4 < 0x7ff00000LL,
+                "loop prologue: tensor too large for 32-bit buffer offsets");
+    a.x = x;
+    a.w = w;
+    a.y = y;
+    a.ep = EpiArgs{};
+    a.ep.bias = bias;
+    a.ep.act = 0;
+    const int tile = tile_m(p.kind);
+    const int64_t Nq = (int64_t)d.B * a.pt.Hq * a.pt.Wq;
+    blocks = (int)(((Nq + tile - 1) / tile) * ((a.Cout + tile - 1) / tile));
+    lds = (size_t)p.wk * tile * (tile + 1) * sizeof(float);
+    return 0;
+}
+
+int loop_prologue_a(const ldm_conv_desc& d5, const ldm_conv_plan& p5, const float* s5, const float* w5, const float* b5,
+                    float* kv2, const ldm_conv_desc& d6, const ldm_conv_plan& p6, const float* s6, const float* w6,
+                    const float* b6, float* kv1, const int64_t* t, int nrows, const float* freqs, const float* w1,
+                    const float* b1, const float* w2, const float* b2, float* temb, const float* x, float* xs, int B,
+                    int C, int HW, hipStream_t st, bool& used) {
+    used = false;
+    if (!prologue_plan_ok(d5, p5) || !prologue_plan_ok(d6, p6)) return 0;
+    LDM_REQUIRE(s5 && w5 && kv2 && s6 && w6 && kv1 && t && freqs && w1 && b1 && w2 && b2 && temb && x && xs && nrows > 0 &&
+                    B > 0 && C > 0 && HW > 0,
+                "loop prologue: bad argument");
+    PrologueAArgs p{};
+    int nb5 = 0, nb6 = 0;
+    size_t lds5 = 0, lds6 = 0;
+    if (int rc = prologue_conv_args(d5, p5, s5, w5, b5, kv2, p.c5, nb5, lds5)) return rc;
+    if (int rc = prologue_conv_args(d6, p6, s6, w6, b6, kv1, p.c6, nb6, lds6)) return rc;
+    p.t = t, p.freqs = freqs, p.w1 = w1, p.b1 = b1, p.w2 = w2, p.b2 = b2, p.temb = temb;
+    p.x = x, p.xs = xs, p.n = (int64_t)B * C * HW, p.nrows = nrows, p.C = C, p.HW = HW;
+    const int64_t nbt = (nrows + kProRows - 1) / kProRows, nbl = (p.n + kProLayout - 1) / kProLayout;
+    LDM_REQUIRE((int64_t)nb5 + nb6 + nbt + nbl < 0x7fffffffLL, "loop prologue: too many blocks");
+    p.e5 = nb5, p.e6 = p.e5 + nb6, p.et = p.e6 + (int)nbt;
+    const dim3 grid((unsigned)(p.et + nbl)), block(64 * kProWK);
+    const size_t lds = std::max(std::max(lds5, lds6), (size_t)kProRows * 256 * sizeof(float));
+    switch (p5.kind * 10 + p6.kind) {
+        case 11: hipLaunchKernelGGL((loop_prologue_a_kernel<1, 1>), grid, block, lds, st, p); break;
+        case 12: hipLaunchKernelGGL((loop_prologue_a_kernel<1, 2>), grid, block, lds, st, p); break;
+        case 21: hipLaunchKernelGGL((loop_prologue_a_kernel<2, 1>), grid, block, lds, st, p); break;
+        default: hipLaunchKernelGGL((loop_prologue_a_kernel<2, 2>), grid, block, lds, st, p); break;
+    }
+    LDM_CHECK_LAUNCH("loop_prologue_a_kernel");
+    used = true;
+    return 0;
+}
+
 }
 
 extern "C" int ldm_conv_forward_ws(const ldm_conv_desc* d, const ldm_conv_plan* plan, const float* x, const float* w,
diff --git a/music-style-transfer-ldm_amd/csrc/loop_prologue.h b/music-style-transfer-ldm_amd/csrc/loop_prologue.h
--- /dev/null
+++ b/music-style-transfer-ldm_amd/csrc/loop_prologue.h
@@ -0,0 +1,45 @@
+#pragma once
+#include "common.h"
+
+#pragma clang fp contract(off)
+
+namespace ldm {
+
+__device__ __forceinline__ void time_mlp_body(const void* t, int t_is_float, int dim, const float* __restrict__ freqs,
+                                              const float* __restrict__ w1, const float* __restrict__ b1,
+                                              const float* __restrict__ w2, const float* __restrict__ b2,
+                                              float* __restrict__ out, float* emb, float* hid, int b, int i, bool on) {
+    const int half = dim / 2;
+    if (on) {
+        const float tv = t_is_float ? ((const float*)t)[b] : (float)((const int64_t*)t)[b];
+        const float arg = tv * freqs[i < half ? i : i - half];
+        emb[i] = i < half ? sinf(arg) : cosf(arg);
+    }
+    __syncthreads();
+    if (on) {
+        const float* wr = w1 + (size_t)i * dim;
+        float acc = 0.f;
+        for (int k = 0; k < dim; ++k) acc = fmaf(wr[k], emb[k], acc);
+        const float x = acc + b1[i];
+        hid[i] = x * 0.5f * (1.0f + erff(x * 0.70710678118654752440f));
+    }
+    __syncthreads();
+    if (on) {
+        const float* wr = w2 + (size_t)i * dim;
+        float acc = 0.f;
+        for (int k = 0; k < dim; ++k) acc = fmaf(wr[k], hid[k], acc);
+        out[(size_t)b * dim + i] = acc + b2[i];
+    }
+}
+
+__device__ __forceinline__ void nchw_to_nhwc_body(const float* __restrict__ x, float* __restrict__ y, int C, int HW,
+                                                  int64_t n, int64_t idx) {
+    if (idx >= n) return;
+    const int c = (int)(idx % C);
+    const int64_t r = idx / C;
+    const int p = (int)(r % HW);
+    const int64_t b = r / HW;
+    y[idx] = x[(b * C + c) * HW + p];
+}
+
+}
diff --git a/music-style-transfer-ldm_amd/csrc/misc.hip b/music-style-transfer-ldm_amd/csrc/misc.hip
--- a/music-style-transfer-ldm_amd/csrc/misc.hip
+++ b/music-style-transfer-ldm_amd/csrc/misc.hip
@@ -1,6 +1,7 @@
 #include <algorithm>
 
 #include "common.h"
+#include "loop_prologue.h"
 
 #pragma clang fp contract(off)
 
@@ -11,30 +12,8 @@
                                                        const float* __restrict__ w2, const float* __restrict__ b2,
                                                        float* __restrict__ out) {
     extern __shared__ __attribute__((aligned(16))) float sm[];
-    float* emb = sm;
-    float* hid = sm + dim;
-    const int b = blockIdx.x, i = threadIdx.x;
-    const float tv = t_is_float ? ((const float*)t)[b] : (float)((const int64_t*)t)[b];
-    const int half = dim / 2;
-    if (i < dim) {
-        const float arg = tv * freqs[i < half ? i : i - half];
-        emb[i] = i < half ? sinf(arg) : cosf(arg);
-    }
-    __syncthreads();
-    if (i < dim) {
-        const float* wr = w1 + (size_t)i * dim;
-        float acc = 0.f;
-        for (int k = 0; k < dim; ++k) acc = fmaf(wr[k], emb[k], acc);
-        const float x = acc + b1[i];
-        hid[i] = x * 0.5f * (1.0f + erff(x * 0.70710678118654752440f));
-    }
-    __syncthreads();
-    if (i < dim) {
-        const float* wr = w2 + (size_t)i * dim;
-        float acc = 0.f;
-        for (int k = 0; k < dim; ++k) acc = fmaf(wr[k], hid[k], acc);
-        out[(size_t)b * dim + i] = acc + b2[i];
-    }
+    const int i = threadIdx.x;
+    time_mlp_body(t, t_is_float, dim, freqs, w1, b1, w2, b2, out, sm, sm + dim, blockIdx.x, i, i < dim);
 }
 
 constexpr int kAttnLT = 16;
@@ -379,14 +358,13 @@
     }
 }
 
-__global__ __launch_bounds__(256) void attention_fold_keys4_kernel(const float* __restrict__ kv, const float* __restrict__ wq,
-                                                                   const float* __restrict__ bq, int B, int E, int heads,
-                                                                   int S, float scale, float* __restrict__ kf,
-                                                                   float* __restrict__ bf) {
+__device__ __forceinline__ void attention_fold_keys4_body(const float* __restrict__ kv, const float* __restrict__ wq,
+                                                          const float* __restrict__ bq, int B, int E, int heads, int S,
+                                                          float scale, float* __restrict__ kf, float* __restrict__ bf,
+                                                          const int64_t idx) {
     const int d = E / heads;
     const int SG = S / 4;
     const int64_t n = (int64_t)B * heads * SG * (E + 1);
-    const int64_t idx = (int64_t)blockIdx.x * blockDim.x + threadIdx.x;
     if (idx >= n) return;
     const int e = (int)(idx % (E + 1));
     int64_t r = idx / (E + 1);
@@ -432,6 +410,29 @@
     float* out = kf + (((int64_t)b * heads + h) * S + sg * 4) * E + e;
 #pragma unroll
     for (int j = 0; j < 4; ++j) out[(int64_t)j * E] = (float)(acc[j] * (double)scale);
+}
+
+__global__ __launch_bounds__(256) void attention_fold_keys4_kernel(const float* __restrict__ kv, const float* __restrict__ wq,
+                                                                   const float* __restrict__ bq, int B, int E, int heads,
+                                                                   int S, float scale, float* __restrict__ kf,
+                                                                   float* __restrict__ bf) {
+    attention_fold_keys4_body(kv, wq, bq, B, E, heads, S, scale, kf, bf, (int64_t)blockIdx.x * blockDim.x + threadIdx.x);
+}
+
+struct FoldKeysJob {
+    const float *kv, *wq, *bq;
+    float *kf, *bf;
+    int32_t E, S;
+    float scale;
+};
+__global__ __launch_bounds__(256) void loop_prologue_b_kernel(FoldKeysJob j1, FoldKeysJob j0, int B, int heads, int nb1) {
+    const int blk = blockIdx.x;
+    if (blk < nb1)
+        attention_fold_keys4_body(j1.kv, j1.wq, j1.bq, B, j1.E, heads, j1.S, j1.scale, j1.kf, j1.bf,
+                                  (int64_t)blk * 256 + threadIdx.x);
+    else
+        attention_fold_keys4_body(j0.kv, j0.wq, j0.bq, B, j0.E, heads, j0.S, j0.scale, j0.kf, j0.bf,
+                                  (int64_t)(blk - nb1) * 256 + threadIdx.x);
 }
 
 __global__ __launch_bounds__(256) void fold_conv_proj_kernel(const float* __restrict__ wc, const float* __restrict__ bc,
@@ -724,16 +725,35 @@
     return 0;
 }
 
+static bool fold_keys4_ok(const float* kv, int32_t S) {
+    static const bool k4_on = [] {
+        const char* e = std::getenv("LDM_FOLD_KEYS4");
+        return e ? std::atoi(e) != 0 : true;
+    }();
+    return k4_on && S % 4 == 0 && ((uintptr_t)kv & 15) == 0;
+}
+
+int attention_fold_keys_pair(const float* kv2, const float* wq2, const float* bq2, int32_t S2, float scale2, float* kf2,
+                             float* bf2, const float* kv1, const float* wq1, const float* bq1, int32_t S1, float scale1,
+                             float* kf1, float* bf1, int32_t B, hipStream_t st, bool& used) {
+    used = false;
+    LDM_REQUIRE(kv2 && wq2 && bq2 && kf2 && bf2 && kv1 && wq1 && bq1 && kf1 && bf1 && B > 0 && S2 > 0 && S1 > 0,
+                "fold keys (pair): bad argument");
+    if (!fold_keys4_ok(kv2, S2) || !fold_keys4_ok(kv1, S1)) return 0;
+    const int64_t nb0 = ((int64_t)B * 4 * (S2 / 4) * (256 + 1) + 255) / 256, nb1 = ((int64_t)B * 4 * (S1 / 4) * (512 + 1) + 255) / 256;
+    LDM_REQUIRE(nb0 + nb1 < 0x7fffffffLL, "fold keys (pair): too many blocks");
+    const FoldKeysJob j0{kv2, wq2, bq2, kf2, bf2, 256, S2, scale2}, j1{kv1, wq1, bq1, kf1, bf1, 512, S1, scale1};
+    hipLaunchKernelGGL(loop_prologue_b_kernel, dim3((unsigned)(nb0 + nb1)), dim3(256), 0, st, j1, j0, B, 4, (int)nb1);
+    LDM_CHECK_LAUNCH("loop_prologue_b_kernel");
+    used = true;
+    return 0;
+}
+
 int attention_fold_keys(const float* kv, const float* wq, const float* bq, int32_t B, int32_t E, int32_t heads,
                         int32_t S, float scale, float* kf, float* bf, hipStream_t st) {
     LDM_REQUIRE(kv && wq && bq && kf && bf && B > 0 && heads > 0 && E % heads == 0 && S > 0, "fold keys: bad argument");
     const int64_t nk = (int64_t)B * heads * E * S, nb = (int64_t)B * heads * S;
-    static const bool k4_on = [] {
-        const char* e = std::getenv("LDM_FOLD_KEYS4");
-        return e ? std::atoi(e) != 0 : true;
-    }();
-    const bool k4 = k4_on && S % 4 == 0 && ((uintptr_t)kv & 15) == 0;
-    if (k4) {
+    if (fold_keys4_ok(kv, S)) {
         const int64_t n4 = (int64_t)B * heads * (S / 4) * (E + 1);
         hipLaunchKernelGGL(attention_fold_keys4_kernel, dim3((unsigned)((n4 + 255) / 256)), dim3(256), 0, st, kv, wq, bq,
                            B, E, heads, S, scale, kf, bf);
diff --git a/music-style-transfer-ldm_amd/csrc/uconv.hip b/music-style-transfer-ldm_amd/csrc/uconv.hip
--- a/music-style-transfer-ldm_amd/csrc/uconv.hip
+++ b/music-style-transfer-ldm_amd/csrc/uconv.hip
@@ -2,6 +2,7 @@
 #include <cstdlib>
 
 #include "uconv_kernel.h"
+#include "loop_prologue.h"
 
 namespace ldm {
 namespace uc {
@@ -28,13 +29,7 @@
 
 __global__ __launch_bounds__(256) void nchw_to_nhwc_kernel(const float* __restrict__ x, float* __restrict__ y, int C,
                                                            int HW, int64_t n) {
-    const int64_t idx = (int64_t)blockIdx.x * blockDim.x + threadIdx.x;
-    if (idx >= n) return;
-    const int c = (int)(idx % C);
-    const int64_t r = idx / C;
-    const int p = (int)(r % HW);
-    const int64_t b = r / HW;
-    y[idx] = x[(b * C + c) * HW + p];
+    nchw_to_nhwc_body(x, y, C, HW, n, (int64_t)blockIdx.x * blockDim.x + threadIdx.x);
 }
 __global__ __launch_bounds__(256) void nhwc_to_nchw_kernel(const float* __restrict__ x, float* __restrict__ y, int C,
                                                            int HW, int64_t n) {
@@ -225,6 +220,7 @@
     a.x0_prev = s.x0_prev;
     if (s.guide_eb) a.skip = s.guide_eb, a.bcast = s.guide_scale, a.y = s.xs2;
     if (s.keep_base) a.skip = s.keep_base, a.bcast = s.keep_row;
+    if (s.x_out) a.y = s.x_out;
     a.B = B;
     a.Hin = Hin;
     a.Win = Win;
@@ -244,6 +240,8 @@
     LDM_REQUIRE(!s.msolver || (layer == 8 && s.x0_log), "step conv: the multistep update is dec1's and needs its x0 log");
     LDM_REQUIRE((!s.plain && !s.guide_eb) || layer == 8, "step conv: the guided loop's two launches are dec1's");
     LDM_REQUIRE(!s.plain || (s.y && !s.guide_eb), "step conv: dec1's base half is a plain conv into y");
+    LDM_REQUIRE(!s.x_out || (layer == 8 && !s.plain && !s.guide_eb && !s.keep_base && !s.y),
+                "step conv: storing the state NCHW is the plain loop's dec1's");
     LDM_REQUIRE(!s.guide_eb || ((s.guide_scale || s.keep_base) && s.xs2 && s.xs2 != s.xs),
                 "step conv: guidance needs its scales and second state");
     LDM_REQUIRE(!s.keep_base || (layer == 8 && !s.plain && s.keep_row && (!s.guide_eb || s.guide_eb == s.keep_base)),
@@ -294,6 +292,7 @@
         if (s.keep_base) return step_dec1_keep(geo, a, s, st);
         if (s.plain || s.guide_eb) return step_dec1_guided(geo, a, s, st);
         LDM_REQUIRE(s.xs && s.coef, "dec1: sampler state, coefficients");
+        if (s.x_out) return step_dec1_last(geo, a, s, st);
     }
     if (ksv == 3) {
         switch (layer) {
diff --git a/music-style-transfer-ldm_amd/csrc/uconv_kernel.h b/music-style-transfer-ldm_amd/csrc/uconv_kernel.h
--- a/music-style-transfer-ldm_amd/csrc/uconv_kernel.h
+++ b/music-style-transfer-ldm_amd/csrc/uconv_kernel.h
@@ -10,7 +10,7 @@
 namespace ldm {
 namespace uc {
 
-enum : int { EPI_RELU = 1, EPI_BCAST = 2, EPI_SKIP = 4, EPI_POSB = 8, EPI_DDIM = 16, EPI_PLANE = 32, EPI_WINDOW = 64, EPI_MSOLVER = 128, EPI_GUIDE = 256, EPI_KEEP = 512 };
+enum : int { EPI_RELU = 1, EPI_BCAST = 2, EPI_SKIP = 4, EPI_POSB = 8, EPI_DDIM = 16, EPI_PLANE = 32, EPI_WINDOW = 64, EPI_MSOLVER = 128, EPI_GUIDE = 256, EPI_KEEP = 512, EPI_XOUT = 1024 };
 
 struct UArgs {
     const float* x;
@@ -627,7 +627,12 @@
 #pragma unroll
                 for (int r = 0; r < 4; ++r) xn[r] = keep_blend(xn[r], pre_kz[k][r], pre_kn[k][r], pre_kw[k], pre_ka, pre_kb);
             }
-            *reinterpret_cast<floatx4*>(a.xs + (size_t)ot.pix * COUT + ot.m) = xn;
+            if constexpr ((EPI & EPI_XOUT) != 0) {
+#pragma unroll
+                for (int r = 0; r < 4; ++r) a.y[lbase + r * hw] = xn[r];
+            } else {
+                *reinterpret_cast<floatx4*>(a.xs + (size_t)ot.pix * COUT + ot.m) = xn;
+            }
             if constexpr ((EPI & EPI_GUIDE) != 0) *reinterpret_cast<floatx4*>(a.y + (size_t)ot.pix * COUT + ot.m) = xn;
         } else if constexpr ((EPI & EPI_DDIM) != 0) {
             const floatx4 xv = pre_s[k];
@@ -645,7 +650,12 @@
 #pragma unroll
                 for (int r = 0; r < 4; ++r) xn[r] = keep_blend(xn[r], pre_kz[k][r], pre_kn[k][r], pre_kw[k], pre_ka, pre_kb);
             }
-            *reinterpret_cast<floatx4*>(a.xs + (size_t)ot.pix * COUT + ot.m) = xn;
+            if constexpr ((EPI & EPI_XOUT) != 0) {
+#pragma unroll
+                for (int r = 0; r < 4; ++r) a.y[lbase + r * hw] = xn[r];
+            } else {
+                *reinterpret_cast<floatx4*>(a.xs + (size_t)ot.pix * COUT + ot.m) = xn;
+            }
             if constexpr ((EPI & EPI_GUIDE) != 0) *reinterpret_cast<floatx4*>(a.y + (size_t)ot.pix * COUT + ot.m) = xn;
         } else {
             *reinterpret_cast<floatx4*>(a.y + (size_t)ot.pix * COUT + ot.m) = o;
@@ -771,6 +781,7 @@
 
 int step_dec1_guided(int geo, const UArgs& a, const StepConv& s, hipStream_t st);
 int step_dec1_keep(int geo, const UArgs& a, const StepConv& s, hipStream_t st);
-
-}
-}
+int step_dec1_last(int geo, const UArgs& a, const StepConv& s, hipStream_t st);
+
+}
+}
diff --git a/music-style-transfer-ldm_amd/csrc/uconv_last.hip b/music-style-transfer-ldm_amd/csrc/uconv_last.hip
--- /dev/null
+++ b/music-style-transfer-ldm_amd/csrc/uconv_last.hip
@@ -0,0 +1,16 @@
+#include "uconv_kernel.h"
+
+namespace ldm {
+namespace uc {
+
+int step_dec1_last(int geo, const UArgs& a, const StepConv& s, hipStream_t st) {
+    LDM_REQUIRE(s.xs && s.coef && a.y && a.y == s.x_out, "dec1 (last step): sampler state, coefficients, x");
+    return dec1_visit(geo, [&](auto g) -> int {
+        constexpr int GEO = decltype(g)::value;
+        if (s.msolver) return dec1_launch<EPI_MSOLVER | EPI_XOUT, GEO>(a, s.dtype, st);
+        return dec1_launch<EPI_DDIM | EPI_XOUT, GEO>(a, s.dtype, st);
+    });
+}
+
+}
+}
diff --git a/music-style-transfer-ldm_amd/csrc/unet.hip b/music-style-transfer-ldm_amd/csrc/unet.hip
--- a/music-style-transfer-ldm_amd/csrc/unet.hip
+++ b/music-style-transfer-ldm_amd/csrc/unet.hip
@@ -312,7 +312,7 @@
 }
 
 static int unet_step_kernels(const ldm_unet_shape& s, const ldm_unet_weights& w, const UNetWs& ws, hipStream_t st,
-                             const float* temb, const DdimFuse& fuse, int S5, int S6, bool bfold) {
+                             const float* temb, const DdimFuse& fuse, int S5, int S6, bool bfold, float* x_out = nullptr) {
     const int HW = s.H * s.W;
     const int L2 = HW / 16, L1 = HW / 64;
     const float* xin[9] = {ws.xs, ws.z1, ws.z2, ws.a2, ws.a1, ws.zb, ws.d4, ws.d3, ws.d2};
@@ -339,6 +339,7 @@
     c[8].eps_log = fuse.eps_log;
     c[8].msolver = fuse.msolver;
     c[8].x0_prev = fuse.x0_prev;
+    c[8].x_out = x_out;
     if (fuse.kw && !fuse.gB) c[8].keep_base = fuse.kbase, c[8].keep_row = fuse.krow, c[8].keep_stride = fuse.kstride;
     auto dec1_guided = [&]() -> int {
         const int Bh = fuse.gB;
@@ -453,6 +454,27 @@
     return 0;
 }
 
+static int g_loop_prologue = [] {
+    const char* e = std::getenv("LDM_LOOP_PROLOGUE");
+    return e ? (std::atoi(e) != 0 ? 1 : 0) : 1;
+}();
+
+static int prologue_stage_a(const ldm_unet_shape& s, const ldm_unet_weights& w, const UNetWs& ws, float* temb_all,
+                            const float* x, const float* s5, const float* s6, const int64_t* t_table, int32_t nsteps,
+                            hipStream_t st, bool& done) {
+    ldm_conv_desc d5, d6;
+    LDM_TRY(layer_desc(s, 10, d5));
+    LDM_TRY(layer_desc(s, 13, d6));
+    return loop_prologue_a(d5, w.ca_plan_kv[0], s5, w.ca_wkv[0], w.ca_bkv[0], ws.kv2, d6, w.ca_plan_kv[1], s6, w.ca_wkv[1],
+                           w.ca_bkv[1], ws.kv1, t_table, nsteps * s.B, w.t_freqs, w.t_w1, w.t_b1, w.t_w2, w.t_b2, temb_all,
+                           x, ws.xs, s.B, s.C, s.H * s.W, st, done);
+}
+static int prologue_stage_b(const ldm_unet_weights& w, const UNetWs& ws, int B, int S5, int S6, hipStream_t st, bool& done) {
+    return attention_fold_keys_pair(ws.kv2, w.ca_wq_raw[0], w.ca_bq[0], S5, (float)std::sqrt(1.0 / 64.0), ws.kf2, ws.bf2,
+                                    ws.kv1, w.ca_wq_raw[1], w.ca_bq[1], S6, (float)std::sqrt(1.0 / 128.0), ws.kf1, ws.bf1,
+                                    B, st, done);
+}
+
 static int sample_loop(const ldm_unet_shape* sc, const ldm_unet_weights* w, float* x, const float* s5, const float* s6,
                        const int64_t* t_table, const float* coef_table, int32_t nsteps, float eta, float* x0_logs,
                        float* eps_logs, int64_t log_step_stride, float* workspace, void* stream, bool msolver,
@@ -475,7 +497,11 @@
     const int64_t n = log_step_stride ? log_step_stride : dense;
     hipStream_t st = (hipStream_t)stream;
     const size_t cw = msolver ? 8 : 4;
-    if (g) {
+    const bool table = g_loop_prologue != 0 && w->use_fold && w->use_step && !g && !kp && !mix;
+    bool a_done = false, b_done = false;
+    if (table) LDM_TRY(prologue_stage_a(*s, *w, ws, temb_all, x, s5, s6, t_table, nsteps, st, a_done));
+    if (a_done) {
+    } else if (g) {
         float* temb_b = temb_all + (size_t)nsteps * s->B * 128;
         LDM_TRY(ldm_time_mlp_forward(t_table, 0, nsteps * sc->B, 128, w->t_freqs, w->t_w1, w->t_b1, w->t_w2, w->t_b2,
                                      temb_b, st));
@@ -495,7 +521,8 @@
         LDM_TRY(ldm_time_mlp_forward(t_table, 0, nsteps * s->B, 128, w->t_freqs, w->t_w1, w->t_b1, w->t_w2, w->t_b2,
                                      temb_all, st));
     }
-    if (S5 == L2 && S6 == L1) {
+    if (a_done) {
+    } else if (S5 == L2 && S6 == L1) {
         LDM_TRY(style_kv(*s, *w, s5, s6, ws, st));
     } else {
         LDM_TRY(style_kv_tokens(*s, *w, 0, s5, S5, ws.kv2, st));
@@ -513,10 +540,14 @@
     if (w->use_fold) {
         LDM_REQUIRE(w->ca_wq_raw[0] && w->ca_wq_raw[1] && w->fold_w[0] && w->fold_w[1] && w->fold_pb[0] && w->fold_pb[1],
                     "ddim_sample: use_fold needs the folded weights");
-        LDM_TRY(attention_fold_keys_bias(ws.kv2, w->ca_wq_raw[0], w->ca_bq[0], s->B, 256, 4, S5,
-                                         (float)std::sqrt(1.0 / 64.0), key_bias5, ws.kf2, ws.bf2, st));
-        LDM_TRY(attention_fold_keys_bias(ws.kv1, w->ca_wq_raw[1], w->ca_bq[1], s->B, 512, 4, S6,
-                                         (float)std::sqrt(1.0 / 128.0), key_bias6, ws.kf1, ws.bf1, st));
+        if (table)
+            LDM_TRY(prologue_stage_b(*w, ws, s->B, S5, S6, st, b_done));
+        if (!b_done) {
+            LDM_TRY(attention_fold_keys_bias(ws.kv2, w->ca_wq_raw[0], w->ca_bq[0], s->B, 256, 4, S5,
+                                             (float)std::sqrt(1.0 / 64.0), key_bias5, ws.kf2, ws.bf2, st));
+            LDM_TRY(attention_fold_keys_bias(ws.kv1, w->ca_wq_raw[1], w->ca_bq[1], s->B, 512, 4, S6,
+                                             (float)std::sqrt(1.0 / 128.0), key_bias6, ws.kf1, ws.bf1, st));
+        }
         if (w->use_step) {
             LDM_REQUIRE(s->C == 32 && s->nf == 64, "ddim_sample: the step kernels are built for latent 32 / 64 filters");
             for (int l = 0; l < 9; ++l) LDM_REQUIRE(w->step_w[l], "ddim_sample: use_step needs the step weights");
@@ -524,8 +555,9 @@
             LDM_REQUIRE(w->step_dtype >= LDM_DT_F32 && w->step_dtype <= LDM_DT_BF16, "ddim_sample: step_dtype");
             const bool bfold = use_bneck_fold(*s, w) && S6 == L1 && !key_bias6;
             if (bfold) LDM_TRY(bneck_fold_values(w->step_bneck_w, ws.kv1, ws.ubn, s->B, st));
-            LDM_TRY(step_layout(x, ws.xs, sc->B, s->C, HW, true, st));
+            if (!a_done) LDM_TRY(step_layout(x, ws.xs, sc->B, s->C, HW, true, st));
             if (g) LDM_TRY(step_layout(x, ws.xs + dense, sc->B, s->C, HW, true, st));
+            const bool xout = g_loop_prologue != 0 && !g && !kp;
             float* kreg = temb_all + (size_t)nsteps * (g ? 3 : 1) * sc->B * 128;
             const int krl = 2 + (g ? sc->B : 0);
             float* krows = kreg + (g ? 3 : 2) * dense + (int64_t)sc->B * HW;
@@ -545,8 +577,10 @@
                     fuse.kbase = kreg, fuse.krow = krows + (size_t)i * krl, fuse.kstride = dense;
                     if (g) fuse.eb = kreg;
                 }
-                LDM_TRY(unet_step_kernels(*s, *w, ws, st, temb_all + (size_t)i * s->B * 128, fuse, S5, S6, bfold));
+                LDM_TRY(unet_step_kernels(*s, *w, ws, st, temb_all + (size_t)i * s->B * 128, fuse, S5, S6, bfold,
+                                          xout && i == nsteps - 1 ? x : nullptr));
             }
+            if (xout) return 0;
             return step_layout(ws.xs, x, sc->B, s->C, HW, false, st);
         }
     }
@@ -596,6 +630,33 @@
     const int64_t avail = (int64_t)(((const char*)base + size) - (const char*)workspace);
     LDM_REQUIRE(avail >= need * 4, "sample: the workspace's allocation ends before the size ldm_sample_workspace_floats "
                                    "gives for these arguments (was it sized for another configuration?)");
+    return 0;
+}
+
+extern "C" int ldm_set_loop_prologue(int on) {
+    const int prev = g_loop_prologue;
+    g_loop_prologue = on ? 1 : 0;
+    return prev;
+}
+
+extern "C" int ldm_loop_prologue(const ldm_unet_shape* s, const ldm_unet_weights* w, const float* x, const float* s5,
+                                 const float* s6, const int64_t* t_table, int32_t nsteps, float* workspace, void* stream,
+                                 int64_t* off, int32_t* stages) {
+    LDM_REQUIRE(s && w && x && s5 && s6 && t_table && workspace && off && stages && nsteps > 0 && s->B > 0,
+                "loop prologue: bad argument");
+    LDM_REQUIRE(w->use_fold && w->use_step && w->ca_wq_raw[0] && w->ca_wq_raw[1], "loop prologue: use_fold and use_step");
+    const int L2 = s->H * s->W / 16, L1 = s->H * s->W / 64;
+    const UNetWs ws = carve(*s, w, workspace);
+    float* temb_all = workspace + ws.total;
+    const bool bfold = use_bneck_fold(*s, w);
+    float* const bufs[9] = {temb_all, ws.kv2, ws.kv1, ws.kf2, ws.bf2, ws.kf1, ws.bf1, bfold ? ws.ubn : nullptr, ws.xs};
+    for (int i = 0; i < 9; ++i) off[i] = bufs[i] ? bufs[i] - workspace : -1;
+    hipStream_t st = (hipStream_t)stream;
+    bool a_done = false, b_done = false;
+    LDM_TRY(prologue_stage_a(*s, *w, ws, temb_all, x, s5, s6, t_table, nsteps, st, a_done));
+    if (a_done) LDM_TRY(prologue_stage_b(*w, ws, s->B, L2, L1, st, b_done));
+    if (b_done && bfold) LDM_TRY(bneck_fold_values(w->step_bneck_w, ws.kv1, ws.ubn, s->B, st));
+    *stages = (a_done ? 1 : 0) | (b_done ? 2 : 0) | (b_done && bfold ? 4 : 0);
     return 0;
 }
 
diff --git a/music-style-transfer-ldm_amd/ldm_amd/_lib.py b/music-style-transfer-ldm_amd/ldm_amd/_lib.py
--- a/music-style-transfer-ldm_amd/ldm_amd/_lib.py
+++ b/music-style-transfer-ldm_amd/ldm_amd/_lib.py
@@ -181,6 +181,9 @@
     "ldm_set_cin1_packed": (c_int32, [c_int32]),
     "ldm_set_cin1_s1": (c_int32, [c_int32]),
     "ldm_set_flash_split": (c_int32, [c_int32]),
+    "ldm_set_loop_prologue": (c_int32, [c_int32]),
+    "ldm_loop_prologue": (c_int32, [ctypes.POINTER(UNetShape), ctypes.POINTER(UNetWeights), c_fp, c_fp, c_fp, c_vp,
+                                    c_int32, c_fp, c_vp, ctypes.POINTER(c_int64), ctypes.POINTER(c_int32)]),
     "ldm_q_sample": (c_int32, [c_fp, c_fp, c_fp, c_int32, c_vp, c_fp, c_int32, c_int64, c_vp]),
     "ldm_predict_start": (c_int32, [c_fp, c_fp, c_fp, c_int32, c_vp, c_fp, c_int32, c_int64, c_vp]),
     "ldm_sched_backward": (c_int32, [c_int32, c_fp, c_fp, c_int32, c_vp, c_fp, c_fp, c_int32, c_int64, c_vp]),
```

After: 14650 steps/s (median of 4 runs). Within noise of the previous version (+0.3%).
